# MILAB-IIT-CV/ATDN_vSLAM

Measured on AMD Instinct MI355X. Metric: frame-pairs/sec, KITTI 1241x376 odometry inference at 1/2/4/8 MI355X, higher is better.
Workload: dtype f32 via 3xf16 split MFMA (fp32 accumulate); 1 GPU; KITTI seq-03-shaped 376x1241 uint8 frames (resident in HBM) resized to 376x1232, GMA flow 12 GRU iters + CLVO head -> 6-DoF trajectory (BASELINE configs[1]); streams_per_gpu=2, gru_iters=12, parallelism=pairs sharded x1, one all-gather of 512-d features, replicated LSTM scan

## Files before the change

### atdn_vslam_amd/csrc/capi.hip

```cpp
#include "../../include/atdn_hip.h"

#include <cmath>
#include <cstring>

#include "clvo.h"
#include "gma.h"
#include "vae.h"
#include "clvo_train.h"
#include "train_kernels.h"
#include "frontend.h"
#include "conv_sf.h"
#include "depth_fusion_host.h"
#include "epilogues_sf.h"
#include "epipolar_host.h"
#include "flow_args.h"
#include "flow_consistency_host.h"
#include "flow_track_host.h"
#include "multiview_depth_host.h"
#include "pnp_host.h"
#include "two_view_host.h"
#include "warm_start_host.h"

namespace atdn {
extern template TileChoice conv_dispatch<MODE_TAP, EpiBias<ACT_NONE>>(const ConvShape&, EpiBias<ACT_NONE>, hipStream_t);
extern template TileChoice conv_dispatch<MODE_TAP, EpiBias<ACT_RELU>>(const ConvShape&, EpiBias<ACT_RELU>, hipStream_t);
extern template TileChoice conv_dispatch<MODE_ROW, EpiBias<ACT_NONE>>(const ConvShape&, EpiBias<ACT_NONE>, hipStream_t);
extern template TileChoice conv_dispatch<MODE_ROW, EpiBias<ACT_RELU>>(const ConvShape&, EpiBias<ACT_RELU>, hipStream_t);
extern template TileChoice conv_dispatch<MODE_TAP, EpiScale>(const ConvShape&, EpiScale, hipStream_t);

extern template TileChoice conv_sf_dispatch<EpiBias<ACT_NONE>>(const ConvShape&, float, EpiBias<ACT_NONE>, hipStream_t);
extern template TileChoice conv_sf_dispatch<SfBias<ACT_NONE>>(const ConvShape&, float, SfBias<ACT_NONE>, hipStream_t);

static thread_local std::string g_last_error;
void set_last_error(const std::string& msg) { g_last_error = msg; }
}

using namespace atdn;

struct atdn_gma { GmaNet net; atdn_gma(int H, int W, int B, int prec) : net(H, W, B, prec) {} };
struct atdn_clvo { ClvoNet net; atdn_clvo(int H, int W, int B) : net(H, W, B) {} };
struct atdn_vae { VaeEncoder net; atdn_vae(int H, int W, int B) : net(H, W, B) {} };
struct atdn_ingest { FrameIngest in; atdn_ingest(int a, int b, int c, int d, int n, int aa) : in(a, b, c, d, n, aa) {} };
struct atdn_clvo_trainer { ClvoTrainer net; atdn_clvo_trainer(int H, int W, int B, int T) : net(H, W, B, T) {} };

template <class T>
static void euler_yxz(const T* r, T* R) {
  const T c1 = std::cos(r[0]), c2 = std::cos(r[1]), c3 = std::cos(r[2]);
  const T s1 = std::sin(r[0]), s2 = std::sin(r[1]), s3 = std::sin(r[2]);
  R[0] = c1 * c3 + s1 * s2 * s3; R[1] = c3 * s1 * s2 - c1 * s3; R[2] = c2 * s1;
  R[3] = c2 * s3;                R[4] = c2 * c3;                R[5] = -s2;
  R[6] = c1 * s2 * s3 - c3 * s1; R[7] = c1 * c3 * s2 + s1 * s3; R[8] = c1 * c2;
}
template <class T>
static void make_transform(const T* rot, const T* tr, T* m) {
  T R[9];
  euler_yxz(rot, R);
  for (int i = 0; i < 3; ++i) { for (int j = 0; j < 3; ++j) m[i * 4 + j] = R[i * 3 + j]; m[i * 4 + 3] = tr[i]; }
  m[12] = 0; m[13] = 0; m[14] = 0; m[15] = 1;
}
template <class T>
static void matmul4(const T* a, const T* b, T* c) {
  for (int i = 0; i < 4; ++i)
    for (int j = 0; j < 4; ++j) {
      T s = 0;
      for (int k = 0; k < 4; ++k) s += a[i * 4 + k] * b[k * 4 + j];
      c[i * 4 + j] = s;
    }
}

extern "C" {

int atdn_version(void) { return 100; }
const char* atdn_last_error(void) { return g_last_error.c_str(); }

int atdn_gma_create(atdn_gma** out, int H, int W, int max_batch, int precision) {
  ATDN_API_BEGIN
  ATDN_CHECK(out, "null out pointer");
  *out = new atdn_gma(H, W, max_batch, precision);
  ATDN_API_END
}
int atdn_gma_set_low_latency(atdn_gma* h, int on) {
  ATDN_API_BEGIN
  ATDN_CHECK(h, "null handle");
  h->net.set_low_latency(on != 0);
  ATDN_API_END
}
int atdn_gma_load(atdn_gma* h, const char* key, const float* data, const int64_t* shape, int rank) {
  ATDN_API_BEGIN
  ATDN_CHECK(h && key && data && rank >= 0 && rank <= 4, "bad state-dict entry");
  h->net.state().put(key, data, shape, rank);
  ATDN_API_END
}
int atdn_gma_finalize(atdn_gma* h) {
  ATDN_API_BEGIN
  ATDN_CHECK(h, "null handle");
  h->net.finalize();
  ATDN_API_END
}
int atdn_gma_forward(atdn_gma* h, const float* im1, const float* im2, int B, int iters, const float* flow_init,
                     float* flow_low, float* flow_up, void* stream) {
  ATDN_API_BEGIN
  ATDN_CHECK(h, "null handle");
  h->net.forward(im1, im2, B, iters, flow_init, flow_low, flow_up, (hipStream_t)stream);
  ATDN_API_END
}
int atdn_gma_forward_predictions(atdn_gma* h, const float* im1, const float* im2, int B, int iters, const float* flow_init,
                                 float* flow_predictions, void* stream) {
  ATDN_API_BEGIN
  ATDN_CHECK(h, "null handle");
  h->net.forward_predictions(im1, im2, B, iters, flow_init, flow_predictions, (hipStream_t)stream);
  ATDN_API_END
}
int atdn_gma_forward_sequence(atdn_gma* h, const float* frames, int B, int iters, const float* flow_init,
                              float* flow_low, float* flow_up, void* stream) {
  ATDN_API_BEGIN
  ATDN_CHECK(h, "null handle");
  h->net.forward_sequence(frames, B, iters, flow_init, flow_low, flow_up, (hipStream_t)stream);
  ATDN_API_END
}
int atdn_gma_forward_sequence_continued(atdn_gma* h, const float* frames, int B, int iters, const float* flow_init,
                                        float* flow_low, float* flow_up, void* stream) {
  ATDN_API_BEGIN
  ATDN_CHECK(h, "null handle");
  h->net.forward_sequence(frames, B, iters, flow_init, flow_low, flow_up, (hipStream_t)stream, true);
  ATDN_API_END
}
long atdn_gma_debug_read(atdn_gma* h, const char* name, float* host, long capacity, void* stream) {
  try {
    if (!h || !name || !host) throw Error("null argument");
    const long n = h->net.debug_read(name, host, capacity, (hipStream_t)stream);
    if (n < 0) throw Error(std::string("unknown tensor name: ") + name);
    return n;
  } catch (const std::exception& e) {
    set_last_error(e.what());
    return -1;
  }
}
int atdn_gma_profile(atdn_gma* h, int B, int iters, int reps, float* ms_out, void* stream) {
  ATDN_API_BEGIN
  ATDN_CHECK(h && ms_out, "null argument");
  static_assert(GmaNet::ST_COUNT == ATDN_GMA_STAGES, "stage table out of sync with the header");
  h->net.profile(B, iters, reps, ms_out, (hipStream_t)stream, 0);
  ATDN_API_END
}
int atdn_gma_profile_mode(atdn_gma* h, int B, int iters, int reps, int mode, float* ms_out, void* stream) {
  ATDN_API_BEGIN
  ATDN_CHECK(h && ms_out, "null argument");
  ATDN_CHECK(mode >= 0 && mode <= 2, "mode must be 0 (pair), 1 (sequence) or 2 (continued sequence)");
  h->net.profile(B, iters, reps, ms_out, (hipStream_t)stream, mode);
  ATDN_API_END
}
int atdn_gma_set_range_probe(atdn_gma* h, int on) {
  ATDN_API_BEGIN
  ATDN_CHECK(h, "null handle");
  h->net.set_probe(on != 0);
  ATDN_API_END
}
long atdn_gma_range_rows(atdn_gma* h) {
  if (!h) { set_last_error("null handle"); return -1; }
  return (long)h->net.probe_rows().size();
}
int atdn_gma_range_row(atdn_gma* h, long index, char* name, int name_capacity, int* iteration, int* limited, float* max_abs,
                       int64_t* over, int64_t* nonfinite) {
  ATDN_API_BEGIN
  ATDN_CHECK(h && name && iteration && limited && max_abs && over && nonfinite, "null argument");
  const auto& rows = h->net.probe_rows();
  ATDN_CHECK(index >= 0 && index < (long)rows.size(), "row index out of range");
  const GmaNet::ProbeRow& r = rows[(size_t)index];
  ATDN_CHECK(name_capacity > (int)r.name.size(), "name buffer too small");
  memcpy(name, r.name.c_str(), r.name.size() + 1);
  *iteration = r.iter; *limited = r.limited ? 1 : 0; *max_abs = r.max_abs;
  *over = (int64_t)r.over; *nonfinite = (int64_t)r.nonfinite;
  ATDN_API_END
}
int atdn_range_probe_launch(const float* x, int64_t rows, int64_t cols, int64_t ld, void* slot, void* stream) {
  ATDN_API_BEGIN
  launch_range_probe(x, (long)rows, (long)cols, (long)ld, static_cast<RangeSlot*>(slot), (hipStream_t)stream);
  ATDN_API_END
}
int atdn_range_probe(const float* x, int64_t rows, int64_t cols, int64_t ld, float* max_abs, int64_t* over, int64_t* nonfinite,
                     void* stream) {
  ATDN_API_BEGIN
  ATDN_CHECK(x && max_abs && over && nonfinite, "null argument");
  hipStream_t st = (hipStream_t)stream;
  DeviceArray<RangeSlot> slot;
  RangeSlot host{};
  slot.alloc(1);
  ATDN_HIP(hipMemsetAsync(slot.p, 0, sizeof(RangeSlot), st));
  launch_range_probe(x, (long)rows, (long)cols, (long)ld, slot.p, st);
  ATDN_HIP(hipMemcpyAsync(&host, slot.p, sizeof(RangeSlot), hipMemcpyDeviceToHost, st));
  ATDN_HIP(hipStreamSynchronize(st));
  memcpy(max_abs, &host.max_bits, sizeof(float));
  *over = (int64_t)host.over;
  *nonfinite = (int64_t)host.nonfinite;
  ATDN_API_END
}
size_t atdn_gma_workspace_bytes(atdn_gma* h) { return h ? h->net.workspace_bytes() : 0; }
void atdn_gma_destroy(atdn_gma* h) { delete h; }
int64_t atdn_device_bytes_live(void) { return (int64_t)device_bytes_live.load(); }

int atdn_clvo_create(atdn_clvo** out, int H, int W, int max_batch) {
  ATDN_API_BEGIN
  ATDN_CHECK(out, "null out pointer");
  *out = new atdn_clvo(H, W, max_batch);
  ATDN_API_END
}
int atdn_clvo_load(atdn_clvo* h, const char* key, const float* data, const int64_t* shape, int rank) {
  ATDN_API_BEGIN
  ATDN_CHECK(h && key && data && rank >= 0 && rank <= 4, "bad state-dict entry");
  h->net.state().put(key, data, shape, rank);
  ATDN_API_END
}
int atdn_clvo_finalize(atdn_clvo* h) {
  ATDN_API_BEGIN
  ATDN_CHECK(h, "null handle");
  h->net.finalize();
  ATDN_API_END
}
int atdn_clvo_encode(atdn_clvo* h, const float* flow, int B, float* feat, void* stream) {
  ATDN_API_BEGIN
  ATDN_CHECK(h && flow && feat, "null argument");
  h->net.encode(flow, B, feat, (hipStream_t)stream);
  ATDN_API_END
}
int atdn_clvo_step(atdn_clvo* h, const float* feat, int T, int Bs, float* state, float* rot, float* tr, void* stream) {
  ATDN_API_BEGIN
  ATDN_CHECK(h && feat && state && rot && tr, "null argument");
  h->net.step(feat, T, Bs, state, rot, tr, (hipStream_t)stream);
  ATDN_API_END
}
int atdn_clvo_last_scan_path(atdn_clvo* h) { return h ? h->net.last_scan_path() : 0; }
void atdn_clvo_destroy(atdn_clvo* h) { delete h; }

int atdn_vae_create(atdn_vae** out, int H, int W, int max_batch) {
  ATDN_API_BEGIN
  ATDN_CHECK(out, "null out pointer");
  *out = new atdn_vae(H, W, max_batch);
  ATDN_API_END
}
int atdn_vae_load(atdn_vae* h, const char* key, const float* data, const int64_t* shape, int rank) {
  ATDN_API_BEGIN
  ATDN_CHECK(h && key && data && rank >= 0 && rank <= 4, "bad state-dict entry");
  h->net.state().put(key, data, shape, rank);
  ATDN_API_END
}
int atdn_vae_finalize(atdn_vae* h) {
  ATDN_API_BEGIN
  ATDN_CHECK(h, "null handle");
  h->net.finalize();
  ATDN_API_END
}
int atdn_vae_embedding_shape(const atdn_vae* h, int* out_h, int* out_w) {
  ATDN_API_BEGIN
  ATDN_CHECK(h && out_h && out_w, "null argument");
  *out_h = h->net.out_h();
  *out_w = h->net.out_w();
  ATDN_API_END
}
int atdn_vae_encode(atdn_vae* h, const float* images, int B, float* mu, void* stream) {
  ATDN_API_BEGIN
  ATDN_CHECK(h && images && mu, "null argument");
  h->net.encode(images, B, mu, (hipStream_t)stream);
  ATDN_API_END
}
int atdn_vae_debug_stage(atdn_vae* h, const float* images, int B, int stage, float* out, long capacity, void* stream) {
  ATDN_API_BEGIN
  ATDN_CHECK(h && images && out, "null argument");
  h->net.debug_stage(images, B, stage, out, capacity, (hipStream_t)stream);
  ATDN_API_END
}
int atdn_vae_scratch_floats(int H, int W, long* floats, int* stages) {
  ATDN_API_BEGIN
  ATDN_CHECK(floats && stages, "null argument");
  ATDN_CHECK(H >= 1 && W >= 1 && (long)H * W <= (1L << 24), "frame size out of range");
  const VaePlan p = vae_plan(H, W);
  floats[0] = p.in4; floats[1] = p.bufA; floats[2] = p.bufB; floats[3] = p.bufS;
  for (int k = 0; k < kVaeStages; ++k) { stages[3 * k] = p.h[k]; stages[3 * k + 1] = p.w[k]; stages[3 * k + 2] = p.ld[k]; }
  ATDN_API_END
}
void atdn_vae_destroy(atdn_vae* h) { delete h; }

int atdn_clvo_trainer_create(atdn_clvo_trainer** out, int H, int W, int batch, int sequence_length) {
  ATDN_API_BEGIN
  ATDN_CHECK(out, "null out pointer");
  *out = new atdn_clvo_trainer(H, W, batch, sequence_length);
  ATDN_API_END
}
int atdn_clvo_trainer_load(atdn_clvo_trainer* h, const char* key, const float* data, const int64_t* shape, int rank) {
  ATDN_API_BEGIN
  ATDN_CHECK(h && key && data && rank >= 0 && rank <= 4, "bad state-dict entry");
  h->net.state().put(key, data, shape, rank);
  ATDN_API_END
}
int atdn_clvo_trainer_finalize(atdn_clvo_trainer* h) {
  ATDN_API_BEGIN
  ATDN_CHECK(h, "null handle");
  h->net.finalize();
  ATDN_API_END
}
int atdn_clvo_trainer_forward_backward(atdn_clvo_trainer* h, const float* flows, const float* true_rot, const float* true_tr,
                                       float* pred_rot, float* pred_tr, float* loss_out, void* stream) {
  ATDN_API_BEGIN
  ATDN_CHECK(h && flows && true_rot && true_tr && loss_out, "null argument");
  *loss_out = h->net.forward_backward(flows, true_rot, true_tr, pred_rot, pred_tr, (hipStream_t)stream);
  ATDN_API_END
}
int atdn_clvo_trainer_gradients(atdn_clvo_trainer* h, float** device_ptr, long* count) {
  ATDN_API_BEGIN
  ATDN_CHECK(h && device_ptr && count, "null argument");
  *device_ptr = h->net.grad_buffer();
  *count = h->net.grad_count();
  ATDN_API_END
}
int atdn_clvo_trainer_adamw_step(atdn_clvo_trainer* h, float lr, float weight_decay, float eps, int step, void* stream) {
  ATDN_API_BEGIN
  ATDN_CHECK(h, "null handle");
  h->net.adamw_step(lr, weight_decay, eps, step, (hipStream_t)stream);
  ATDN_API_END
}
int atdn_clvo_trainer_set_loss(atdn_clvo_trainer* h, float alpha, int w, int mode) {
  ATDN_API_BEGIN
  ATDN_CHECK(h, "null handle");
  h->net.set_loss(alpha, w, mode);
  ATDN_API_END
}
int atdn_clvo_trainer_loss_terms(atdn_clvo_trainer* h, float* terms3_host) {
  ATDN_API_BEGIN
  ATDN_CHECK(h && terms3_host, "null argument");
  const float* t = h->net.loss_terms();
  ATDN_CHECK(t, "loss_terms: no iteration with alpha != 1 has run since set_loss");
  std::memcpy(terms3_host, t, 3 * sizeof(float));
  ATDN_API_END
}
int atdn_clvo_loss(const float* pred_rot, const float* pred_tr, const float* true_rot, const float* true_tr, int B, int T, float alpha,
                   int w, int mode, float* loss3_host, float* d_rot, float* d_tr, void* stream) {
  ATDN_API_BEGIN
  ATDN_CHECK(pred_rot && pred_tr && true_rot && true_tr && loss3_host && d_rot && d_tr, "null argument");
  ATDN_CHECK(mode == 0 || mode == 1, "atdn_clvo_loss: mode is 0 (reference) or 1 (gradient)");
  ATDN_CHECK(B >= 1 && T >= 1 && w >= 1 && w <= T, "atdn_clvo_loss: the composite window needs 1 <= w <= sequence length");
  hipStream_t st = (hipStream_t)stream;
  DeviceBuf loss3;
  loss3.alloc(4);
  launch_clvo_loss_composite(pred_rot, pred_tr, true_rot, true_tr, B, T, alpha, w, mode == 1, false, loss3.p, d_rot, d_tr, st);
  ATDN_HIP(hipMemcpyAsync(loss3_host, loss3.p, 3 * sizeof(float), hipMemcpyDeviceToHost, st));
  ATDN_HIP(hipStreamSynchronize(st));
  ATDN_API_END
}
long atdn_clvo_trainer_read(atdn_clvo_trainer* h, const char* key, int kind, float* host, long capacity, void* stream) {
  try {
    ATDN_CHECK(h && key && host, "null argument");
    return h->net.read(key, kind, host, capacity, (hipStream_t)stream);
  } catch (const std::exception& e) {
    set_last_error(e.what());
    return -1;
  }
}
void atdn_clvo_trainer_destroy(atdn_clvo_trainer* h) { delete h; }

int atdn_pose_transform_f32(const float* rot, const float* tr, float* mat16) {
  ATDN_API_BEGIN
  ATDN_CHECK(rot && tr && mat16, "null argument");
  make_transform(rot, tr, mat16);
  ATDN_API_END
}
int atdn_pose_rel2abs(const float* rot, const float* tr, int T, double* poses) {
  ATDN_API_BEGIN
  ATDN_CHECK(rot && tr && poses && T >= 0, "bad argument");
  for (int i = 0; i < 16; ++i) poses[i] = (i % 5 == 0) ? 1.0 : 0.0;
  for (int t = 0; t < T; ++t) {
    const double r[3] = {rot[t * 3], rot[t * 3 + 1], rot[t * 3 + 2]};
    const double x[3] = {tr[t * 3], tr[t * 3 + 1], tr[t * 3 + 2]};
    double m[16];
    make_transform(r, x, m);
    matmul4(poses + (long)t * 16, m, poses + (long)(t + 1) * 16);
  }
  ATDN_API_END
}
int atdn_pose_accumulate_f32(float* pose16, const float* rot, const float* tr) {
  ATDN_API_BEGIN
  ATDN_CHECK(pose16 && rot && tr, "null argument");
  float m[16], o[16];
  make_transform(rot, tr, m);
  matmul4(pose16, m, o);
  for (int i = 0; i < 16; ++i) pose16[i] = o[i];
  ATDN_API_END
}

int atdn_flow_forward_interpolate_host(const float* flow_low, int B, int h, int w, float* out) {
  ATDN_API_BEGIN
  ATDN_CHECK(flow_low && out, "null argument");
  ATDN_CHECK(B >= 1 && h >= 1 && w >= 1 && (long)h * w <= (1L << 24), "bad batch or grid size");
  const long bytes = (long)B * 2 * h * w * 4;
  ATDN_CHECK(disjoint(flow_low, bytes, out, bytes), "input and output overlap");
  forward_interpolate_host(flow_low, B, h, w, out);
  ATDN_API_END
}

int atdn_flow_consistency_host(const float* flow_fw, const float* flow_bw, int B, int H, int W, double alpha1, double alpha2,
                               unsigned char* mask, int* count) {
  ATDN_API_BEGIN
  flow_consistency_check_args(flow_fw, flow_bw, B, H, W, alpha1, alpha2, mask, count);
  flow_consistency_host(flow_fw, flow_bw, B, H, W, alpha1, alpha2, mask, count);
  ATDN_API_END
}

int atdn_flow_two_view_depth_host(const float* flow, const float* pose, const unsigned char* mask, int B, int H, int W, double fx,
                                  double fy, double cx, double cy, double max_epipolar, double min_sin2, double max_depth,
                                  float* depth, int* counts) {
  ATDN_API_BEGIN
  const TwoViewCamera cam{fx, fy, cx, cy, max_epipolar, min_sin2, max_depth};
  two_view_check_args(flow, pose, mask, B, H, W, cam, depth, counts);
  two_view_depth_host(flow, pose, mask, B, H, W, cam, depth, counts);
  ATDN_API_END
}

int atdn_flow_track_step_host(const float* flow, const unsigned char* mask, const float* acc_in, const unsigned char* alive_in,
                              int B, int H, int W, float* acc_out, unsigned char* alive_out, const float* pose, double fx,
                              double fy, double cx, double cy, double max_epipolar, double min_sin2, double max_depth, float* depth,
                              int* counts) {
  ATDN_API_BEGIN
  const TwoViewCamera cam{fx, fy, cx, cy, max_epipolar, min_sin2, max_depth};
  flow_track_check_args(flow, mask, acc_in, alive_in, B, H, W, acc_out, alive_out, pose, cam, depth, counts);
  flow_track_step_host(flow, mask, acc_in, alive_in, B, H, W, acc_out, alive_out, pose, cam, depth, counts);
  ATDN_API_END
}

int atdn_depth_fuse_host(const float* bank, const float* poses, const int* targets, const int* sources, int N, int B, int S, int H,
                         int W, double fx, double fy, double cx, double cy, double max_reproj, double max_rel_depth, int min_views,
                         double min_z, int average, float* fused, unsigned char* views, int* counts) {
  ATDN_API_BEGIN
  depth_fuse_check_args(bank, poses, targets, sources, N, B, S, H, W, fx, fy, cx, cy, max_reproj, max_rel_depth, min_views, min_z,
                        fused, views, counts);
  depth_fuse_host(bank, poses, targets, sources, N, B, S, H, W,
                  depth_fuse_params(fx, fy, cx, cy, max_reproj, max_rel_depth, min_views, min_z, average), fused, views, counts);
  ATDN_API_END
}

int atdn_multiview_depth_host(const float* acc_bank, const unsigned char* alive_bank, const float* poses, const int* slots,
                              const float* depth_init, int N, int B, int S, int H, int W, double fx, double fy, double cx, double cy,
                              double scale_px, double inlier_px, double min_z, int min_views, double max_rel_sigma, double max_depth,
                              int iters, float* depth, float* info, unsigned char* views, int* counts) {
  ATDN_API_BEGIN
  multiview_check_args(acc_bank, alive_bank, poses, slots, depth_init, N, B, S, H, W, fx, fy, cx, cy, scale_px, inlier_px, min_z,
                       min_views, max_rel_sigma, max_depth, iters, depth, info, views, counts);
  multiview_depth_host(acc_bank, alive_bank, poses, slots, depth_init, N, B, S, H, W,
                       multiview_params(fx, fy, cx, cy, scale_px, inlier_px, min_z, min_views, max_rel_sigma, max_depth, iters, H, W),
                       depth, info, views, counts);
  ATDN_API_END
}

int atdn_pnp_terms_host(const float* depth, const float* flow, const unsigned char* mask, const float* pose, int B, int H, int W,
                        double fx, double fy, double cx, double cy, double scale_px, double inlier_px, double min_z, double* sums,
                        int* counts) {
  ATDN_API_BEGIN
  const void* out[2] = {sums, counts};
  const long out_bytes[2] = {(long)B * PNP_TERMS * 8, (long)B * 12};
  pnp_check_args(depth, flow, mask, pose, B, H, W, fx, fy, cx, cy, scale_px, inlier_px, min_z, false, out, out_bytes, 2);
  pnp_terms_host(depth, flow, mask, pose, B, H, W, pnp_params(fx, fy, cx, cy, scale_px, inlier_px, min_z, H, W), sums, counts);
  ATDN_API_END
}

int atdn_pnp_solve_host(const float* depth, const float* flow, const unsigned char* mask, const float* pose_init, int B, int H,
                        int W, double fx, double fy, double cx, double cy, double scale_px, double inlier_px, double min_z, int iters,
                        float* pose_out, double* cost, int* counts) {
  ATDN_API_BEGIN
  const void* out[3] = {pose_out, cost, counts};
  const long out_bytes[3] = {(long)B * 48, (long)B * 8, (long)B * 16};
  pnp_check_args(depth, flow, mask, pose_init, B, H, W, fx, fy, cx, cy, scale_px, inlier_px, min_z, false, out, out_bytes, 3);
  ATDN_CHECK(iters >= 0 && iters <= 64, "iters must be in [0, 64]");
  pnp_solve_host(depth, flow, mask, pose_init, B, H, W, pnp_params(fx, fy, cx, cy, scale_px, inlier_px, min_z, H, W), iters,
                 pose_out, cost, counts);
  ATDN_API_END
}

int atdn_epipolar_terms_host(const float* flow, const unsigned char* mask, const float* pose, int B, int H, int W, double fx,
                             double fy, double cx, double cy, double scale_px, double inlier_px, double* sums, int* counts) {
  ATDN_API_BEGIN
  const void* out[2] = {sums, counts};
  const long out_bytes[2] = {(long)B * PLANE_TERMS * 8, (long)B * 12};
  epipolar_check_args(flow, mask, pose, B, H, W, fx, fy, cx, cy, scale_px, inlier_px, false, out, out_bytes, 2);
  epipolar_terms_host(flow, mask, pose, B, H, W, epipolar_params(fx, fy, cx, cy, scale_px, inlier_px), sums, counts);
  ATDN_API_END
}

int atdn_epipolar_solve_host(const float* flow, const unsigned char* mask, const float* pose_init, int B, int H, int W, double fx,
                             double fy, double cx, double cy, double scale_px, double inlier_px, int iters, float* pose_out,
                             double* cost, int* counts) {
  ATDN_API_BEGIN
  const void* out[3] = {pose_out, cost, counts};
  const long out_bytes[3] = {(long)B * 48, (long)B * 8, (long)B * 16};
  epipolar_check_args(flow, mask, pose_init, B, H, W, fx, fy, cx, cy, scale_px, inlier_px, false, out, out_bytes, 3);
  ATDN_CHECK(iters >= 0 && iters <= 64, "iters must be in [0, 64]");
  epipolar_solve_host(flow, mask, pose_init, B, H, W, epipolar_params(fx, fy, cx, cy, scale_px, inlier_px), iters, pose_out, cost,
                      counts);
  ATDN_API_END
}

int atdn_corr_lookup(const float* pyr0, const float* pyr1, const float* pyr2, const float* pyr3, int B, int H8,
                     int W8, const float* coords, float* out, int ldo, void* stream) {
  ATDN_API_BEGIN
  ATDN_CHECK(pyr0 && pyr1 && pyr2 && pyr3 && coords && out && B >= 1, "null argument");
  ATDN_CHECK((H8 >> 3) >= 2 && (W8 >> 3) >= 2, "map too small for four pyramid levels");
  PyramidLevels pl;
  const float* b[4] = {pyr0, pyr1, pyr2, pyr3};
  for (int l = 0; l < 4; ++l) { pl.base[l] = b[l]; pl.H[l] = H8 >> l; pl.W[l] = W8 >> l; }
  launch_lookup(pl, coords, (long)B * H8 * W8, out, ldo, (hipStream_t)stream);
  ATDN_API_END
}

int atdn_corr_pyramid(const float* fmap1, const float* fmap2, int B, int H8, int W8, int C, float* pyr0, float* pyr1,
                      float* pyr2, float* pyr3, void* stream) {
  ATDN_API_BEGIN
  ATDN_CHECK(fmap1 && fmap2 && pyr0 && pyr1 && pyr2 && pyr3 && B >= 1 && C % 32 == 0, "bad argument");
  const int N = H8 * W8;
  ConvShape c;
  c.src0 = fmap1; c.ld0 = C; c.sb0 = (long)N * C; c.C0 = C; c.H = 1; c.W = N;
  c.w = fmap2; c.wb = (long)N * C; c.ldw = C; c.N = N; c.nimg = B;
  conv_dispatch<MODE_TAP>(c, EpiScale{1.0f / sqrtf((float)C), pyr0, (long)N * N, N}, (hipStream_t)stream);
  float* p[4] = {pyr0, pyr1, pyr2, pyr3};
  for (int l = 1; l < 4; ++l) launch_avgpool(p[l - 1], H8 >> (l - 1), W8 >> (l - 1), p[l], (long)B * N, (hipStream_t)stream);
  ATDN_API_END
}

int atdn_corr_lookup_bricks(const float* fmap1, const float* fmap2, int B, int H8, int W8, int C, const float* coords,
                            float* pyr0, float* pyr1, float* pyr2, float* pyr3, float* samples,
                            const float* convc1_weight_host, const float* convc1_bias_host, float* cor1, void* stream) {
  ATDN_API_BEGIN
  ATDN_CHECK(fmap1 && fmap2 && B >= 1 && H8 >= 1 && W8 >= 1, "bad argument");
  ATDN_CHECK(C == 256, "the correlation kernel keeps a source strip's whole K = 256 in registers: C must be 256");
  ATDN_CHECK((H8 >> 3) >= 2 && (W8 >> 3) >= 2, "map too small for four pyramid levels");
  ATDN_CHECK(!(samples || cor1) || coords, "a lookup needs coordinates");
  ATDN_CHECK(!cor1 || (convc1_weight_host && convc1_bias_host), "cor1 needs convc1's weight [256][324] and bias [256]");
  hipStream_t st = (hipStream_t)stream;
  const int N = H8 * W8;
  const long n8 = (long)B * N;
  BrickPyramid bp;
  bp.N = N; bp.NPB = brick_pixel_blocks(N);
  WeightArena A;
  DeviceBuf f1, f2, plain[3], fbrick[4], pyr[4], scratch, outsf, csf;
  sf_counter_attach();
  f1.alloc(n8 * 256); f2.alloc(n8 * 256);
  launch_to_sf(fmap1, f1.p, n8, 256, st);
  launch_to_sf(fmap2, f2.p, n8, 256, st);
  float* rowmajor[4] = {pyr0, pyr1, pyr2, pyr3};
  int pH[4], pW[4];
  for (int l = 0; l < 4; ++l) {
    pH[l] = H8 >> l; pW[l] = W8 >> l;
    bp.H[l] = pH[l]; bp.W[l] = pW[l]; bp.BW[l] = cdiv(pW[l], 8); bp.BH[l] = cdiv(pH[l], 4); bp.NB[l] = bp.BW[l] * bp.BH[l] * 32;
    const float* src = f2.p;
    long src_sb = (long)N * 256;
    if (l > 0) {
      const float* prev = l == 1 ? f2.p : plain[l - 2].p;
      const long prev_sb = l == 1 ? (long)N * 256 : (long)pH[l - 1] * pW[l - 1] * 256;
      src_sb = (long)pH[l] * pW[l] * 256;
      plain[l - 1].alloc((long)B * src_sb);
      launch_pool_features_sf(prev, B, pH[l - 1], pW[l - 1], 256, prev_sb, plain[l - 1].p, src_sb, st);
      src = plain[l - 1].p;
    }
    fbrick[l].alloc((long)B * bp.NB[l] * 256);
    launch_brick_rows(src, src_sb, B, pH[l], pW[l], 256, fbrick[l].p, (long)bp.NB[l] * 256, st);
    pyr[l].alloc((long)B * bp.NPB * kBrickPixelBlock * bp.NB[l]);
    launch_corr_bricks(f1.p, (long)N * 256, fbrick[l].p, (long)bp.NB[l] * 256, B, N, bp.NB[l], 1.0f / sqrtf(256.0f), pyr[l].p, false, st);
    bp.base[l] = pyr[l].p;
    if (rowmajor[l]) launch_unbrick(pyr[l].p, bp.NB[l], N, pH[l], pW[l], n8, rowmajor[l], st);
  }
  if (samples) {
    outsf.alloc(n8 * 352);
    launch_lookup_bricks(bp, coords, n8, outsf.p, st);
    scratch.alloc(n8 * 352);
    launch_from_sf(outsf.p, scratch.p, n8, 352, st);
    ATDN_HIP(hipMemcpy2DAsync(samples, 324 * sizeof(float), scratch.p, 352 * sizeof(float), 324 * sizeof(float), (size_t)n8,
                              hipMemcpyDeviceToDevice, st));
  }
  if (cor1) {
    StateDict sd;
    const int64_t ws[4] = {256, 324, 1, 1}, bs[1] = {256};
    sd.put("c.weight", convc1_weight_host, ws, 4);
    sd.put("c.bias", convc1_bias_host, bs, 1);
    PackedConv L = pack_conv_sf(A, sd, {"c"});
    pack_fragment_major16(A, L);
    A.upload();
    resolve(A, L);
    csf.alloc(n8 * 256);
    launch_lookup_conv(bp, coords, n8, nullptr, L.wf16, L.wscale, L.b, csf.p, false, st);
    launch_from_sf(csf.p, cor1, n8, 256, st);
    ATDN_HIP(hipStreamSynchronize(st));
  }
  ATDN_HIP(hipStreamSynchronize(st));
  ATDN_API_END
}

int atdn_conv2d_nhwc(const float* src, int nimg, int H, int W, int Cin, const float* weight_host,
                     const float* bias_host, int Cout, int KH, int KW, int stride, int padH, int padW, int relu,
                     float* dst, void* stream) {
  ATDN_API_BEGIN
  ATDN_CHECK(src && weight_host && dst && nimg >= 1, "null argument");
  const bool row = (Cin == 4 || Cin == 16);
  ATDN_CHECK(row || Cin % 32 == 0, "Cin must be 4, 16 or a multiple of 32");
  StateDict sd;
  const int64_t ws[4] = {Cout, Cin, KH, KW};
  sd.put("c.weight", weight_host, ws, 4);
  std::vector<float> zb(Cout, 0.f);
  const int64_t bs[1] = {Cout};
  sd.put("c.bias", bias_host ? bias_host : zb.data(), bs, 1);
  WeightArena A;
  PackedConv L = pack_conv(A, sd, {"c"}, row ? MODE_ROW : MODE_TAP, Cin);
  A.upload();
  resolve(A, L);
  ConvShape s;
  s.src0 = src; s.ld0 = Cin; s.sb0 = (long)H * W * Cin; s.C0 = L.C; s.H = H; s.W = W;
  s.KH = KH; s.KW = KW; s.stride = stride; s.padH = padH; s.padW = padW;
  s.w = L.w; s.ldw = L.ldw; s.N = Cout; s.nimg = nimg;
  const int Ho = conv_out(H, KH, stride, padH), Wo = conv_out(W, KW, stride, padW);
  hipStream_t st = (hipStream_t)stream;
  if (row) {
    if (relu) conv_dispatch<MODE_ROW>(s, EpiBias<ACT_RELU>{L.b, dst, (long)Ho * Wo * Cout, Cout, 1.f}, st);
    else conv_dispatch<MODE_ROW>(s, EpiBias<ACT_NONE>{L.b, dst, (long)Ho * Wo * Cout, Cout, 1.f}, st);
  } else {
    if (relu) conv_dispatch<MODE_TAP>(s, EpiBias<ACT_RELU>{L.b, dst, (long)Ho * Wo * Cout, Cout, 1.f}, st);
    else conv_dispatch<MODE_TAP>(s, EpiBias<ACT_NONE>{L.b, dst, (long)Ho * Wo * Cout, Cout, 1.f}, st);
  }
  ATDN_HIP(hipStreamSynchronize(st));
  ATDN_API_END
}

int atdn_resize_frames(const float* src, int planes, int Hin, int Win, int Hout, int Wout, float* dst, void* stream) {
  return atdn_resize_frames_mode(src, planes, Hin, Win, Hout, Wout, ATDN_RESIZE_ANTIALIAS, dst, stream);
}
int atdn_resize_frames_mode(const float* src, int planes, int Hin, int Win, int Hout, int Wout, int antialias, float* dst,
                            void* stream) {
  ATDN_API_BEGIN
  ATDN_CHECK(src && dst && planes >= 1 && Hin >= 1 && Win >= 1 && Hout >= 1 && Wout >= 1, "bad argument");
  ATDN_CHECK(antialias == 0 || antialias == 1, "antialias must be ATDN_RESIZE_BILINEAR or ATDN_RESIZE_ANTIALIAS");
  launch_resize<float>(src, planes, Hin, Win, Hout, Wout, antialias, dst, (hipStream_t)stream);
  ATDN_API_END
}
int atdn_resize_frames_u8(const uint8_t* src, int planes, int Hin, int Win, int Hout, int Wout, int antialias, float* dst,
                          void* stream) {
  ATDN_API_BEGIN
  ATDN_CHECK(src && dst && planes >= 1 && Hin >= 1 && Win >= 1 && Hout >= 1 && Wout >= 1, "bad argument");
  ATDN_CHECK(antialias == 0 || antialias == 1, "antialias must be ATDN_RESIZE_BILINEAR or ATDN_RESIZE_ANTIALIAS");
  launch_resize<unsigned char>(src, planes, Hin, Win, Hout, Wout, antialias, dst, (hipStream_t)stream);
  ATDN_API_END
}
int atdn_pad_frames(const float* src, int planes, int H, int W, int left, int right, int top, int bottom, float* dst,
                    void* stream) {
  ATDN_API_BEGIN
  ATDN_CHECK(src && dst && planes >= 1 && H >= 1 && W >= 1 && left >= 0 && right >= 0 && top >= 0 && bottom >= 0, "bad argument");
  launch_pad_replicate(src, planes, H, W, left, right, top, bottom, dst, (hipStream_t)stream);
  ATDN_API_END
}
int atdn_ingest_create(atdn_ingest** out, int Hin, int Win, int Hout, int Wout, int max_frames, int antialias) {
  ATDN_API_BEGIN
  ATDN_CHECK(out, "null out pointer");
  ATDN_CHECK(antialias == 0 || antialias == 1, "antialias must be ATDN_RESIZE_BILINEAR or ATDN_RESIZE_ANTIALIAS");
  *out = new atdn_ingest(Hin, Win, Hout, Wout, max_frames, antialias);
  ATDN_API_END
}
int atdn_ingest_frames_u8(atdn_ingest* h, const uint8_t* host_frames, int n_frames, float* dst, void* stream) {
  ATDN_API_BEGIN
  ATDN_CHECK(h, "null handle");
  h->in.ingest(host_frames, n_frames, dst, (hipStream_t)stream);
  ATDN_API_END
}
void atdn_ingest_destroy(atdn_ingest* h) { delete h; }

int atdn_conv2d_nhwc_sf_epi(const float* src, int nimg, int H, int W, int Cin, const float* weight_host,
                            const float* bias_host, int Cout, int KH, int KW, int stride, int padH, int padW, int sf_store,
                            float* dst, void* stream) {
  ATDN_API_BEGIN
  ATDN_CHECK(src && weight_host && dst && nimg >= 1 && Cin % 32 == 0, "bad argument (Cin must be a multiple of 32)");
  ATDN_CHECK(sf_store >= 0 && sf_store <= 7 && (sf_store & 6) != 6, "sf_store: bit 0 names the epilogue, bit 1 or bit 2 the tile form");
  const int tile_form = (sf_store & 2) ? 1 : (sf_store & 4) ? 2 : 0;
  sf_store &= 1;
  ATDN_CHECK(!sf_store || Cout % 32 == 0, "the split-f16 store needs Cout % 32 == 0");
  StateDict sd;
  const int64_t ws[4] = {Cout, Cin, KH, KW};
  sd.put("c.weight", weight_host, ws, 4);
  std::vector<float> zb(Cout, 0.f);
  const int64_t bs[1] = {Cout};
  sd.put("c.bias", bias_host ? bias_host : zb.data(), bs, 1);
  WeightArena A;
  PackedConv L = pack_conv_sf(A, sd, {"c"});
  A.upload();
  resolve(A, L);
  hipStream_t st = (hipStream_t)stream;
  DeviceBuf tmp, osf;
  const long rows = (long)nimg * H * W;
  tmp.alloc(rows * Cin);
  launch_to_sf(src, tmp.p, rows, Cin, st);
  ConvShape s;
  s.src0 = tmp.p; s.ld0 = Cin; s.sb0 = (long)H * W * Cin; s.C0 = L.C; s.H = H; s.W = W;
  s.KH = KH; s.KW = KW; s.stride = stride; s.padH = padH; s.padW = padW;
  s.w = L.w; s.ldw = L.ldw; s.N = Cout; s.nimg = nimg;
  const int Ho = conv_out(H, KH, stride, padH), Wo = conv_out(W, KW, stride, padW);
  s.wfrag16 = L.wf16;
  s.tile_form = tile_form;
  if (sf_store) {
    const long orows = (long)nimg * Ho * Wo;
    osf.alloc(orows * Cout);
    conv_sf_dispatch(s, L.wscale, SfBias<ACT_NONE>{L.b, osf.p, (long)Ho * Wo * Cout, Cout}, st);
    launch_from_sf(osf.p, dst, orows, Cout, st);
    ATDN_HIP(hipStreamSynchronize(st));
  } else {
    conv_sf_dispatch(s, L.wscale, EpiBias<ACT_NONE>{L.b, dst, (long)Ho * Wo * Cout, Cout, 1.f}, st);
    ATDN_HIP(hipStreamSynchronize(st));
  }
  ATDN_API_END
}

int atdn_conv2d_nhwc_sf(const float* src, int nimg, int H, int W, int Cin, const float* weight_host,
                        const float* bias_host, int Cout, int KH, int KW, int stride, int padH, int padW, float* dst,
                        void* stream) {
  return atdn_conv2d_nhwc_sf_epi(src, nimg, H, W, Cin, weight_host, bias_host, Cout, KH, KW, stride, padH, padW, 0, dst, stream);
}

}
```

### atdn_vslam_amd/csrc/corr_bricks.hip

```cpp
#include "kernels.h"

#include "conv_mfma.h"
#include "sf.h"

namespace atdn {
namespace {

typedef float v4f __attribute__((ext_vector_type(4)));
typedef float f32x4v __attribute__((ext_vector_type(4)));
typedef __attribute__((address_space(1))) v4f gv4f;

struct CorrArgs {
  const float* f1; long sb1;
  const float* f2b; long sb2;
  float* out;
  int B, N, NB, NPB, strips, splits, tiles_per_split;
  float scale;
};

template <bool FAST>
__global__ __launch_bounds__(256, 2) void corr_bricks_kernel(const CorrArgs a) {
  constexpr int KROW = 160;
  constexpr int KT = 32;
  constexpr int NC = 8;
  constexpr int CH = KT * KROW;
  constexpr int IMG = NC * CH;
  __shared__ __attribute__((aligned(16))) char lds[2 * IMG];

  const int tid = threadIdx.x, lane = tid & 63, wave = tid >> 6;
  const int nblk = a.B * a.splits * a.strips;
  const int id = xcd_remap(blockIdx.x, nblk);
  const int strip4 = id % a.strips;
  const int rest = id / a.strips;
  const int split = rest % a.splits, b = rest / a.splits;
  const int n16 = lane & 15, g16 = lane >> 4;
  const char* f1 = reinterpret_cast<const char*>(a.f1 + (long)b * a.sb1);
  const char* f2 = reinterpret_cast<const char*>(a.f2b + (long)b * a.sb2);

  f16x8 qh[2][NC], ql[2][NC];
  int mrow[2];
#pragma unroll
  for (int rb = 0; rb < 2; ++rb) {
    mrow[rb] = (strip4 * 4 + wave) * 32 + 16 * rb + n16;
    const char* qrow = f1 + (long)min(mrow[rb], a.N - 1) * 1024 + 16 * g16;
#pragma unroll
    for (int c = 0; c < NC; ++c) {
      qh[rb][c] = *reinterpret_cast<const f16x8*>(qrow + c * 128);
      if (!FAST) ql[rb][c] = *reinterpret_cast<const f16x8*>(qrow + c * 128 + 64);
    }
  }

  const int lr = tid >> 3, ls = tid & 7;
  const int t0 = split * a.tiles_per_split;
  const int nt = min(a.tiles_per_split, a.NB / KT - t0);
  v4f kreg[NC];
  auto fetch = [&](int j) __attribute__((always_inline)) {
    const char* src = f2 + (long)((t0 + j) * KT + lr) * 1024 + 16 * ls;
#pragma unroll
    for (int c = 0; c < NC; ++c) kreg[c] = *reinterpret_cast<const v4f*>(src + c * 128);
  };
  auto stash = [&](int buf) __attribute__((always_inline)) {
#pragma unroll
    for (int c = 0; c < NC; ++c) *reinterpret_cast<v4f*>(lds + buf * IMG + c * CH + lr * KROW + 16 * ls) = kreg[c];
  };
  const bool odd = (lane & 1) != 0;
  long orow[2][2];
  const long NBK = a.NB / KT;
#pragma unroll
  for (int rb = 0; rb < 2; ++rb)
#pragma unroll
    for (int h = 0; h < 2; ++h) {
      const int prow = h == 0 ? (mrow[rb] & ~1) : (mrow[rb] | 1);
      orow[rb][h] = ((((long)b * a.NPB + (prow >> 6)) * NBK + t0) * 64 + (prow & 63)) * KT + (odd ? 16 : 0) + 4 * g16;
    }

  fetch(0);
  stash(0);
  __syncthreads();
  fetch(min(1, nt - 1));
  for (int j = 0; j < nt; ++j) {
    const char* img = lds + (j & 1) * IMG + n16 * KROW + 16 * g16;
    f32x4v acc[2][2];
#pragma unroll
    for (int kb = 0; kb < 2; ++kb)
#pragma unroll
      for (int rb = 0; rb < 2; ++rb)
#pragma unroll
        for (int e = 0; e < 4; ++e) acc[kb][rb][e] = 0.f;
    f16x8 kh[2][2], kl[2][2];
    auto read_rows = [&](int set, int c) __attribute__((always_inline)) {
#pragma unroll
      for (int kb = 0; kb < 2; ++kb) {
        const char* kp = img + c * CH + 16 * kb * KROW;
        kh[set][kb] = *reinterpret_cast<const f16x8*>(kp);
        if (!FAST) kl[set][kb] = *reinterpret_cast<const f16x8*>(kp + 64);
      }
    };
    read_rows(0, 0);
#pragma unroll
    for (int c = 0; c < NC; ++c) {
      if (c + 1 < NC) read_rows((c + 1) & 1, c + 1);
      __builtin_amdgcn_sched_barrier(0);
#pragma unroll
      for (int kb = 0; kb < 2; ++kb)
#pragma unroll
        for (int rb = 0; rb < 2; ++rb) {
          f32x4v v = acc[kb][rb];
          if (!FAST) {
            v = __builtin_amdgcn_mfma_f32_16x16x32_f16(kl[c & 1][kb], qh[rb][c], v, 0, 0, 0);
            v = __builtin_amdgcn_mfma_f32_16x16x32_f16(kh[c & 1][kb], ql[rb][c], v, 0, 0, 0);
          }
          v = __builtin_amdgcn_mfma_f32_16x16x32_f16(kh[c & 1][kb], qh[rb][c], v, 0, 0, 0);
          acc[kb][rb] = v;
        }
      __builtin_amdgcn_sched_barrier(0);
    }
    stash((j + 1) & 1);
    fetch(min(j + 2, nt - 1));
#pragma unroll
    for (int rb = 0; rb < 2; ++rb) {
      const f32x4v A = acc[0][rb] * a.scale, Bv = acc[1][rb] * a.scale;
      f32x4v recv;
#pragma unroll
      for (int e = 0; e < 4; ++e) {
        const float send = odd ? A[e] : Bv[e];
        recv[e] = __int_as_float(__builtin_amdgcn_update_dpp(0, __float_as_int(send), 0xB1, 0xF, 0xF, true));
      }
      f32x4v v1, v2;
#pragma unroll
      for (int e = 0; e < 4; ++e) { v1[e] = odd ? recv[e] : A[e]; v2[e] = odd ? Bv[e] : recv[e]; }
      __builtin_nontemporal_store(v1, reinterpret_cast<gv4f*>(reinterpret_cast<uintptr_t>(a.out + orow[rb][0])));
      __builtin_nontemporal_store(v2, reinterpret_cast<gv4f*>(reinterpret_cast<uintptr_t>(a.out + orow[rb][1])));
      orow[rb][0] += 64 * KT;
      orow[rb][1] += 64 * KT;
    }
    __syncthreads();
  }
}

}

void launch_corr_bricks(const float* f1, long sb1, const float* f2b, long sb2, int B, int N, int NB, float scale, float* out,
                        bool fast, hipStream_t st) {
  ATDN_CHECK(f1 && f2b && out && B >= 1 && N >= 1 && NB >= 32 && NB % 32 == 0, "corr_bricks: bad argument");
  CorrArgs a;
  a.NPB = brick_pixel_blocks(N);
  a.f1 = f1; a.sb1 = sb1; a.f2b = f2b; a.sb2 = sb2; a.out = out; a.B = B; a.N = N; a.NB = NB; a.scale = scale;
  a.strips = cdiv(N, 128);
  const int tiles = NB / 32;
  int best = 1;
  double best_eff = 0.0;
  for (int s = 1; s <= 8; ++s) {
    const int tps = cdiv(tiles, s);
    if (s > 1 && tps < 8) break;
    const int used = cdiv(tiles, tps);
    const double blocks = (double)B * a.strips * used;
    const double eff = blocks / (512.0 * std::ceil(blocks / 512.0));
    if (eff > best_eff + 0.02) { best_eff = eff; best = s; }
  }
  a.tiles_per_split = cdiv(tiles, best);
  a.splits = cdiv(tiles, a.tiles_per_split);
  const int nblk = B * a.splits * a.strips;
  if (fast) hipLaunchKernelGGL(corr_bricks_kernel<true>, dim3(nblk), dim3(256), 0, st, a);
  else hipLaunchKernelGGL(corr_bricks_kernel<false>, dim3(nblk), dim3(256), 0, st, a);
  ATDN_HIP(hipGetLastError());
}

}
```

### atdn_vslam_amd/csrc/gma.h

```cpp
#pragma once
#include <vector>
#include <map>
#include <memory>

#include "attention.h"
#include "conv_dispatch.h"
#include "device_buf.h"
#include "kernels.h"
#include "range_probe.h"
#include "weights.h"

namespace atdn {

struct EncoderWeights {
  PackedConv stem;
  struct Block { PackedConv c1, c2, ds; bool has_ds = false; } blk[6];
  PackedConv head;
};

class GmaNet {
 public:
  GmaNet(int H, int W, int max_batch, int precision);
  ~GmaNet();
  StateDict& state() { return sd_; }
  void finalize();
  void forward(const float* im1, const float* im2, int B, int iters, const float* flow_init, float* flow_low,
               float* flow_up, hipStream_t st);
  void forward_predictions(const float* im1, const float* im2, int B, int iters, const float* flow_init, float* preds,
                           hipStream_t st);
  void forward_sequence(const float* frames, int B, int iters, const float* flow_init, float* flow_low, float* flow_up,
                        hipStream_t st, bool continued = false);
  long debug_read(const char* name, float* host, long capacity, hipStream_t st);
  size_t workspace_bytes() const { return ws_bytes_; }
  enum Stage { ST_FNET = 0, ST_CORR, ST_POOL, ST_CNET, ST_ATTN, ST_LOOKUP, ST_MOTION, ST_AGG, ST_GRU_ZR, ST_GRU_Q, ST_FLOWHEAD,
               ST_MASK, ST_GRU_CTX, ST_ATTN_LOGITS, ST_AGG_VT, ST_CONVC1, ST_GRU_ZR_V, ST_GRU_Q_V, ST_COUNT };
  void profile(int B, int iters, int reps, float* ms, hipStream_t st, int mode = 0);

  int H, W, H8, W8, N, ldN, maxB, precision;
  int dev_ = 0;
  bool norm_on_load_ = false;
  bool classic_ = false;
  bool low_latency_ = false;
  void set_low_latency(bool on);
  DeviceBuf attn_part_;
  DeviceBuf enc2_[4];
  hipStream_t par_stream_ = nullptr;
  std::vector<hipEvent_t> par_events_;
  size_t par_next_ = 0;
  bool par_ = false;
  bool par_ok_ = true;
  void fork(hipStream_t from, hipStream_t to);
  DeviceBuf fbrick_[4], fplain_[3], coords_used_;
  int brickBW_[4], brickBH_[4], brickNB_[4];
  BrickPyramid brick_pyramid() const;
  DeviceBuf rowmax_, rinv_;

  struct ProbeRow { std::string name; int iter; bool limited; float max_abs; long long over, nonfinite; };
  static constexpr int kProbeMaxRows = 1536;
  void set_probe(bool on);
  const std::vector<ProbeRow>& probe_rows() const { return probe_rows_; }

 private:
  bool probe_ = false;
  int probe_it_ = -1;
  DeviceArray<RangeSlot> probe_slots_;
  std::vector<ProbeRow> probe_rows_;
  void probe_begin(hipStream_t st);
  void probe_end(hipStream_t st);
  void probe(const std::string& name, bool limited, const float* p, long rows, long cols, long ld, hipStream_t st);
  void run_body(int B, int iters, hipStream_t st);
  void run_encoder(const EncoderWeights& E, bool instance, int nimg, hipStream_t st, float** out_buf, int* outH,
                   int* outW);
  void iteration(int B, hipStream_t st);
  void run_body_sf(int B, int iters, hipStream_t st);
  void run_encoder_sf(const EncoderWeights& E, bool instance, int nimg, hipStream_t st, float** out_buf, int first_img = 0,
                      DeviceBuf* bufs = nullptr);
  void iteration_sf(int B, hipStream_t st);
  void capture(int B, int iters);
  void launch_body(int B, int iters, hipStream_t st);
  int seq_ = 0;
  int last_frame_ = -1;
  float* preds_out_ = nullptr;
  long preds_stride_ = 0;
  void mask_head_sf(int B, hipStream_t st);
  void mask_head(int B, hipStream_t st);
  int last_B_ = 0;

  StateDict sd_;
  WeightArena arena_;
  bool ready_ = false;
  bool use_graph_ = true;
  EncoderWeights fnet_, cnet_;
  PackedConv convc1_, convc2_, convf1_, convf2_, convm_, to_v_, to_qk_;
  long convf1_sf_off_ = -1;
  float convf1_wscale_ = 1.f;
  float fh2_mul_ = 1.f;
  long fh2_w32_off_ = -1;
  DeviceBuf fhG_;
  PackedConv gru_zr_[2], gru_q_[2], fh1_, fh2_, mask0_, mask2_;
  PackedConv gru_zr_ctx_[2], gru_q_ctx_[2];
  const float* gamma_ = nullptr;
  long gamma_off_ = -1;
  long to_v_w32_off_ = -1;

  DeviceBuf img4_, enc_[4], scratch_, pcnt_, fin_, fmap_, psum_, pm2_, mean_[3], rstd_[3];
  DeviceBuf pyr_[4], h_[2], x_, qk_, attn_, vT_, corrfeat_, cor1_, corflo_, flo1_, z_, rh_, fh_, mask_;
  DeviceBuf coords1_, flow4_, pre_zr_[2], pre_q_[2];
  int pyrH_[4], pyrW_[4];
  size_t ws_bytes_ = 0;

  struct Timer;
  Timer* timer_ = nullptr;
  void mark(int stage, hipStream_t st);

  hipStream_t cap_stream_ = nullptr;
  std::map<std::pair<int, int>, hipGraphExec_t> graphs_;
};

}
```

### atdn_vslam_amd/csrc/gma.hip

```cpp
#include "gma.h"
#include "small_convs.h"
#include "conv_sf.h"
#include "epilogues_sf.h"

namespace atdn { const float* zero_line(); }

namespace atdn {

extern template TileChoice conv_dispatch<MODE_TAP, EpiBias<ACT_NONE>>(const ConvShape&, EpiBias<ACT_NONE>, hipStream_t);
extern template TileChoice conv_dispatch<MODE_TAP, EpiBias<ACT_RELU>>(const ConvShape&, EpiBias<ACT_RELU>, hipStream_t);
extern template TileChoice conv_dispatch<MODE_ROW, EpiBias<ACT_RELU>>(const ConvShape&, EpiBias<ACT_RELU>, hipStream_t);
extern template TileChoice conv_dispatch<MODE_TAP, EpiBiasStats>(const ConvShape&, EpiBiasStats, hipStream_t);
extern template TileChoice conv_dispatch<MODE_ROW, EpiBiasStats>(const ConvShape&, EpiBiasStats, hipStream_t);
extern template TileChoice conv_dispatch<MODE_TAP, EpiBiasReluAddRelu>(const ConvShape&, EpiBiasReluAddRelu, hipStream_t);
extern template TileChoice conv_dispatch<MODE_TAP, EpiContextSplit>(const ConvShape&, EpiContextSplit, hipStream_t);
extern template TileChoice conv_dispatch<MODE_TAP, EpiScale>(const ConvShape&, EpiScale, hipStream_t);
extern template TileChoice conv_dispatch<MODE_TAP, EpiQK>(const ConvShape&, EpiQK, hipStream_t);
extern template TileChoice conv_dispatch<MODE_TAP, EpiStoreT>(const ConvShape&, EpiStoreT, hipStream_t);
extern template TileChoice conv_dispatch<MODE_TAP, EpiAggregate>(const ConvShape&, EpiAggregate, hipStream_t);
extern template TileChoice conv_dispatch<MODE_TAP, EpiGruZR>(const ConvShape&, EpiGruZR, hipStream_t);
extern template TileChoice conv_dispatch<MODE_TAP, EpiGruQ>(const ConvShape&, EpiGruQ, hipStream_t);
extern template TileChoice conv_dispatch<MODE_TAP, EpiFlowDelta>(const ConvShape&, EpiFlowDelta, hipStream_t);

extern template TileChoice conv_dispatch<MODE_ROW, SfBias<ACT_RELU>>(const ConvShape&, SfBias<ACT_RELU>, hipStream_t);
#define ATDN_EXTERN_SF(EPI) extern template TileChoice conv_sf_dispatch<EPI>(const ConvShape&, float, EPI, hipStream_t);
ATDN_EXTERN_SF(SfBias<ACT_NONE>) ATDN_EXTERN_SF(SfBias<ACT_RELU>) ATDN_EXTERN_SF(EpiBias<ACT_NONE>)
ATDN_EXTERN_SF(EpiBiasStats) ATDN_EXTERN_SF(SfBiasReluAddRelu) ATDN_EXTERN_SF(SfContextSplit)
ATDN_EXTERN_SF(SfQK) ATDN_EXTERN_SF(SfVT)
ATDN_EXTERN_SF(SfGruZR) ATDN_EXTERN_SF(SfGruQ)
extern template void conv_sf_dispatch_pair<SfBias<ACT_RELU>>(const ConvShape&, float, SfBias<ACT_RELU>, const ConvShape&, float,
                                                             SfBias<ACT_RELU>, hipStream_t);

namespace {

struct FastGuard {
  bool prev;
  explicit FastGuard(bool on) : prev(sf_fast_mode()) { sf_fast_mode() = on; }
  ~FastGuard() { sf_fast_mode() = prev; }
};

constexpr int XLD = 384;
constexpr int CORR_LD = 352;

ConvShape conv_shape(const PackedConv& L, const float* src, int ld, long sb, int nimg, int H, int W, int stride,
                     int padH, int padW) {
  ConvShape s;
  s.src0 = src; s.ld0 = ld; s.sb0 = sb; s.C0 = L.C;
  s.H = H; s.W = W; s.KH = L.KH; s.KW = L.KW; s.stride = stride; s.padH = padH; s.padW = padW;
  s.w = L.w; s.wfrag16 = L.wf16; s.ldw = L.ldw; s.N = L.N; s.nimg = nimg;
  return s;
}

EncoderWeights pack_encoder(WeightArena& A, const StateDict& sd, const std::string& p, bool batchnorm, bool sf) {
  EncoderWeights E;
  auto fold = [&](const std::string& norm) { return bn_affine(sd, norm); };
  auto pack_conv = [&](WeightArena& A_, const StateDict& sd_, const std::vector<std::string>& names, int mode, int cpix,
                       const ChannelAffine* f = nullptr) {
    return (sf && mode == MODE_TAP) ? pack_conv_sf(A_, sd_, names, f) : atdn::pack_conv(A_, sd_, names, mode, cpix, f);
  };
  if (batchnorm) { auto a = fold(p + "norm1"); E.stem = pack_conv(A, sd, {p + "conv1"}, MODE_ROW, 4, &a); }
  else E.stem = pack_conv(A, sd, {p + "conv1"}, MODE_ROW, 4);
  if (sf) pack_stem_sf(A, E.stem);
  int bi = 0;
  for (int li = 1; li <= 3; ++li)
    for (int k = 0; k < 2; ++k, ++bi) {
      const std::string q = p + "layer" + std::to_string(li) + "." + std::to_string(k) + ".";
      auto& B = E.blk[bi];
      B.has_ds = (li > 1 && k == 0);
      if (batchnorm) {
        auto a1 = fold(q + "norm1"), a2 = fold(q + "norm2");
        B.c1 = pack_conv(A, sd, {q + "conv1"}, MODE_TAP, 0, &a1);
        B.c2 = pack_conv(A, sd, {q + "conv2"}, MODE_TAP, 0, &a2);
        if (B.has_ds) { auto a3 = fold(q + "norm3"); B.ds = pack_conv(A, sd, {q + "downsample.0"}, MODE_TAP, 0, &a3); }
      } else {
        B.c1 = pack_conv(A, sd, {q + "conv1"}, MODE_TAP, 0);
        B.c2 = pack_conv(A, sd, {q + "conv2"}, MODE_TAP, 0);
        if (B.has_ds) B.ds = pack_conv(A, sd, {q + "downsample.0"}, MODE_TAP, 0);
      }
    }
  E.head = pack_conv(A, sd, {p + "conv2"}, MODE_TAP, 0);
  return E;
}

void resolve_encoder(const WeightArena& A, EncoderWeights& E) {
  resolve(A, E.stem);
  for (auto& b : E.blk) { resolve(A, b.c1); resolve(A, b.c2); if (b.has_ds) resolve(A, b.ds); }
  resolve(A, E.head);
}

}

struct GmaNet::Timer {
  std::vector<std::pair<int, hipEvent_t>> marks;
  hipEvent_t start = nullptr;
};

void GmaNet::mark(int stage, hipStream_t st) {
  if (!timer_) return;
  hipEvent_t e;
  ATDN_HIP(hipEventCreate(&e));
  ATDN_HIP(hipEventRecord(e, st));
  timer_->marks.emplace_back(stage, e);
}

void GmaNet::profile(int B, int iters, int reps, float* ms, hipStream_t st, int mode) {
  ATDN_CHECK(ready_ && B >= 1 && B <= maxB && reps >= 1, "bad profile request");
  ATDN_CHECK(mode == 0 || precision >= 1, "sequence modes are built for the split-f16 pipeline");
  ATDN_CHECK(!probe_, "switch the range probe off before profiling: its launches would be timed with the stages");
  for (int i = 0; i < ST_COUNT; ++i) ms[i] = 0.f;
  seq_ = mode;
  last_frame_ = 0;
  for (int r = 0; r < reps; ++r) {
    Timer t;
    timer_ = &t;
    if (precision >= 1) launch_init_coords_sf(nullptr, B, H8, W8, coords1_.p, flow4_.p, x_.p, XLD, 254, st);
    else launch_init_coords(nullptr, B, H8, W8, coords1_.p, flow4_.p, x_.p + 254, XLD, st);
    ATDN_HIP(hipEventCreate(&t.start));
    ATDN_HIP(hipEventRecord(t.start, st));
    try { if (precision >= 1) { FastGuard fg(precision == 2); run_body_sf(B, iters, st); } else run_body(B, iters, st); } catch (...) { timer_ = nullptr; throw; }
    timer_ = nullptr;
    ATDN_HIP(hipStreamSynchronize(st));
    hipEvent_t prev = t.start;
    for (auto& m : t.marks) {
      float d = 0.f;
      ATDN_HIP(hipEventElapsedTime(&d, prev, m.second));
      ms[m.first] += d;
      prev = m.second;
    }
    for (auto& m : t.marks) (void)hipEventDestroy(m.second);
    (void)hipEventDestroy(t.start);
  }
}

GmaNet::GmaNet(int H_, int W_, int max_batch, int precision_) : H(H_), W(W_), maxB(max_batch), precision(precision_) {
  ATDN_CHECK(precision >= 0 && precision <= 2, "precision must be 0 (fp32 MFMA), 1 (split-f16 MFMA) or 2 (plain f16 MFMA)");
  ATDN_CHECK(H % 8 == 0 && W % 8 == 0 && H > 0 && W > 0, "frame size must be a multiple of 8 (use the padder)");
  ATDN_CHECK(H >= 128 && W >= 128,
             "frame size must be at least 128x128: level 3 of the correlation pyramid needs at least 2x2 cells (the reference "
             "divides by H/64 - 1 and W/64 - 1 when it samples that level, and returns NaN below)");
  ATDN_CHECK(max_batch >= 1 && max_batch <= 64, "max_batch out of range");
  H8 = H / 8; W8 = W / 8; N = H8 * W8; ldN = round_up(N, 32);
  norm_on_load_ = precision == 1;
  classic_ = precision == 0;
  const char* ng = getenv("ATDN_NO_GRAPH");
  use_graph_ = !(ng && ng[0] == '1');
  (void)hipGetDevice(&dev_);
}

void GmaNet::fork(hipStream_t from, hipStream_t to) {
  ATDN_CHECK(par_next_ < par_events_.size(), "out of branch events");
  hipEvent_t e = par_events_[par_next_++];
  ATDN_HIP(hipEventRecord(e, from));
  ATDN_HIP(hipStreamWaitEvent(to, e, 0));
}

void GmaNet::set_low_latency(bool on) {
  ATDN_CHECK(!ready_, "set_low_latency: call it before finalize() (the workspace and the captured graphs depend on it)");
  low_latency_ = on;
}

GmaNet::~GmaNet() {
  DeviceGuard dg(dev_);
  (void)hipDeviceSynchronize();
  for (auto& kv : graphs_) (void)hipGraphExecDestroy(kv.second);
  if (cap_stream_) (void)hipStreamDestroy(cap_stream_);
  if (par_stream_) (void)hipStreamDestroy(par_stream_);
  for (auto& e : par_events_) (void)hipEventDestroy(e);
}

void GmaNet::set_probe(bool on) {
  ATDN_CHECK(!on || precision == 0,
             "the range probe needs an exact-fp32 handle (ATDN_PRECISION_F32): only that path writes every intermediate tensor "
             "as plain fp32 and never clamps; the split-f16 / f16 paths store range-limited values and fuse some tensors away");
  probe_ = on;
}

void GmaNet::probe_begin(hipStream_t st) {
  probe_slots_.reserve(kProbeMaxRows);
  ATDN_HIP(hipMemsetAsync(probe_slots_.p, 0, kProbeMaxRows * sizeof(RangeSlot), st));
  probe_rows_.clear();
  probe_it_ = -1;
}

void GmaNet::probe(const std::string& name, bool limited, const float* p, long rows, long cols, long ld, hipStream_t st) {
  ATDN_CHECK((int)probe_rows_.size() < kProbeMaxRows, "range probe: slot table full");
  launch_range_probe(p, rows, cols, ld, probe_slots_.p + probe_rows_.size(), st);
  probe_rows_.push_back({name, probe_it_, limited, 0.f, 0, 0});
}

void GmaNet::probe_end(hipStream_t st) {
  std::vector<RangeSlot> host(probe_rows_.size());
  if (!host.empty())
    ATDN_HIP(hipMemcpyAsync(host.data(), probe_slots_.p, host.size() * sizeof(RangeSlot), hipMemcpyDeviceToHost, st));
  ATDN_HIP(hipStreamSynchronize(st));
  for (size_t i = 0; i < host.size(); ++i) {
    ProbeRow& r = probe_rows_[i];
    static_assert(sizeof(float) == sizeof(unsigned int), "fp32");
    memcpy(&r.max_abs, &host[i].max_bits, sizeof(float));
    r.over = (long long)host[i].over;
    r.nonfinite = (long long)host[i].nonfinite;
  }
}

void GmaNet::finalize() {
  ATDN_CHECK(!ready_, "finalize called twice");
  const std::string u = "update_block.";
  const bool sf = precision >= 1;
  auto tap = [&](const std::vector<std::string>& names, bool has_bias = true) {
    return sf ? pack_conv_sf(arena_, sd_, names, nullptr, has_bias)
              : pack_conv(arena_, sd_, names, MODE_TAP, 0, nullptr, has_bias);
  };
  fnet_ = pack_encoder(arena_, sd_, "fnet.", false, sf);
  cnet_ = pack_encoder(arena_, sd_, "cnet.", true, sf);
  convc1_ = tap({u + "encoder.convc1"});
  if (sf) pack_fragment_major16(arena_, convc1_);
  convc2_ = tap({u + "encoder.convc2"});
  convf1_ = pack_conv(arena_, sd_, {u + "encoder.convf1"}, MODE_ROW, 4);
  {
    const HostTensor& w = sd_.get(u + "encoder.convf1.weight");
    ATDN_CHECK(w.shape[0] == 128 && w.shape[1] == 2 && w.shape[2] == 7 && w.shape[3] == 7, "convf1 is 7x7, 2 -> 128");
    float mx = 0.f;
    for (float v : w.data) mx = std::max(mx, std::fabs(v));
    int e = 0;
    if (mx > 0.f) (void)std::frexp(mx, &e);
    const int p = 1 - e;
    convf1_wscale_ = std::ldexp(1.0f, -p);
    convf1_sf_off_ = arena_.alloc(4L * 2 * 4 * 2 * 64 * 4);
    _Float16* f = reinterpret_cast<_Float16*>(arena_.at(convf1_sf_off_));
    for (int wv = 0; wv < 4; ++wv)
      for (int cb = 0; cb < 2; ++cb)
        for (int s = 0; s < 4; ++s)
          for (int lane = 0; lane < 64; ++lane)
            for (int i = 0; i < 8; ++i) {
              const int n = 32 * wv + 16 * cb + (lane & 15), g = lane >> 4;
              const int ky = 2 * s + (g >> 1), kx = 4 * (g & 1) + (i >> 1), c = i & 1;
              const float v = (ky < 7 && kx < 7) ? std::ldexp(w.data[(((long)n * 2 + c) * 7 + ky) * 7 + kx], p) : 0.f;
              const _Float16 hi = (_Float16)v, lo = (_Float16)(v - (float)hi);
              const long frag = (((long)wv * 2 + cb) * 4 + s) * 2;
              f[(frag * 64 + lane) * 8 + i] = hi;
              f[((frag + 1) * 64 + lane) * 8 + i] = lo;
            }
  }
  convf2_ = tap({u + "encoder.convf2"});
  convm_ = tap({u + "encoder.conv"});
  to_v_ = tap({u + "aggregator.to_v"}, false);
  to_qk_ = tap({"att.to_qk"}, false);
  for (int p = 0; p < 2; ++p) {
    const std::string t = std::to_string(p + 1);
    if (sf) {
      const std::vector<std::pair<int, int>> ctx = {{128, 256}};
      const HostTensor& wv = sd_.get(u + "aggregator.to_v.weight");
      const HostTensor& gam = sd_.get(u + "aggregator.gamma");
      ATDN_CHECK(gam.data.size() == 1, "aggregator.gamma is one value");
      gru_zr_[p] = pack_gru_sf_folded(arena_, sd_, {u + "gru.convz" + t, u + "gru.convr" + t}, wv, (double)gam.data[0]);
      gru_q_[p] = pack_gru_sf_folded(arena_, sd_, {u + "gru.convq" + t}, wv, (double)gam.data[0]);
      gru_zr_ctx_[p] = pack_conv_sf_channels(arena_, sd_, {u + "gru.convz" + t, u + "gru.convr" + t}, ctx, false);
      gru_q_ctx_[p] = pack_conv_sf_channels(arena_, sd_, {u + "gru.convq" + t}, ctx, false);
    } else {
      gru_zr_[p] = tap({u + "gru.convz" + t, u + "gru.convr" + t});
      gru_q_[p] = tap({u + "gru.convq" + t});
    }
  }
  fh1_ = tap({u + "flow_head.conv1"});
  fh2_ = tap({u + "flow_head.conv2"});
  if (sf) {
    const HostTensor& w = sd_.get(u + "flow_head.conv2.weight");
    ATDN_CHECK(w.shape.size() == 4 && w.shape[0] == 2 && w.shape[1] == 256 && w.shape[2] == 3 && w.shape[3] == 3, "flow head conv2 shape");
    fh2_w32_off_ = arena_.alloc(18 * 256);
    for (int o = 0; o < 2; ++o)
      for (int c = 0; c < 256; ++c)
        for (int t = 0; t < 9; ++t) arena_.at(fh2_w32_off_)[(t * 2 + o) * 256 + c] = w.data[((long)o * 256 + c) * 9 + t];
    float mx = 0.f;
    for (float v : w.data) mx = std::max(mx, std::fabs(v));
    int e = 0;
    if (mx > 0.f) (void)std::frexp(mx, &e);
    fh2_mul_ = std::ldexp(1.0f, 1 - e);
  }
  mask0_ = tap({u + "mask.0"});
  mask2_ = tap({u + "mask.2"});
  gamma_off_ = pack_vector(arena_, sd_.get(u + "aggregator.gamma").data);
  if (sf) to_v_w32_off_ = pack_vector(arena_, sd_.get(u + "aggregator.to_v.weight").data);
  arena_.upload();
  resolve_encoder(arena_, fnet_);
  resolve_encoder(arena_, cnet_);
  for (PackedConv* L : {&convc1_, &convc2_, &convf1_, &convf2_, &convm_, &to_v_, &to_qk_, &gru_zr_[0], &gru_zr_[1],
                        &gru_q_[0], &gru_q_[1], &fh1_, &fh2_, &mask0_, &mask2_})
    resolve(arena_, *L);
  if (sf) for (PackedConv* L : {&gru_zr_ctx_[0], &gru_zr_ctx_[1], &gru_q_ctx_[0], &gru_q_ctx_[1]}) resolve(arena_, *L);
  gamma_ = arena_.dev(gamma_off_);

  const int B = maxB;
  const int H2 = conv_out(H, 7, 2, 3), W2 = conv_out(W, 7, 2, 3);
  const long n8 = (long)B * N;
  img4_.alloc(2L * B * H * W * 4);
  for (int i = 0; i < (sf ? 4 : 3); ++i) enc_[i].alloc(2L * B * H2 * W2 * 64);
  fmap_.alloc(2L * B * N * 256);
  const long groups = (long)cdiv(H2 * W2, 64) * 4 + 8;
  psum_.alloc(2L * B * groups * 128); pm2_.alloc(2L * B * groups * 128); pcnt_.alloc(2L * B * groups); fin_.alloc(2L * B * 32 * 128 * 4 * 2);
  for (int i = 0; i < 3; ++i) { mean_[i].alloc(2L * B * 128); rstd_[i].alloc(2L * B * 128); }
  pyrH_[0] = H8; pyrW_[0] = W8;
  for (int l = 1; l < 4; ++l) { pyrH_[l] = pyrH_[l - 1] / 2; pyrW_[l] = pyrW_[l - 1] / 2; }
  ATDN_CHECK(pyrH_[3] >= 2 && pyrW_[3] >= 2, "frame too small for a 4-level pyramid");
  for (int l = 0; l < 4; ++l) {
    brickBW_[l] = cdiv(pyrW_[l], 8); brickBH_[l] = cdiv(pyrH_[l], 4); brickNB_[l] = brickBW_[l] * brickBH_[l] * 32;
    pyr_[l].alloc(classic_ ? n8 * pyrH_[l] * pyrW_[l] : (long)B * brick_pixel_blocks(N) * kBrickPixelBlock * brickNB_[l]);
  }
  if (sf) {
    for (int l = 0; l < 4; ++l) fbrick_[l].alloc((long)B * brickNB_[l] * 256);
    for (int l = 1; l < 4; ++l) fplain_[l - 1].alloc((long)B * pyrH_[l] * pyrW_[l] * 256);
    coords_used_.alloc(n8 * 2);
  }
  h_[0].alloc(n8 * 128); h_[1].alloc(n8 * 128); x_.alloc(n8 * XLD);
  const AttnGeom ag = attn_geom(B, N, ldN);
  qk_.alloc(n8 * 256); attn_.alloc(std::max(n8 * ldN, attn_floats(ag)));
  if (classic_) vT_.alloc((long)B * 128 * ldN);
  if (sf) { rowmax_.alloc((long)B * ag.Npad); rinv_.alloc((long)B * ag.Npad); }
  if (sf && low_latency_ && attn_v_splits(attn_geom(1, N, ldN)) > 1) attn_part_.alloc(8L * B * ag.Npad * 128);
  if (sf && low_latency_) {
    for (int i = 0; i < 4; ++i) enc2_[i].alloc((long)B * H2 * W2 * 64);
    ATDN_HIP(hipStreamCreateWithFlags(&par_stream_, hipStreamNonBlocking));
    par_events_.resize(2 * (1 + 64));
    for (auto& e : par_events_) ATDN_HIP(hipEventCreateWithFlags(&e, hipEventDisableTiming));
  }
  corrfeat_.alloc(n8 * CORR_LD); cor1_.alloc(n8 * 256); corflo_.alloc(n8 * 256); flo1_.alloc(n8 * 128);
  z_.alloc(n8 * 128); rh_.alloc(n8 * 128); fh_.alloc(n8 * 256); mask_.alloc(n8 * 576);
  if (sf) fhG_.alloc(2 * n8 * 18);
  coords1_.alloc(n8 * 2); flow4_.alloc(n8 * 4);
  if (sf) for (int p = 0; p < 2; ++p) { pre_zr_[p].alloc(n8 * 256); pre_q_[p].alloc(n8 * 128); }
  ATDN_HIP(hipMemset(corrfeat_.p, 0, corrfeat_.n * sizeof(float)));
  if (vT_.p) ATDN_HIP(hipMemset(vT_.p, 0, vT_.n * sizeof(float)));
  ATDN_HIP(hipMemset(attn_.p, 0, attn_.n * sizeof(float)));
  ATDN_HIP(hipMemset(flow4_.p, 0, flow4_.n * sizeof(float)));
  ATDN_HIP(hipDeviceSynchronize());
  ws_bytes_ = 0;
  DeviceBuf* all[] = {&img4_, &enc_[0], &enc_[1], &enc_[2], &enc_[3], &fmap_, &psum_, &pm2_, &pyr_[0], &pyr_[1], &pyr_[2],
                      &pyr_[3], &h_[0], &h_[1], &x_, &qk_, &attn_, &vT_, &corrfeat_, &cor1_, &corflo_, &flo1_, &z_,
                      &rh_, &fh_, &mask_, &coords1_, &flow4_};
  for (auto* b : all) ws_bytes_ += (size_t)b->n * sizeof(float);
  (void)zero_line();
  sf_counter_attach();
  ATDN_HIP(hipStreamCreateWithFlags(&cap_stream_, hipStreamNonBlocking));
  ready_ = true;
}

void GmaNet::run_encoder(const EncoderWeights& E, bool instance, int nimg, hipStream_t st, float** out_buf, int* outH,
                         int* outW) {
  int h = conv_out(H, 7, 2, 3), w = conv_out(W, 7, 2, 3);
  float* P = enc_[0].p; float* Q = enc_[1].p; float* R = enc_[2].p;
  auto stats_conv = [&](auto mode_tag, const PackedConv& L, const float* src, int ld, int ih, int iw, int stride,
                        int pad, float* dst, int slot) {
    constexpr int MODE = decltype(mode_tag)::value;
    ConvShape s = conv_shape(L, src, ld, (long)ih * iw * ld, nimg, ih, iw, stride, pad, pad);
    const int oh = conv_out(ih, L.KH, stride, pad), ow = conv_out(iw, L.KW, stride, pad);
    EpiBiasStats ep{L.b, dst, (long)oh * ow * L.N, L.N, psum_.p, pm2_.p, 0};
    TileChoice t = conv_dispatch<MODE>(s, ep, st);
    const int groups = cdiv(oh * ow, t.BM) * (t.BM / 32);
    ATDN_CHECK((long)nimg * groups * L.N <= psum_.n, "statistics scratch too small");
    launch_in_finalize_cnt(psum_.p, pm2_.p, nullptr, nimg, groups, oh * ow, L.N, 1e-5f, mean_[slot].p, rstd_[slot].p,
                           reinterpret_cast<double*>(fin_.p), st);
  };
  using TapT = std::integral_constant<int, MODE_TAP>;
  using RowT = std::integral_constant<int, MODE_ROW>;
  auto pr = [&](int bi, const char* leaf, bool limited, const float* p, long pixels, int ch) {
    if (!probe_) return;
    std::string name = instance ? "fnet." : "cnet.";
    if (bi >= 0) name += "layer" + std::to_string(bi / 2 + 1) + "." + std::to_string(bi % 2);
    probe(name + leaf, limited, p, (long)nimg * pixels, ch, ch, st);
  };

  if (instance) {
    stats_conv(RowT{}, E.stem, img4_.p, 4, H, W, 2, 3, P, 0);
    pr(-1, "conv1.raw", false, P, (long)h * w, 64);
    launch_in_apply(P, mean_[0].p, rstd_[0].p, nullptr, nullptr, nullptr, nimg, (long)h * w, 64, st);
  } else {
    ConvShape s = conv_shape(E.stem, img4_.p, 4, (long)H * W * 4, nimg, H, W, 2, 3, 3);
    conv_dispatch<MODE_ROW>(s, EpiBias<ACT_RELU>{E.stem.b, P, (long)h * w * 64, 64, 1.f}, st);
  }
  pr(-1, "conv1.out", true, P, (long)h * w, 64);
  int c = 64;
  for (int bi = 0; bi < 6; ++bi) {
    const auto& Bk = E.blk[bi];
    const int stride = Bk.has_ds ? 2 : 1;
    const int co = Bk.c1.N;
    const int oh = conv_out(h, 3, stride, 1), ow = conv_out(w, 3, stride, 1);
    const long ohw = (long)oh * ow;
    if (instance) {
      stats_conv(TapT{}, Bk.c1, P, c, h, w, stride, 1, Q, 0);
      pr(bi, ".conv1.raw", false, Q, ohw, co);
      launch_in_apply(Q, mean_[0].p, rstd_[0].p, nullptr, nullptr, nullptr, nimg, ohw, co, st);
      pr(bi, ".conv1.out", true, Q, ohw, co);
      stats_conv(TapT{}, Bk.c2, Q, co, oh, ow, 1, 1, R, 0);
      pr(bi, ".conv2.raw", false, R, ohw, co);
      if (Bk.has_ds) {
        stats_conv(TapT{}, Bk.ds, P, c, h, w, 2, 0, Q, 1);
        pr(bi, ".downsample.raw", false, Q, ohw, co);
        launch_in_apply(R, mean_[0].p, rstd_[0].p, Q, mean_[1].p, rstd_[1].p, nimg, ohw, co, st);
      } else {
        launch_in_apply(R, mean_[0].p, rstd_[0].p, P, nullptr, nullptr, nimg, ohw, co, st);
      }
      std::swap(P, R);
    } else {
      ConvShape s1 = conv_shape(Bk.c1, P, c, (long)h * w * c, nimg, h, w, stride, 1, 1);
      conv_dispatch<MODE_TAP>(s1, EpiBias<ACT_RELU>{Bk.c1.b, Q, ohw * co, co, 1.f}, st);
      pr(bi, ".conv1.out", true, Q, ohw, co);
      ConvShape s2 = conv_shape(Bk.c2, Q, co, ohw * co, nimg, oh, ow, 1, 1, 1);
      if (Bk.has_ds) {
        ConvShape sd = conv_shape(Bk.ds, P, c, (long)h * w * c, nimg, h, w, 2, 0, 0);
        conv_dispatch<MODE_TAP>(sd, EpiBias<ACT_NONE>{Bk.ds.b, R, ohw * co, co, 1.f}, st);
        pr(bi, ".downsample.out", true, R, ohw, co);
        conv_dispatch<MODE_TAP>(s2, EpiBiasReluAddRelu{Bk.c2.b, R, ohw * co, co, P, ohw * co, co}, st);
      } else {
        conv_dispatch<MODE_TAP>(s2, EpiBiasReluAddRelu{Bk.c2.b, P, ohw * co, co, R, ohw * co, co}, st);
        std::swap(P, R);
      }
    }
    pr(bi, "", true, P, ohw, co);
    h = oh; w = ow; c = co;
  }
  *out_buf = P; *outH = h; *outW = w;
}

void GmaNet::iteration(int B, hipStream_t st) {
  const long n8 = (long)B * N;
  PyramidLevels pl;
  for (int l = 0; l < 4; ++l) { pl.base[l] = pyr_[l].p; pl.H[l] = pyrH_[l]; pl.W[l] = pyrW_[l]; }
  launch_lookup(pl, coords1_.p, n8, corrfeat_.p, CORR_LD, st);
  mark(ST_LOOKUP, st);
  auto pr = [&](const char* name, bool limited, const float* p, long rows, long cols, long ld) {
    if (probe_) probe(name, limited, p, rows, cols, ld, st);
  };
  pr("corr_lookup", true, corrfeat_.p, n8, 324, CORR_LD);

  ConvShape s = conv_shape(convc1_, corrfeat_.p, CORR_LD, (long)N * CORR_LD, B, H8, W8, 1, 0, 0);
  conv_dispatch<MODE_TAP>(s, EpiBias<ACT_RELU>{convc1_.b, cor1_.p, (long)N * 256, 256, 1.f}, st);
  mark(ST_CONVC1, st);
  pr("encoder.convc1", true, cor1_.p, n8, 256, 256);
  s = conv_shape(convc2_, cor1_.p, 256, (long)N * 256, B, H8, W8, 1, 1, 1);
  conv_dispatch<MODE_TAP>(s, EpiBias<ACT_RELU>{convc2_.b, corflo_.p, (long)N * 256, 256, 1.f}, st);
  pr("encoder.convc2", true, corflo_.p, n8, convc2_.N, 256);
  s = conv_shape(convf1_, flow4_.p, 4, (long)N * 4, B, H8, W8, 1, 3, 3);
  conv_dispatch<MODE_ROW>(s, EpiBias<ACT_RELU>{convf1_.b, flo1_.p, (long)N * 128, 128, 1.f}, st);
  pr("encoder.convf1", true, flo1_.p, n8, 128, 128);
  s = conv_shape(convf2_, flo1_.p, 128, (long)N * 128, B, H8, W8, 1, 1, 1);
  conv_dispatch<MODE_TAP>(s, EpiBias<ACT_RELU>{convf2_.b, corflo_.p + 192, (long)N * 256, 256, 1.f}, st);
  pr("encoder.convf2", true, corflo_.p + 192, n8, convf2_.N, 256);
  s = conv_shape(convm_, corflo_.p, 256, (long)N * 256, B, H8, W8, 1, 1, 1);
  float* mf = x_.p + 128;
  conv_dispatch<MODE_TAP>(s, EpiBias<ACT_RELU>{convm_.b, mf, (long)N * XLD, XLD, 1.f}, st);
  mark(ST_MOTION, st);
  pr("encoder.conv", true, mf, n8, convm_.N, XLD);

  s = conv_shape(to_v_, mf, XLD, (long)N * XLD, B, H8, W8, 1, 0, 0);
  conv_dispatch<MODE_TAP>(s, EpiStoreT{vT_.p, (long)128 * ldN, ldN}, st);
  mark(ST_AGG_VT, st);
  pr("aggregator.to_v", true, vT_.p, (long)B * 128, N, ldN);
  ConvShape a;
  a.src0 = attn_.p; a.ld0 = ldN; a.sb0 = (long)N * ldN; a.C0 = ldN; a.H = 1; a.W = N;
  a.w = vT_.p; a.wb = (long)128 * ldN; a.ldw = ldN; a.N = 128; a.nimg = B;
  conv_dispatch<MODE_TAP>(a, EpiAggregate{gamma_, mf, (long)N * XLD, XLD, x_.p + 256, (long)N * XLD, XLD}, st);
  mark(ST_AGG, st);
  pr("aggregator.out", true, x_.p + 256, n8, 128, XLD);

  for (int p = 0; p < 2; ++p) {
    const float* hin = h_[p].p;
    float* hout = h_[p ^ 1].p;
    const int ph = p ? 2 : 0, pw = p ? 0 : 2;
    ConvShape g = conv_shape(gru_zr_[p], hin, 128, (long)N * 128, B, H8, W8, 1, ph, pw);
    g.C0 = 128; g.src1 = x_.p; g.ld1 = XLD; g.sb1 = (long)N * XLD; g.C1 = XLD;
    conv_dispatch<MODE_TAP>(g, EpiGruZR{gru_zr_[p].b, hin, z_.p, rh_.p, (long)N * 128}, st);
    mark(p ? ST_GRU_ZR_V : ST_GRU_ZR, st);
    pr(p ? "gru.z2" : "gru.z1", false, z_.p, n8, 128, 128);
    pr(p ? "gru.rh2" : "gru.rh1", true, rh_.p, n8, 128, 128);
    g.src0 = rh_.p; g.w = gru_q_[p].w; g.ldw = gru_q_[p].ldw; g.N = gru_q_[p].N;
    conv_dispatch<MODE_TAP>(g, EpiGruQ{gru_q_[p].b, hin, z_.p, hout, (long)N * 128}, st);
    mark(p ? ST_GRU_Q_V : ST_GRU_Q, st);
    pr(p ? "gru.h2" : "gru.h1", true, hout, n8, 128, 128);
  }

  s = conv_shape(fh1_, h_[0].p, 128, (long)N * 128, B, H8, W8, 1, 1, 1);
  conv_dispatch<MODE_TAP>(s, EpiBias<ACT_RELU>{fh1_.b, fh_.p, (long)N * 256, 256, 1.f}, st);
  pr("flow_head.conv1", true, fh_.p, n8, 256, 256);
  s = conv_shape(fh2_, fh_.p, 256, (long)N * 256, B, H8, W8, 1, 1, 1);
  conv_dispatch<MODE_TAP>(s, EpiFlowDelta{fh2_.b, coords1_.p, flow4_.p, x_.p + 254, XLD, (long)N * XLD, W8, (long)N}, st);
  mark(ST_FLOWHEAD, st);
  pr("flow", true, flow4_.p, n8, 2, 4);
  pr("coords1", false, coords1_.p, n8, 2, 2);
}

void GmaNet::run_body(int B, int iters, hipStream_t st) {
  float* f; int fh, fw;
  run_encoder(fnet_, true, 2 * B, st, &f, &fh, &fw);
  ATDN_CHECK(fh == H8 && fw == W8, "encoder geometry mismatch");
  ConvShape s = conv_shape(fnet_.head, f, 128, (long)N * 128, 2 * B, H8, W8, 1, 0, 0);
  conv_dispatch<MODE_TAP>(s, EpiBias<ACT_NONE>{fnet_.head.b, fmap_.p, (long)N * 256, 256, 1.f}, st);
  mark(ST_FNET, st);
  auto pr = [&](const char* name, bool limited, const float* p, long rows, long cols, long ld) {
    if (probe_) probe(name, limited, p, rows, cols, ld, st);
  };
  pr("fnet.conv2", true, fmap_.p, 2L * B * N, 256, 256);

  ConvShape c;
  c.src0 = fmap_.p; c.ld0 = 256; c.sb0 = (long)N * 256; c.C0 = 256; c.H = 1; c.W = N;
  c.w = fmap_.p + (long)B * N * 256; c.wb = (long)N * 256; c.ldw = 256; c.N = N; c.nimg = B;
  conv_dispatch<MODE_TAP>(c, EpiScale{1.0f / sqrtf(256.0f), pyr_[0].p, (long)N * N, N}, st);
  mark(ST_CORR, st);
  pr("corr.0", false, pyr_[0].p, (long)B * N, N, N);
  for (int l = 1; l < 4; ++l) {
    launch_avgpool(pyr_[l - 1].p, pyrH_[l - 1], pyrW_[l - 1], pyr_[l].p, (long)B * N, st);
    if (probe_) probe("corr." + std::to_string(l), false, pyr_[l].p, (long)B * N, (long)pyrH_[l] * pyrW_[l], (long)pyrH_[l] * pyrW_[l], st);
  }
  mark(ST_POOL, st);

  run_encoder(cnet_, false, B, st, &f, &fh, &fw);
  s = conv_shape(cnet_.head, f, 128, (long)N * 128, B, H8, W8, 1, 0, 0);
  conv_dispatch<MODE_TAP>(s, EpiContextSplit{cnet_.head.b, h_[0].p, (long)N * 128, x_.p, (long)N * XLD, XLD}, st);
  mark(ST_CNET, st);
  pr("net0", true, h_[0].p, (long)B * N, 128, 128);
  pr("inp", true, x_.p, (long)B * N, 128, XLD);

  s = conv_shape(to_qk_, x_.p, XLD, (long)N * XLD, B, H8, W8, 1, 0, 0);
  conv_dispatch<MODE_TAP>(s, EpiQK{1.0f / sqrtf(128.0f), 128, qk_.p, (long)N * 256, 256}, st);
  pr("att.qk", true, qk_.p, (long)B * N, 256, 256);
  ConvShape q;
  q.src0 = qk_.p; q.ld0 = 256; q.sb0 = (long)N * 256; q.C0 = 128; q.H = 1; q.W = N;
  q.w = qk_.p + 128; q.wb = (long)N * 256; q.ldw = 256; q.N = N; q.nimg = B;
  conv_dispatch<MODE_TAP>(q, EpiScale{1.0f, attn_.p, (long)N * ldN, ldN}, st);
  mark(ST_ATTN_LOGITS, st);
  pr("att.logits", false, attn_.p, (long)B * N, N, ldN);
  launch_softmax_rows(attn_.p, (long)B * N, N, ldN, st);
  mark(ST_ATTN, st);
  pr("att.attn", false, attn_.p, (long)B * N, N, ldN);

  for (int it = 0; it < iters; ++it) {
    probe_it_ = it;
    iteration(B, st);
    if (preds_out_) {
      mask_head(B, st);
      launch_upsample(mask_.p, flow4_.p, B, H8, W8, nullptr, preds_out_ + it * preds_stride_, st);
      pr("flow_up", false, preds_out_ + it * preds_stride_, 1, preds_stride_, preds_stride_);
    }
  }
  probe_it_ = -1;
  if (!preds_out_) mask_head(B, st);
  mark(ST_MASK, st);
}

void GmaNet::mask_head(int B, hipStream_t st) {
  ConvShape s = conv_shape(mask0_, h_[0].p, 128, (long)N * 128, B, H8, W8, 1, 1, 1);
  conv_dispatch<MODE_TAP>(s, EpiBias<ACT_RELU>{mask0_.b, fh_.p, (long)N * 256, 256, 1.f}, st);
  if (probe_) probe("mask.0", true, fh_.p, (long)B * N, 256, 256, st);
  s = conv_shape(mask2_, fh_.p, 256, (long)N * 256, B, H8, W8, 1, 0, 0);
  conv_dispatch<MODE_TAP>(s, EpiBias<ACT_NONE>{mask2_.b, mask_.p, (long)N * 576, 576, 0.25f}, st);
  if (probe_) probe("mask", false, mask_.p, (long)B * N, 576, 576, st);
}

void GmaNet::run_encoder_sf(const EncoderWeights& E, bool instance, int nimg, hipStream_t st, float** out_buf, int first_img,
                            DeviceBuf* bufs) {
  const float* images = img4_.p + (long)first_img * H * W * 4;
  int h = conv_out(H, 7, 2, 3), w = conv_out(W, 7, 2, 3);
  DeviceBuf* eb = bufs ? bufs : enc_;
  float* X = eb[0].p; float* R = eb[1].p; float* Y = eb[2].p; float* O = eb[3].p;
  auto stats_sf = [&](const PackedConv& L, const float* src, int ld, int ih, int iw, int stride, int pad, float* dst,
                      int slot, int in_slot = -1) {
    ConvShape s = conv_shape(L, src, ld, (long)ih * iw * ld, nimg, ih, iw, stride, pad, pad);
    if (in_slot >= 0) { s.in_mean = mean_[in_slot].p; s.in_rstd = rstd_[in_slot].p; }
    const int oh = conv_out(ih, L.KH, stride, pad), ow = conv_out(iw, L.KW, stride, pad);
    EpiBiasStats ep{L.b, dst, (long)oh * ow * L.N, L.N, psum_.p, pm2_.p, 0, pcnt_.p};
    TileChoice t = conv_sf_dispatch(s, L.wscale, ep, st);
    const int groups = t.groups_per_img;
    ATDN_CHECK((long)nimg * groups * L.N <= psum_.n && (long)nimg * groups <= pcnt_.n, "statistics scratch too small");
    if (t.counted)
      launch_in_finalize_cnt(psum_.p, pm2_.p, pcnt_.p, nimg, groups, oh * ow, L.N, 1e-5f, mean_[slot].p,
                             rstd_[slot].p, reinterpret_cast<double*>(fin_.p), st);
    else
      launch_in_finalize_cnt(psum_.p, pm2_.p, nullptr, nimg, groups, oh * ow, L.N, 1e-5f, mean_[slot].p, rstd_[slot].p,
                             reinterpret_cast<double*>(fin_.p), st);
  };
  const bool stem_raw = instance && norm_on_load_;
  if (stem_raw) {
    const int groups = stem_sf_groups(h, w);
    ATDN_CHECK((long)nimg * groups * 64 <= psum_.n && (long)nimg * groups <= pcnt_.n, "statistics scratch too small");
    launch_stem_sf(3, images, nimg, H, W, E.stem.wf, E.stem.wscale, E.stem.b, X, psum_.p, pm2_.p, pcnt_.p, nullptr, nullptr, st);
    launch_in_finalize_cnt(psum_.p, pm2_.p, pcnt_.p, nimg, groups, h * w, 64, 1e-5f, mean_[2].p, rstd_[2].p,
                           reinterpret_cast<double*>(fin_.p), st);
  } else if (instance) {
    const int groups = stem_sf_groups(h, w);
    ATDN_CHECK((long)nimg * groups * 64 <= psum_.n && (long)nimg * groups <= pcnt_.n, "statistics scratch too small");
    launch_stem_sf(1, images, nimg, H, W, E.stem.wf, E.stem.wscale, E.stem.b, nullptr, psum_.p, pm2_.p, pcnt_.p, nullptr,
                   nullptr, st);
    launch_in_finalize_cnt(psum_.p, pm2_.p, pcnt_.p, nimg, groups, h * w, 64, 1e-5f, mean_[0].p, rstd_[0].p,
                           reinterpret_cast<double*>(fin_.p), st);
    launch_stem_sf(2, images, nimg, H, W, E.stem.wf, E.stem.wscale, E.stem.b, X, nullptr, nullptr, nullptr, mean_[0].p,
                   rstd_[0].p, st);
  } else {
    launch_stem_sf(0, images, nimg, H, W, E.stem.wf, E.stem.wscale, E.stem.b, X, nullptr, nullptr, nullptr, nullptr,
                   nullptr, st);
  }
  int c = 64;
  for (int bi = 0; bi < 6; ++bi) {
    const auto& Bk = E.blk[bi];
    const int stride = Bk.has_ds ? 2 : 1;
    const int co = Bk.c1.N;
    const int oh = conv_out(h, 3, stride, 1), ow = conv_out(w, 3, stride, 1);
    const long ohw = (long)oh * ow;
    if (instance && norm_on_load_) {
      const bool raw_in = stem_raw && bi == 0;
      ATDN_CHECK(!raw_in || !Bk.has_ds, "the block behind the stem has no downsample branch");
      stats_sf(Bk.c1, X, c, h, w, stride, 1, R, 0, raw_in ? 2 : -1);
      stats_sf(Bk.c2, R, co, oh, ow, 1, 1, Y, 1, 0);
      if (Bk.has_ds) {
        stats_sf(Bk.ds, X, c, h, w, 2, 0, R, 0);
        launch_in_apply_sf(Y, O, mean_[1].p, rstd_[1].p, nullptr, R, mean_[0].p, rstd_[0].p, nimg, ohw, co, st);
      } else if (raw_in) {
        launch_in_apply_sf(Y, O, mean_[1].p, rstd_[1].p, nullptr, X, mean_[2].p, rstd_[2].p, nimg, ohw, co, st, true);
      } else {
        launch_in_apply_sf(Y, O, mean_[1].p, rstd_[1].p, X, nullptr, nullptr, nullptr, nimg, ohw, co, st);
      }
    } else if (instance) {
      stats_sf(Bk.c1, X, c, h, w, stride, 1, R, 0);
      launch_in_apply_sf(R, Y, mean_[0].p, rstd_[0].p, nullptr, nullptr, nullptr, nullptr, nimg, ohw, co, st);
      stats_sf(Bk.c2, Y, co, oh, ow, 1, 1, R, 0);
      if (Bk.has_ds) {
        stats_sf(Bk.ds, X, c, h, w, 2, 0, Y, 1);
        launch_in_apply_sf(R, O, mean_[0].p, rstd_[0].p, nullptr, Y, mean_[1].p, rstd_[1].p, nimg, ohw, co, st);
      } else {
        launch_in_apply_sf(R, O, mean_[0].p, rstd_[0].p, X, nullptr, nullptr, nullptr, nimg, ohw, co, st);
      }
    } else {
      const float* res = X;
      if (Bk.has_ds) {
        ConvShape sd = conv_shape(Bk.ds, X, c, (long)h * w * c, nimg, h, w, 2, 0, 0);
        conv_sf_dispatch(sd, Bk.ds.wscale, SfBias<ACT_NONE>{Bk.ds.b, R, ohw * co, co}, st);
        res = R;
      }
      ConvShape s1 = conv_shape(Bk.c1, X, c, (long)h * w * c, nimg, h, w, stride, 1, 1);
      conv_sf_dispatch(s1, Bk.c1.wscale, SfBias<ACT_RELU>{Bk.c1.b, Y, ohw * co, co}, st);
      ConvShape s2 = conv_shape(Bk.c2, Y, co, ohw * co, nimg, oh, ow, 1, 1, 1);
      conv_sf_dispatch(s2, Bk.c2.wscale, SfBiasReluAddRelu{Bk.c2.b, res, ohw * co, co, O, ohw * co, co}, st);
    }
    std::swap(X, O);
    h = oh; w = ow; c = co;
  }
  ATDN_CHECK(h == H8 && w == W8, "encoder geometry mismatch");
  *out_buf = X;
}

void GmaNet::iteration_sf(int B, hipStream_t st) {
  const long n8 = (long)B * N;
  ConvShape s;
  if (par_) fork(st, par_stream_);
  launch_lookup_conv(brick_pyramid(), coords1_.p, n8, coords_used_.p, convc1_.wf16, convc1_.wscale, convc1_.b, cor1_.p,
                     sf_fast_mode(), st);
  mark(ST_LOOKUP, st);
  s = conv_shape(convc2_, cor1_.p, 256, (long)N * 256, B, H8, W8, 1, 1, 1);
  const ConvShape sf2 = conv_shape(convf2_, flo1_.p, 128, (long)N * 128, B, H8, W8, 1, 1, 1);
  if (par_) {
    launch_flow_conv7_sf(flow4_.p, B, H8, W8, arena_.dev(convf1_sf_off_), convf1_wscale_, convf1_.b, flo1_.p, sf_fast_mode(), par_stream_);
    conv_sf_dispatch(sf2, convf2_.wscale, SfBias<ACT_RELU>{convf2_.b, corflo_.p + 192, (long)N * 256, 256}, par_stream_);
    conv_sf_dispatch(s, convc2_.wscale, SfBias<ACT_RELU>{convc2_.b, corflo_.p, (long)N * 256, 256}, st);
    fork(par_stream_, st);
  } else {
    launch_flow_conv7_sf(flow4_.p, B, H8, W8, arena_.dev(convf1_sf_off_), convf1_wscale_, convf1_.b, flo1_.p, sf_fast_mode(), st);
    conv_sf_dispatch_pair(s, convc2_.wscale, SfBias<ACT_RELU>{convc2_.b, corflo_.p, (long)N * 256, 256},
                          sf2, convf2_.wscale, SfBias<ACT_RELU>{convf2_.b, corflo_.p + 192, (long)N * 256, 256}, st);
  }
  s = conv_shape(convm_, corflo_.p, 256, (long)N * 256, B, H8, W8, 1, 1, 1);
  float* mf = x_.p + 128;
  conv_sf_dispatch(s, convm_.wscale, SfBias<ACT_RELU>{convm_.b, mf, (long)N * XLD, XLD}, st);
  mark(ST_MOTION, st);

  launch_attn_v(attn_.p, rinv_.p, attn_geom(B, N, ldN), nullptr, nullptr, mf, x_.p + 256, (long)N * XLD, XLD,
                sf_fast_mode(), st, attn_part_.p);
  mark(ST_AGG, st);

  for (int p = 0; p < 2; ++p) {
    const float* hin = h_[p].p;
    float* hout = h_[p ^ 1].p;
    const int ph = p ? 2 : 0, pw = p ? 0 : 2;
    ConvShape g = conv_shape(gru_zr_[p], hin, 128, (long)N * 128, B, H8, W8, 1, ph, pw);
    g.C0 = 128; g.src1 = x_.p + 128; g.ld1 = XLD; g.sb1 = (long)N * XLD; g.C1 = 256;
    conv_sf_dispatch(g, gru_zr_[p].wscale,
                     SfGruZR{gru_zr_[p].b, hin, z_.p, rh_.p, (long)N * 128, pre_zr_[p].p, (long)N * 256}, st);
    mark(p ? ST_GRU_ZR_V : ST_GRU_ZR, st);
    g.src0 = rh_.p; g.w = gru_q_[p].w; g.wfrag16 = gru_q_[p].wf16; g.ldw = gru_q_[p].ldw; g.N = gru_q_[p].N;
    conv_sf_dispatch(g, gru_q_[p].wscale, SfGruQ{gru_q_[p].b, hin, z_.p, hout, (long)N * 128, pre_q_[p].p}, st);
    mark(p ? ST_GRU_Q_V : ST_GRU_Q, st);
  }

  s = conv_shape(fh1_, h_[0].p, 128, (long)N * 128, B, H8, W8, 1, 1, 1);
  const SfFlowDelta fd{fh2_.b, coords1_.p, flow4_.p, x_.p, XLD, (long)N * XLD, 254, W8, (long)N};
  const long fh_gs = (long)maxB * N * 18;
  launch_flow_head_fused(s, fh1_.wscale, SfFlowHeadPartial{fh1_.b, arena_.dev(fh2_w32_off_), fhG_.p, (long)N, fh2_mul_, 1.0f / fh2_mul_, fh_gs}, st);
  launch_flow_gather(fhG_.p, fh_gs, B, H8, W8, fd, st);
  mark(ST_FLOWHEAD, st);
}

void GmaNet::run_body_sf(int B, int iters, hipStream_t st) {
  float* f;
  const int nfeat = seq_ == 0 ? 2 * B : seq_ == 1 ? B + 1 : B;
  hipStream_t sB = par_ ? par_stream_ : st;
  if (par_) fork(st, sB);
  run_encoder_sf(fnet_, true, nfeat, st, &f, seq_ == 2 ? 1 : 0);
  ConvShape s = conv_shape(fnet_.head, f, 128, (long)N * 128, nfeat, H8, W8, 1, 0, 0);
  float* fdst = fmap_.p + (seq_ == 2 ? (long)N * 256 : 0);
  conv_sf_dispatch(s, fnet_.head.wscale, SfBias<ACT_NONE>{fnet_.head.b, fdst, (long)N * 256, 256}, st);
  mark(ST_FNET, st);

  const float* target = fmap_.p + (long)(seq_ ? 1 : B) * N * 256;
  for (int l = 0; l < 4; ++l) {
    const float* plain = target;
    long plain_sb = (long)N * 256;
    if (l > 0) {
      const float* prev = l == 1 ? target : fplain_[l - 2].p;
      const long prev_sb = l == 1 ? (long)N * 256 : (long)pyrH_[l - 1] * pyrW_[l - 1] * 256;
      plain_sb = (long)pyrH_[l] * pyrW_[l] * 256;
      launch_pool_features_sf(prev, B, pyrH_[l - 1], pyrW_[l - 1], 256, prev_sb, fplain_[l - 1].p, plain_sb, st);
      plain = fplain_[l - 1].p;
    }
    launch_brick_rows(plain, plain_sb, B, pyrH_[l], pyrW_[l], 256, fbrick_[l].p, (long)brickNB_[l] * 256, st);
    launch_corr_bricks(fmap_.p, (long)N * 256, fbrick_[l].p, (long)brickNB_[l] * 256, B, N, brickNB_[l], 1.0f / sqrtf(256.0f), pyr_[l].p,
                       sf_fast_mode(), st);
    if (l == 0) mark(ST_CORR, st);
  }
  mark(ST_POOL, st);

  run_encoder_sf(cnet_, false, B, sB, &f, 0, par_ ? enc2_ : nullptr);
  s = conv_shape(cnet_.head, f, 128, (long)N * 128, B, H8, W8, 1, 0, 0);
  conv_sf_dispatch(s, cnet_.head.wscale,
                   SfContextSplit{cnet_.head.b, h_[0].p, (long)N * 128, x_.p, (long)N * XLD, XLD}, sB);
  mark(ST_CNET, st);

  s = conv_shape(to_qk_, x_.p, XLD, (long)N * XLD, B, H8, W8, 1, 0, 0);
  conv_sf_dispatch(s, to_qk_.wscale, SfQK{1.0f / sqrtf(128.0f), 128, qk_.p, (long)N * 256, 256}, sB);
  {
    const AttnGeom ag = attn_geom(B, N, ldN);
    launch_qk_rowmax(qk_.p, ag, rowmax_.p, sB);
    mark(ST_ATTN_LOGITS, st);
    launch_qk_softmax(qk_.p, ag, rowmax_.p, attn_.p, rinv_.p, sf_fast_mode(), sB);
  }
  mark(ST_ATTN, st);

  for (int p = 0; p < 2; ++p) {
    const int ph = p ? 2 : 0, pw = p ? 0 : 2;
    ConvShape g = conv_shape(gru_zr_ctx_[p], x_.p, XLD, (long)N * XLD, B, H8, W8, 1, ph, pw);
    conv_sf_dispatch(g, gru_zr_ctx_[p].wscale, EpiBias<ACT_NONE>{nullptr, pre_zr_[p].p, (long)N * 256, 256, 1.f}, sB);
    g = conv_shape(gru_q_ctx_[p], x_.p, XLD, (long)N * XLD, B, H8, W8, 1, ph, pw);
    conv_sf_dispatch(g, gru_q_ctx_[p].wscale, EpiBias<ACT_NONE>{nullptr, pre_q_[p].p, (long)N * 128, 128, 1.f}, sB);
  }
  mark(ST_GRU_CTX, st);
  if (par_) fork(sB, st);

  for (int it = 0; it < iters; ++it) {
    iteration_sf(B, st);
    if (preds_out_) {
      mask_head_sf(B, st);
      launch_upsample(mask_.p, flow4_.p, B, H8, W8, nullptr, preds_out_ + it * preds_stride_, st);
    }
  }
  if (!preds_out_) mask_head_sf(B, st);
  mark(ST_MASK, st);
}

void GmaNet::mask_head_sf(int B, hipStream_t st) {
  ConvShape s = conv_shape(mask0_, h_[0].p, 128, (long)N * 128, B, H8, W8, 1, 1, 1);
  conv_sf_dispatch(s, mask0_.wscale, SfBias<ACT_RELU>{mask0_.b, fh_.p, (long)N * 256, 256}, st);
  s = conv_shape(mask2_, fh_.p, 256, (long)N * 256, B, H8, W8, 1, 0, 0);
  conv_sf_dispatch(s, mask2_.wscale, EpiBias<ACT_NONE>{mask2_.b, mask_.p, (long)N * 576, 576, 0.25f}, st);
}

void GmaNet::capture(int B, int iters) {
  const bool want_par = low_latency_ && precision >= 1 && B <= 2 && par_stream_ != nullptr && !preds_out_ && par_ok_;
  for (int attempt = want_par ? 0 : 1; attempt < 2; ++attempt) {
    hipGraph_t graph = nullptr;
    hipGraphExec_t exec = nullptr;
    ATDN_HIP(hipStreamBeginCapture(cap_stream_, hipStreamCaptureModeThreadLocal));
    par_ = attempt == 0;
    par_next_ = 0;
    try {
      if (precision >= 1) { FastGuard fg(precision == 2); run_body_sf(B, iters, cap_stream_); } else run_body(B, iters, cap_stream_);
      par_ = false;
      ATDN_HIP(hipStreamEndCapture(cap_stream_, &graph));
      ATDN_HIP(hipGraphInstantiate(&exec, graph, nullptr, nullptr, 0));
    } catch (...) {
      const bool was_par = par_ || attempt == 0;
      par_ = false;
      hipGraph_t g2 = nullptr;
      (void)hipStreamEndCapture(cap_stream_, &g2);
      if (g2) (void)hipGraphDestroy(g2);
      if (graph) (void)hipGraphDestroy(graph);
      (void)hipGetLastError();
      if (attempt == 0 && was_par) {
        fprintf(stderr, "atdn: the flow graph could not be captured with parallel branches; capturing it as one chain\n");
        par_ok_ = false;
        continue;
      }
      throw;
    }
    (void)hipGraphDestroy(graph);
    graphs_[{B, iters * 4 + seq_}] = exec;
    return;
  }
}

void GmaNet::forward_sequence(const float* frames, int B, int iters, const float* flow_init, float* flow_low,
                               float* flow_up, hipStream_t st, bool continued) {
  ATDN_CHECK(ready_, "weights not finalized");
  ATDN_CHECK(precision >= 1, "sequence mode is built for the split-f16 pipeline");
  ATDN_CHECK(B >= 1 && B <= maxB, "batch exceeds max_batch of this handle");
  ATDN_CHECK(iters >= 1 && iters <= 64, "iters out of range");
  ATDN_CHECK(frames && flow_low && flow_up, "null tensor");
  const long frame = 3L * H * W;
  if (continued) {
    ATDN_CHECK(last_frame_ >= 1, "continued sequence call without a previous sequence call on this handle");
    ATDN_HIP(hipMemcpyAsync(fmap_.p, fmap_.p + (long)last_frame_ * N * 256, (size_t)N * 256 * sizeof(float),
                            hipMemcpyDeviceToDevice, st));
    seq_ = 2;
  } else {
    seq_ = 1;
  }
  last_frame_ = 0;
  launch_prep_images(frames, frames + (long)B * frame, B, H, W, img4_.p, st, 1);
  launch_init_coords_sf(flow_init, B, H8, W8, coords1_.p, flow4_.p, x_.p, XLD, 254, st);
  launch_body(B, iters, st);
  launch_upsample(mask_.p, flow4_.p, B, H8, W8, flow_low, flow_up, st);
  last_frame_ = B;
}

void GmaNet::launch_body(int B, int iters, hipStream_t st) {
  last_B_ = B;
  if (use_graph_ && !probe_) {
    auto key = std::make_pair(B, iters * 4 + seq_);
    if (!graphs_.count(key)) capture(B, iters);
    ATDN_HIP(hipGraphLaunch(graphs_[key], st));
  } else {
    if (precision >= 1) { FastGuard fg(precision == 2); run_body_sf(B, iters, st); } else run_body(B, iters, st);
  }
}

void GmaNet::forward(const float* im1, const float* im2, int B, int iters, const float* flow_init, float* flow_low,
                     float* flow_up, hipStream_t st) {
  ATDN_CHECK(ready_, "weights not finalized");
  ATDN_CHECK(B >= 1 && B <= maxB, "batch exceeds max_batch of this handle");
  ATDN_CHECK(iters >= 1 && iters <= 64, "iters out of range");
  ATDN_CHECK(im1 && im2 && flow_low && flow_up, "null tensor");
  seq_ = 0;
  last_frame_ = 0;
  if (probe_) probe_begin(st);
  launch_prep_images(im1, im2, B, H, W, img4_.p, st, B);
  if (precision >= 1) launch_init_coords_sf(flow_init, B, H8, W8, coords1_.p, flow4_.p, x_.p, XLD, 254, st);
  else launch_init_coords(flow_init, B, H8, W8, coords1_.p, flow4_.p, x_.p + 254, XLD, st);
  if (probe_) {
    probe("image", true, img4_.p, 2L * B * H * W, 3, 4, st);
    probe("flow_init", true, flow4_.p, (long)B * N, 2, 4, st);
  }
  launch_body(B, iters, st);
  launch_upsample(mask_.p, flow4_.p, B, H8, W8, flow_low, flow_up, st);
  if (probe_) {
    probe("flow_low", false, flow_low, 1, 2L * B * N, 2L * B * N, st);
    probe("flow_up", false, flow_up, 1, 2L * B * H * W, 2L * B * H * W, st);
    probe_end(st);
  }
}

void GmaNet::forward_predictions(const float* im1, const float* im2, int B, int iters, const float* flow_init, float* preds,
                                 hipStream_t st) {
  ATDN_CHECK(ready_, "weights not finalized");
  ATDN_CHECK(B >= 1 && B <= maxB, "batch exceeds max_batch of this handle");
  ATDN_CHECK(iters >= 1 && iters <= 64, "iters out of range");
  ATDN_CHECK(im1 && im2 && preds, "null tensor");
  seq_ = 0;
  last_frame_ = 0;
  last_B_ = B;
  if (probe_) probe_begin(st);
  launch_prep_images(im1, im2, B, H, W, img4_.p, st, B);
  if (precision >= 1) launch_init_coords_sf(flow_init, B, H8, W8, coords1_.p, flow4_.p, x_.p, XLD, 254, st);
  else launch_init_coords(flow_init, B, H8, W8, coords1_.p, flow4_.p, x_.p + 254, XLD, st);
  if (probe_) {
    probe("image", true, img4_.p, 2L * B * H * W, 3, 4, st);
    probe("flow_init", true, flow4_.p, (long)B * N, 2, 4, st);
  }
  struct Guard {
    GmaNet* n; ~Guard() { n->preds_out_ = nullptr; n->preds_stride_ = 0; }
  } guard{this};
  preds_out_ = preds;
  preds_stride_ = (long)B * 2 * H * W;
  if (precision >= 1) { FastGuard fg(precision == 2); run_body_sf(B, iters, st); } else run_body(B, iters, st);
  if (probe_) probe_end(st);
}

BrickPyramid GmaNet::brick_pyramid() const {
  BrickPyramid bp;
  for (int l = 0; l < 4; ++l) {
    bp.base[l] = pyr_[l].p; bp.H[l] = pyrH_[l]; bp.W[l] = pyrW_[l];
    bp.BW[l] = brickBW_[l]; bp.BH[l] = brickBH_[l]; bp.NB[l] = brickNB_[l];
  }
  bp.N = N; bp.NPB = brick_pixel_blocks(N);
  return bp;
}

long GmaNet::debug_read(const char* name, float* host, long capacity, hipStream_t st) {
  const std::string k(name);
  if (!classic_ && k.size() == 4 && k.compare(0, 3, "pyr") == 0 && k[3] >= '0' && k[3] <= '3') {
    const int l = k[3] - '0';
    const long rows = (long)maxB * N, total = rows * pyrH_[l] * pyrW_[l];
    scratch_.reserve(total);
    launch_unbrick(pyr_[l].p, brickNB_[l], N, pyrH_[l], pyrW_[l], rows, scratch_.p, st);
    ATDN_HIP(hipStreamSynchronize(st));
    const long n = std::min(capacity, total);
    ATDN_HIP(hipMemcpy(host, scratch_.p, (size_t)n * sizeof(float), hipMemcpyDeviceToHost));
    return n;
  }
  if (!classic_ && k == "corrfeat") {
    launch_lookup_bricks(brick_pyramid(), coords_used_.p, (long)(last_B_ > 0 ? last_B_ : maxB) * N, corrfeat_.p, st);
  }
  if (k == "sf_clamped") {
    ATDN_CHECK(capacity >= 1, "sf_clamped needs room for one float");
    host[0] = (float)sf_counter_read_reset(st);
    return 1;
  }
  const DeviceBuf* b = nullptr;
  if (k == "fmap") b = &fmap_; else if (k == "pyr0") b = &pyr_[0]; else if (k == "pyr1") b = &pyr_[1];
  else if (k == "pyr2") b = &pyr_[2]; else if (k == "pyr3") b = &pyr_[3]; else if (k == "net") b = &h_[0];
  else if (k == "x") b = &x_; else if (k == "attn") b = &attn_; else if (k == "corrfeat") b = &corrfeat_;
  else if (k == "mask") b = &mask_; else if (k == "coords1") b = &coords1_; else if (k == "flow4") b = &flow4_;
  else if (k == "qk") b = &qk_; else if (k == "img4") b = &img4_;
  else if (k == "cor1") b = &cor1_;
  if (k == "agg") {
    if (classic_) return -1;
    scratch_.reserve(x_.n);
    launch_from_sf(x_.p, scratch_.p, x_.n / 32, 32, st);
    ATDN_HIP(hipStreamSynchronize(st));
    const long rows = std::min(capacity / 128, (long)maxB * N);
    if (rows > 0)
      ATDN_HIP(hipMemcpy2D(host, 128 * sizeof(float), scratch_.p + 256, XLD * sizeof(float), 128 * sizeof(float), (size_t)rows,
                           hipMemcpyDeviceToHost));
    return rows * 128;
  }
  if (!b) return -1;
  long n = std::min(capacity, b->n);
  if (k == "attn" && !classic_) {
    const long rows = (long)maxB * N * ldN;
    scratch_.reserve(rows);
    ATDN_HIP(hipMemsetAsync(scratch_.p, 0, (size_t)rows * sizeof(float), st));
    launch_attn_decode(attn_.p, rinv_.p, attn_geom(maxB, N, ldN), scratch_.p, st);
    ATDN_HIP(hipStreamSynchronize(st));
    n = std::min(capacity, rows);
    ATDN_HIP(hipMemcpy(host, scratch_.p, (size_t)n * sizeof(float), hipMemcpyDeviceToHost));
    return n;
  }
  const bool is_sf = precision >= 1 && (k == "fmap" || k == "net" || k == "x" || k == "attn" || k == "corrfeat" || k == "qk" || k == "cor1");
  const float* src = b->p;
  if (is_sf) {
    scratch_.reserve(b->n);
    launch_from_sf(b->p, scratch_.p, b->n / 32, 32, st);
    src = scratch_.p;
    if (k == "x")
      launch_mfg_reconstruct(scratch_.p, (long)maxB * N, XLD, 128, 256, arena_.dev(to_v_w32_off_), gamma_, coords_used_.p, N, W8, 254, st);
  }
  ATDN_HIP(hipStreamSynchronize(st));
  ATDN_HIP(hipMemcpy(host, src, (size_t)n * sizeof(float), hipMemcpyDeviceToHost));
  return n;
}

}
```

### atdn_vslam_amd/csrc/kernels.h

```cpp
#pragma once
#include "common.h"

namespace atdn {

bool& sf_fast_mode();

struct PyramidLevels {
  const float* base[4];
  int H[4], W[4];
};

void launch_prep_images(const float* im1, const float* im2, int B, int H, int W, float* img4, hipStream_t st, int n2);

int stem_sf_groups(int Ho, int Wo);
void launch_stem_sf(int mode, const float* img4, int nimg, int H, int W, const float* wfrag, float wscale,
                    const float* bias, float* out_sf, float* part_sum, float* part_m2, float* part_cnt,
                    const float* mean, const float* rstd, hipStream_t st);

void launch_in_finalize_cnt(const float* part_sum, const float* part_m2, const float* part_cnt, int nimg,
                            int groups_per_img, int HW, int C, float eps, float* mean, float* rstd, double* scratch,
                            hipStream_t st);
void launch_in_apply(float* x, const float* mean, const float* rstd, const float* res, const float* rmean,
                     const float* rrstd, int nimg, long HW, int C, hipStream_t st);

void launch_avgpool(const float* src, int H, int W, float* dst, long rows, hipStream_t st);

void launch_lookup(const PyramidLevels& pyr, const float* coords1, long npix_total, float* out, int ldo,
                   hipStream_t st);

void launch_softmax_rows(float* x, long rows, int n, int ld, hipStream_t st);

void launch_init_coords(const float* flow_init, int B, int H8, int W8, float* coords1, float* flow4, float* xflow,
                        int ldx, hipStream_t st);

void launch_upsample(const float* mask, const float* flow4, int B, int H8, int W8, float* flow_low, float* flow_up,
                     hipStream_t st);

void launch_prep_flow(const float* flow, int B, int H, int W, const float* dw_w, const float* dw_b, float* out4,
                      hipStream_t st);
void launch_prep_rgb(const float* images, int B, int H, int W, float* out4, hipStream_t st);
void launch_linear(const float* W0, const float* x0, int K0, int ldx0, const float* W1, const float* x1, int K1,
                   int ldx1, const float* b0, const float* b1, int act, float* y, int ldy, int N, int B,
                   hipStream_t st);
struct LstmPipeArgs {
  int Hd, B, do1, do_lin, do2;
  const float *pre1, *Whh1, *bhh1, *h1_in; float *c1, *h1_out;
  const float *Wlin, *blin, *lin_in; float* lin_out;
  const float *Wih2, *bih2, *Whh2, *bhh2, *x2_in, *h2_in; float *c2, *h2_out;
};
void launch_lstm_pipe(const LstmPipeArgs& a, hipStream_t st);
long lstm_scan_exchange_bytes();
bool lstm_scan_fits_device();
void launch_lstm_scan(const float* pre1, const float* Whh1, const float* bhh1, const float* Wlin, const float* blin,
                      const float* Wih2, const float* bih2, const float* Whh2, const float* bhh2, float* state, float* h2seq,
                      void* exchange, int T, hipStream_t st);
struct MlpHead { const float *w0, *b0, *w1, *b1, *w2; };
void launch_mlp_heads(const float* h2, int B, MlpHead rot, MlpHead tr, float* rot_out, float* tr_out, hipStream_t st);

void launch_to_sf(const float* src, float* dst, long rows, int C, hipStream_t st);
void launch_from_sf(const float* src, float* dst, long rows, int C, hipStream_t st);
void launch_mfg_reconstruct(float* x, long rows, int ld, int cmf, int cagg, const float* wv, const float* gamma,
                            const float* coords_used, int N, int W8, int cflow, hipStream_t st);
void launch_in_apply_sf(const float* x, float* y, const float* mean, const float* rstd, const float* res,
                        const float* res_raw, const float* rmean, const float* rrstd, int nimg, long HW, int C,
                        hipStream_t st, bool res_relu = false);
void launch_pool_features_sf(const float* src, int nimg, int H, int W, int C, long sb, float* dst, long db, hipStream_t st);
void launch_init_coords_sf(const float* flow_init, int B, int H8, int W8, float* coords1, float* flow4, float* x,
                           int ldx, int cflow, hipStream_t st);

void launch_fill(float* p, long n, float v, hipStream_t st);

constexpr int kBrickPixelBlock = 64;
struct BrickPyramid {
  const float* base[4];
  int H[4], W[4], BW[4], BH[4], NB[4];
  int N;
  int NPB;
};
inline int brick_pixel_blocks(int N) { return 2 * ((N + 127) / 128); }
void launch_brick_rows(const float* src, long sb, int nimg, int H, int W, int C, float* dst, long db, hipStream_t st);
void launch_corr_bricks(const float* f1, long sb1, const float* f2b, long sb2, int B, int N, int NB, float scale, float* out,
                        bool fast, hipStream_t st);
void launch_unbrick(const float* src, long NB, int N, int H, int W, long npix, float* dst, hipStream_t st);
void launch_lookup_conv(const BrickPyramid& pyr, const float* coords1, long npix, float* coords_used, const float* wfrag,
                        float wscale, const float* bias, float* out, bool fast, hipStream_t st);
void launch_lookup_bricks(const BrickPyramid& pyr, const float* coords1, long npix, float* out, hipStream_t st);

}
```

### atdn_vslam_amd/csrc/kernels.hip

```cpp
#include "kernels.h"
#include "sf.h"

namespace atdn {

bool& sf_fast_mode() {
  static thread_local bool fast = false;
  return fast;
}

__device__ __forceinline__ float wave_sum(float v) {
#pragma unroll
  for (int o = 32; o > 0; o >>= 1) v += __shfl_xor(v, o);
  return v;
}
__device__ __forceinline__ float wave_max(float v) {
#pragma unroll
  for (int o = 32; o > 0; o >>= 1) v = fmaxf(v, __shfl_xor(v, o));
  return v;
}
template <bool MAX>
__device__ __forceinline__ float block_reduce(float v, float* sm) {
  v = MAX ? wave_max(v) : wave_sum(v);
  __syncthreads();
  if ((threadIdx.x & 63) == 0) sm[threadIdx.x >> 6] = v;
  __syncthreads();
  const float a = sm[0], b = sm[1], c = sm[2], d = sm[3];
  return MAX ? fmaxf(fmaxf(a, b), fmaxf(c, d)) : ((a + b) + (c + d));
}

__global__ void prep_images_kernel(const float* __restrict__ im1, const float* __restrict__ im2, int B, int n2, long HW,
                                   float4* __restrict__ out) {
  const long i = (long)blockIdx.x * blockDim.x + threadIdx.x;
  if (i >= (long)(B + n2) * HW) return;
  const long img = i / HW, p = i - img * HW;
  const float* src = (img < B ? im1 + img * 3 * HW : im2 + (img - B) * 3 * HW) + p;
  float4 v;
  v.x = 2.f * (src[0] / 255.0f) - 1.0f;
  v.y = 2.f * (src[HW] / 255.0f) - 1.0f;
  v.z = 2.f * (src[2 * HW] / 255.0f) - 1.0f;
  v.w = 0.f;
  out[i] = v;
}
void launch_prep_images(const float* im1, const float* im2, int B, int H, int W, float* img4, hipStream_t st, int n2) {
  const long n = (long)(B + n2) * H * W;
  hipLaunchKernelGGL(prep_images_kernel, dim3((unsigned)cdivl(n, 256)), dim3(256), 0, st, im1, im2, B, n2, (long)H * W,
                     reinterpret_cast<float4*>(img4));
  ATDN_HIP(hipGetLastError());
}

constexpr int FIN_SPLIT = 32;
__global__ __launch_bounds__(1024) void in_finalize_cnt_kernel(const float* __restrict__ ps,
                                                               const float* __restrict__ pm2,
                                                               const float* __restrict__ pc, int groups, int C,
                                                               int HW, double* __restrict__ part) {
  __shared__ double s_n[16][64], s_s1[16][64], s_sq[16][64], s_m2[16][64];
  const int img = blockIdx.y, z = blockIdx.z, lane = threadIdx.x & 63, wv = threadIdx.x >> 6;
  const int c = blockIdx.x * 64 + lane;
  const int per = (groups + FIN_SPLIT - 1) / FIN_SPLIT;
  const int g0 = z * per, g1 = min(groups, g0 + per);
  double n = 0.0, s1 = 0.0, sq = 0.0, m2 = 0.0;
  if (c < C) {
    const float* s = ps + (long)img * groups * C + c;
    const float* m = pm2 + (long)img * groups * C + c;
    const float* cn = pc ? pc + (long)img * groups : nullptr;
#pragma unroll 8
    for (int g = g0 + wv; g < g1; g += 16) {
      const float cnt = cn ? cn[g] : (float)max(0, min(32, HW - g * 32));
      if (cnt > 0.f) {
        const double sg = (double)s[(long)g * C];
        n += (double)cnt;
        s1 += sg;
        sq += sg * sg * (cnt == 32.f ? 0.03125 : 1.0 / (double)cnt);
        m2 += (double)m[(long)g * C];
      }
    }
  }
  s_n[wv][lane] = n; s_s1[wv][lane] = s1; s_sq[wv][lane] = sq; s_m2[wv][lane] = m2;
  __syncthreads();
  if (wv == 0 && c < C) {
    n = 0.0; s1 = 0.0; sq = 0.0; m2 = 0.0;
    for (int k = 0; k < 16; ++k) { n += s_n[k][lane]; s1 += s_s1[k][lane]; sq += s_sq[k][lane]; m2 += s_m2[k][lane]; }
    double* o = part + (((long)img * FIN_SPLIT + z) * C + c) * 4;
    o[0] = n; o[1] = s1; o[2] = sq; o[3] = m2;
  }
}
__global__ void in_finalize_merge_kernel(const double* __restrict__ part, int nimg, int HW, int C, float eps,
                                         float* __restrict__ mean, float* __restrict__ rstd) {
  const int i = blockIdx.x * blockDim.x + threadIdx.x;
  if (i >= nimg * C) return;
  const int img = i / C, c = i - img * C;
  double n = 0.0, s1 = 0.0, sq = 0.0, m2 = 0.0;
  for (int z = 0; z < FIN_SPLIT; ++z) {
    const double* p = part + (((long)img * FIN_SPLIT + z) * C + c) * 4;
    n += p[0]; s1 += p[1]; sq += p[2]; m2 += p[3];
  }
  const double mu = n > 0.0 ? s1 / n : 0.0;
  const double between = n > 0.0 ? fmax(sq - s1 * s1 / n, 0.0) : 0.0;
  const float mu_f = (float)mu, rs_f = (float)(1.0 / sqrt((m2 + between) / (double)HW + (double)eps));
  mean[i] = mu_f;
  rstd[i] = rs_f;
  sf_report(!(fabsf(mu_f) <= 3.0e38f) | !(rs_f <= 3.0e38f));
}
void launch_in_finalize_cnt(const float* part_sum, const float* part_m2, const float* part_cnt, int nimg,
                            int groups_per_img, int HW, int C, float eps, float* mean, float* rstd, double* scratch,
                            hipStream_t st) {
  hipLaunchKernelGGL(in_finalize_cnt_kernel, dim3(cdiv(C, 64), nimg, FIN_SPLIT), dim3(1024), 0, st, part_sum, part_m2,
                     part_cnt, groups_per_img, C, HW, scratch);
  ATDN_HIP(hipGetLastError());
  hipLaunchKernelGGL(in_finalize_merge_kernel, dim3(cdiv(nimg * C, 128)), dim3(128), 0, st, scratch, nimg, HW, C, eps,
                     mean, rstd);
  ATDN_HIP(hipGetLastError());
}

__global__ void in_apply_kernel(float4* __restrict__ x, const float* __restrict__ mean, const float* __restrict__ rstd,
                                const float4* __restrict__ res, const float* __restrict__ rmean,
                                const float* __restrict__ rrstd, long per_img4, int C, long total4) {
  for (long i = (long)blockIdx.x * blockDim.x + threadIdx.x; i < total4; i += (long)gridDim.x * blockDim.x) {
    const long img = i / per_img4;
    const int c = (int)((i * 4) % C);
    const float* mu = mean + img * C + c;
    const float* rs = rstd + img * C + c;
    float4 v = x[i];
    v.x = fmaxf((v.x - mu[0]) * rs[0], 0.f);
    v.y = fmaxf((v.y - mu[1]) * rs[1], 0.f);
    v.z = fmaxf((v.z - mu[2]) * rs[2], 0.f);
    v.w = fmaxf((v.w - mu[3]) * rs[3], 0.f);
    if (res) {
      float4 r = res[i];
      if (rmean) {
        const float* m2 = rmean + img * C + c;
        const float* r2 = rrstd + img * C + c;
        r.x = (r.x - m2[0]) * r2[0]; r.y = (r.y - m2[1]) * r2[1];
        r.z = (r.z - m2[2]) * r2[2]; r.w = (r.w - m2[3]) * r2[3];
      }
      v.x = fmaxf(r.x + v.x, 0.f); v.y = fmaxf(r.y + v.y, 0.f);
      v.z = fmaxf(r.z + v.z, 0.f); v.w = fmaxf(r.w + v.w, 0.f);
    }
    x[i] = v;
  }
}
void launch_in_apply(float* x, const float* mean, const float* rstd, const float* res, const float* rmean,
                     const float* rrstd, int nimg, long HW, int C, hipStream_t st) {
  ATDN_CHECK(C % 4 == 0, "in_apply needs C % 4 == 0");
  const long per_img4 = HW * C / 4, total4 = per_img4 * nimg;
  const int grid = (int)std::min<long>(cdivl(total4, 256), 256 * 16);
  hipLaunchKernelGGL(in_apply_kernel, dim3(grid), dim3(256), 0, st, reinterpret_cast<float4*>(x), mean, rstd,
                     reinterpret_cast<const float4*>(res), rmean, rrstd, per_img4, C, total4);
  ATDN_HIP(hipGetLastError());
}

__global__ void avgpool_kernel(const float* __restrict__ src, int H, int W, int Ho, int Wo, float* __restrict__ dst,
                               long total) {
  for (long i = (long)blockIdx.x * blockDim.x + threadIdx.x; i < total; i += (long)gridDim.x * blockDim.x) {
    const long row = i / (Ho * Wo);
    const int rem = (int)(i - row * (Ho * Wo));
    const int y = rem / Wo, x = rem - y * Wo;
    const float* p = src + row * ((long)H * W) + (long)(2 * y) * W + 2 * x;
    dst[i] = (((p[0] + p[1]) + p[W]) + p[W + 1]) * 0.25f;
  }
}
void launch_avgpool(const float* src, int H, int W, float* dst, long rows, hipStream_t st) {
  const int Ho = H / 2, Wo = W / 2;
  const long total = rows * Ho * Wo;
  const int grid = (int)std::min<long>(cdivl(total, 256), 256 * 32);
  hipLaunchKernelGGL(avgpool_kernel, dim3(grid), dim3(256), 0, st, src, H, W, Ho, Wo, dst, total);
  ATDN_HIP(hipGetLastError());
}

constexpr int LK_WIN = 12;
__global__ __launch_bounds__(256) void lookup_kernel(const PyramidLevels pyr, const float* __restrict__ coords1,
                                                     long npix, float* __restrict__ out, int ldo) {
  __shared__ float win[4][LK_WIN * LK_WIN + 16];
  const int lvl = threadIdx.x >> 6, lane = threadIdx.x & 63;
  const int Hl = pyr.H[lvl], Wl = pyr.W[lvl];
  const float inv = 1.0f / (float)(1 << lvl);
  const float wm1 = (float)(Wl - 1), hm1 = (float)(Hl - 1);
  const float sfx = wm1 / 2.f, sfy = hm1 / 2.f;
  float* w = win[lvl];
  for (long p = blockIdx.x; p < npix; p += gridDim.x) {
    const float xc = coords1[p * 2 + 0] * inv, yc = coords1[p * 2 + 1] * inv;
    const bool sane = (fabsf(xc) < 1.0e6f) && (fabsf(yc) < 1.0e6f);
    const int wx0 = sane ? (int)floorf(xc) - 5 : -(1 << 24), wy0 = sane ? (int)floorf(yc) - 5 : -(1 << 24);
    const float* src = pyr.base[lvl] + p * ((long)Hl * Wl);
#pragma unroll
    for (int t = 0; t < 3; ++t) {
      const int c = lane + 64 * t;
      if (c < LK_WIN * LK_WIN) {
        const int wy = c / LK_WIN, wx = c - wy * LK_WIN;
        const int y = wy0 + wy, x = wx0 + wx;
        const bool ok = ((unsigned)y < (unsigned)Hl) & ((unsigned)x < (unsigned)Wl);
        w[c] = ok ? src[(long)y * Wl + x] : 0.f;
      }
    }
    __builtin_amdgcn_s_waitcnt(0);
    __builtin_amdgcn_wave_barrier();
    float* o = out + p * ldo + lvl * 81;
#pragma unroll
    for (int t = 0; t < 2; ++t) {
      const int k = lane + 64 * t;
      if (k < 81) {
        const int i = k / 9, j = k - i * 9;
        float v = 0.f;
        if (sane) {
          const float px = xc + (float)(i - 4), py = yc + (float)(j - 4);
          const float xg = 2.f * px / wm1 - 1.f, yg = 2.f * py / hm1 - 1.f;
          const float ix = (xg + 1.f) * sfx, iy = (yg + 1.f) * sfy;
          const float xw = floorf(ix), yn = floorf(iy);
          const float ww = ix - xw, ee = 1.f - ww, nn = iy - yn, ss = 1.f - nn;
          const int lx = min(max((int)xw - wx0, 0), LK_WIN - 2), ly = min(max((int)yn - wy0, 0), LK_WIN - 2);
          const float* q = w + ly * LK_WIN + lx;
          v = ((q[0] * (ee * ss) + q[1] * (ww * ss)) + q[LK_WIN] * (ee * nn)) + q[LK_WIN + 1] * (ww * nn);
        }
        o[k] = v;
      }
    }
    __builtin_amdgcn_wave_barrier();
  }
}
void launch_lookup(const PyramidLevels& pyr, const float* coords1, long npix_total, float* out, int ldo,
                   hipStream_t st) {
  ATDN_CHECK(ldo >= 324, "lookup output row too short");
  const int grid = (int)std::min<long>(npix_total, 256 * 16);
  hipLaunchKernelGGL(lookup_kernel, dim3(grid), dim3(256), 0, st, pyr, coords1, npix_total, out, ldo);
  ATDN_HIP(hipGetLastError());
}

__global__ __launch_bounds__(256) void softmax_rows_kernel(float* __restrict__ x, int n, int ld) {
  __shared__ float sm[4];
  float* row = x + (long)blockIdx.x * ld;
  float mx = -INFINITY;
  for (int i = threadIdx.x; i < n; i += 256) mx = fmaxf(mx, row[i]);
  mx = block_reduce<true>(mx, sm);
  float s = 0.f;
  for (int i = threadIdx.x; i < n; i += 256) {
    const float e = expf(row[i] - mx);
    row[i] = e;
    s += e;
  }
  s = block_reduce<false>(s, sm);
  for (int i = threadIdx.x; i < n; i += 256) row[i] = row[i] / s;
  for (int i = n + threadIdx.x; i < ld; i += 256) row[i] = 0.f;
}
void launch_softmax_rows(float* x, long rows, int n, int ld, hipStream_t st) {
  hipLaunchKernelGGL(softmax_rows_kernel, dim3((unsigned)rows), dim3(256), 0, st, x, n, ld);
  ATDN_HIP(hipGetLastError());
}

__global__ void init_coords_kernel(const float* __restrict__ flow_init, int B, int H8, int W8,
                                   float* __restrict__ coords1, float* __restrict__ flow4, float* __restrict__ xflow,
                                   int ldx) {
  const long N = (long)H8 * W8;
  const long i = (long)blockIdx.x * blockDim.x + threadIdx.x;
  if (i >= B * N) return;
  const long img = i / N;
  const int m = (int)(i - img * N);
  const float x0 = (float)(m % W8), y0 = (float)(m / W8);
  float fx = 0.f, fy = 0.f;
  if (flow_init) { fx = flow_init[(img * 2 + 0) * N + m]; fy = flow_init[(img * 2 + 1) * N + m]; }
  const float cx = x0 + fx, cy = y0 + fy;
  coords1[i * 2 + 0] = cx;
  coords1[i * 2 + 1] = cy;
  const float flx = cx - x0, fly = cy - y0;
  reinterpret_cast<float4*>(flow4)[i] = make_float4(flx, fly, 0.f, 0.f);
  xflow[i * ldx + 0] = flx;
  xflow[i * ldx + 1] = fly;
}
void launch_init_coords(const float* flow_init, int B, int H8, int W8, float* coords1, float* flow4, float* xflow,
                        int ldx, hipStream_t st) {
  const long n = (long)B * H8 * W8;
  hipLaunchKernelGGL(init_coords_kernel, dim3((unsigned)cdivl(n, 256)), dim3(256), 0, st, flow_init, B, H8, W8,
                     coords1, flow4, xflow, ldx);
  ATDN_HIP(hipGetLastError());
}

__global__ __launch_bounds__(256) void upsample_kernel(const float* __restrict__ mask, const float* __restrict__ flow4,
                                                       int B, int H8, int W8, float* __restrict__ flow_low,
                                                       float* __restrict__ flow_up) {
  const long N = (long)H8 * W8;
  const long p = (long)blockIdx.x * 4 + (threadIdx.x >> 6);
  if (p >= B * N) return;
  const int lane = threadIdx.x & 63;
  const long img = p / N;
  const int m = (int)(p - img * N);
  const int h = m / W8, w = m - h * W8;
  const float* mk = mask + p * 576 + lane;
  float e[9];
  float mx = -INFINITY;
#pragma unroll
  for (int k = 0; k < 9; ++k) { e[k] = mk[k * 64]; mx = fmaxf(mx, e[k]); }
  float s = 0.f;
#pragma unroll
  for (int k = 0; k < 9; ++k) { e[k] = __builtin_amdgcn_exp2f((e[k] - mx) * 1.4426950408889634f); s += e[k]; }
  const float rs = 1.0f / s;
  float ux = 0.f, uy = 0.f;
#pragma unroll
  for (int k = 0; k < 9; ++k) {
    const int yy = h + k / 3 - 1, xx = w + k % 3 - 1;
    float fx = 0.f, fy = 0.f;
    if ((unsigned)yy < (unsigned)H8 && (unsigned)xx < (unsigned)W8) {
      const float4 f = reinterpret_cast<const float4*>(flow4)[img * N + (long)yy * W8 + xx];
      fx = 8.f * f.x; fy = 8.f * f.y;
    }
    const float wk = e[k] * rs;
    ux += wk * fx;
    uy += wk * fy;
  }
  const int i = lane >> 3, j = lane & 7;
  const long Hf = 8L * H8, Wf = 8L * W8;
  const long o = (img * 2) * Hf * Wf + (long)(8 * h + i) * Wf + 8 * w + j;
  flow_up[o] = ux;
  flow_up[o + Hf * Wf] = uy;
  if (lane == 0 && flow_low) {
    const float4 f = reinterpret_cast<const float4*>(flow4)[p];
    flow_low[(img * 2 + 0) * N + m] = f.x;
    flow_low[(img * 2 + 1) * N + m] = f.y;
  }
}
void launch_upsample(const float* mask, const float* flow4, int B, int H8, int W8, float* flow_low, float* flow_up,
                     hipStream_t st) {
  const long n = (long)B * H8 * W8;
  hipLaunchKernelGGL(upsample_kernel, dim3((unsigned)cdivl(n, 4)), dim3(256), 0, st, mask, flow4, B, H8, W8, flow_low,
                     flow_up);
  ATDN_HIP(hipGetLastError());
}

__global__ void prep_flow_kernel(const float* __restrict__ flow, int B, long HW, float sx, float sy, const float* dw_w,
                                 const float* dw_b, float4* __restrict__ out) {
  const long i = (long)blockIdx.x * blockDim.x + threadIdx.x;
  if (i >= B * HW) return;
  const long img = i / HW, p = i - img * HW;
  const float* s = flow + img * 2 * HW + p;
  float4 v;
  v.x = (s[0] / sx) * dw_w[0] + dw_b[0];
  v.y = (s[HW] / sy) * dw_w[1] + dw_b[1];
  v.z = 0.f; v.w = 0.f;
  out[i] = v;
}
void launch_prep_flow(const float* flow, int B, int H, int W, const float* dw_w, const float* dw_b, float* out4,
                      hipStream_t st) {
  const long n = (long)B * H * W;
  hipLaunchKernelGGL(prep_flow_kernel, dim3((unsigned)cdivl(n, 256)), dim3(256), 0, st, flow, B, (long)H * W,
                     58.1837f, 17.7647f, dw_w, dw_b, reinterpret_cast<float4*>(out4));
  ATDN_HIP(hipGetLastError());
}

__global__ void prep_rgb_kernel(const float* __restrict__ img, int B, long HW, float4* __restrict__ out) {
  const long i = (long)blockIdx.x * blockDim.x + threadIdx.x;
  if (i >= B * HW) return;
  const long b = i / HW, p = i - b * HW;
  const float* s = img + b * 3 * HW + p;
  float4 v;
  v.x = ((s[0] / 255.0f) - 0.485f) / 0.229f;
  v.y = ((s[HW] / 255.0f) - 0.456f) / 0.224f;
  v.z = ((s[2 * HW] / 255.0f) - 0.406f) / 0.225f;
  v.w = 0.f;
  out[i] = v;
}
void launch_prep_rgb(const float* images, int B, int H, int W, float* out4, hipStream_t st) {
  const long n = (long)B * H * W;
  hipLaunchKernelGGL(prep_rgb_kernel, dim3((unsigned)cdivl(n, 256)), dim3(256), 0, st, images, B, (long)H * W,
                     reinterpret_cast<float4*>(out4));
  ATDN_HIP(hipGetLastError());
}

__global__ __launch_bounds__(256) void linear_kernel(const float* __restrict__ W0, const float* __restrict__ x0, int K0,
                                                     int ldx0, const float* __restrict__ W1,
                                                     const float* __restrict__ x1, int K1, int ldx1,
                                                     const float* __restrict__ b0, const float* __restrict__ b1,
                                                     int act, float* __restrict__ y, int ldy, int N, int B) {
  const int n = blockIdx.x * 4 + (threadIdx.x >> 6);
  if (n >= N) return;
  const int lane = threadIdx.x & 63;
  for (int b = 0; b < B; ++b) {
    float acc = 0.f;
    const float4* w = reinterpret_cast<const float4*>(W0 + (long)n * K0);
    const float4* x = reinterpret_cast<const float4*>(x0 + (long)b * ldx0);
    for (int k = lane; k < K0 / 4; k += 64) {
      const float4 a = w[k], v = x[k];
      acc += a.x * v.x + a.y * v.y + a.z * v.z + a.w * v.w;
    }
    if (W1) {
      const float4* w1 = reinterpret_cast<const float4*>(W1 + (long)n * K1);
      const float4* x1v = reinterpret_cast<const float4*>(x1 + (long)b * ldx1);
      for (int k = lane; k < K1 / 4; k += 64) {
        const float4 a = w1[k], v = x1v[k];
        acc += a.x * v.x + a.y * v.y + a.z * v.z + a.w * v.w;
      }
    }
    acc = wave_sum(acc);
    if (lane == 0) {
      float v = acc + (b0 ? b0[n] : 0.f) + (b1 ? b1[n] : 0.f);
      if (act == 1) v = mishf_(v);
      y[(long)b * ldy + n] = v;
    }
  }
}
void launch_linear(const float* W0, const float* x0, int K0, int ldx0, const float* W1, const float* x1, int K1,
                   int ldx1, const float* b0, const float* b1, int act, float* y, int ldy, int N, int B,
                   hipStream_t st) {
  ATDN_CHECK(K0 % 4 == 0 && K1 % 4 == 0 && ldx0 % 4 == 0 && ldx1 % 4 == 0, "linear: K and ld must be multiples of 4");
  hipLaunchKernelGGL(linear_kernel, dim3(cdiv(N, 4)), dim3(256), 0, st, W0, x0, K0, ldx0, W1, x1, K1, ldx1, b0, b1, act,
                     y, ldy, N, B);
  ATDN_HIP(hipGetLastError());
}

__global__ __launch_bounds__(256) void lstm_pipe_kernel(const LstmPipeArgs a) {
  __shared__ float gate[4];
  const int Hd = a.Hd, lane = threadIdx.x & 63, wv = threadIdx.x >> 6;
  auto dot = [&](const float* __restrict__ wrow, const float* __restrict__ x) {
    float acc = 0.f;
    for (int k = lane; k < Hd / 4; k += 64) {
      const float4 w = reinterpret_cast<const float4*>(wrow)[k];
      const float4 v = reinterpret_cast<const float4*>(x)[k];
      acc += w.x * v.x + w.y * v.y + w.z * v.z + w.w * v.w;
    }
    return wave_sum(acc);
  };
  int blk = blockIdx.x;
  if (blk < Hd) {
    if (!a.do1) return;
    const int j = blk;
    for (int b = 0; b < a.B; ++b) {
      const float acc = dot(a.Whh1 + ((long)wv * Hd + j) * Hd, a.h1_in + (long)b * Hd);
      if (lane == 0) gate[wv] = a.pre1[(long)b * 4 * Hd + wv * Hd + j] + (acc + a.bhh1[wv * Hd + j]);
      __syncthreads();
      if (threadIdx.x == 0) {
        const float cn = sigmoidf_(gate[1]) * a.c1[(long)b * Hd + j] + sigmoidf_(gate[0]) * tanhf(gate[2]);
        a.c1[(long)b * Hd + j] = cn;
        a.h1_out[(long)b * Hd + j] = sigmoidf_(gate[3]) * tanhf(cn);
      }
      __syncthreads();
    }
    return;
  }
  blk -= Hd;
  if (blk < Hd / 4) {
    if (!a.do_lin) return;
    const int j = blk * 4 + wv;
    for (int b = 0; b < a.B; ++b) {
      const float acc = dot(a.Wlin + (long)j * Hd, a.lin_in + (long)b * Hd);
      if (lane == 0) a.lin_out[(long)b * Hd + j] = mishf_(acc + a.blin[j]);
    }
    return;
  }
  blk -= Hd / 4;
  if (!a.do2) return;
  const int j = blk;
  for (int b = 0; b < a.B; ++b) {
    const float ax = dot(a.Wih2 + ((long)wv * Hd + j) * Hd, a.x2_in + (long)b * Hd);
    const float ah = dot(a.Whh2 + ((long)wv * Hd + j) * Hd, a.h2_in + (long)b * Hd);
    if (lane == 0) gate[wv] = (ax + a.bih2[wv * Hd + j]) + (ah + a.bhh2[wv * Hd + j]);
    __syncthreads();
    if (threadIdx.x == 0) {
      const float cn = sigmoidf_(gate[1]) * a.c2[(long)b * Hd + j] + sigmoidf_(gate[0]) * tanhf(gate[2]);
      a.c2[(long)b * Hd + j] = cn;
      a.h2_out[(long)b * Hd + j] = sigmoidf_(gate[3]) * tanhf(cn);
    }
    __syncthreads();
  }
}
void launch_lstm_pipe(const LstmPipeArgs& a, hipStream_t st) {
  ATDN_CHECK(a.Hd % 16 == 0 && a.B >= 1, "lstm_pipe: bad arguments");
  hipLaunchKernelGGL(lstm_pipe_kernel, dim3(2 * a.Hd + a.Hd / 4), dim3(256), 0, st, a);
  ATDN_HIP(hipGetLastError());
}

__global__ __launch_bounds__(256) void mlp_heads_kernel(const float* __restrict__ h2, MlpHead rot, MlpHead tr,
                                                        float* __restrict__ rot_out, float* __restrict__ tr_out) {
  __shared__ float x[512];
  __shared__ float a1[2][128];
  __shared__ float a2[2][64];
  const int b = blockIdx.x, t = threadIdx.x;
  x[t] = h2[(long)b * 512 + t];
  x[t + 256] = h2[(long)b * 512 + 256 + t];
  __syncthreads();
  const int hd = t >> 7, u = t & 127;
  const MlpHead& H = hd ? tr : rot;
  {
    const float* w = H.w0 + (long)u * 512;
    float acc = 0.f;
    for (int k = 0; k < 512; ++k) acc += w[k] * x[k];
    a1[hd][u] = mishf_(acc + H.b0[u]);
  }
  __syncthreads();
  if (u < 64) {
    const float* w = H.w1 + (long)u * 128;
    float acc = 0.f;
    for (int k = 0; k < 128; ++k) acc += w[k] * a1[hd][k];
    a2[hd][u] = mishf_(acc + H.b1[u]);
  }
  __syncthreads();
  if (u < 3) {
    const float* w = H.w2 + (long)u * 64;
    float acc = 0.f;
    for (int k = 0; k < 64; ++k) acc += w[k] * a2[hd][k];
    (hd ? tr_out : rot_out)[(long)b * 3 + u] = acc;
  }
}
void launch_mlp_heads(const float* h2, int B, MlpHead rot, MlpHead tr, float* rot_out, float* tr_out, hipStream_t st) {
  hipLaunchKernelGGL(mlp_heads_kernel, dim3(B), dim3(256), 0, st, h2, rot, tr, rot_out, tr_out);
  ATDN_HIP(hipGetLastError());
}

const float* zero_line() {
  static float* z = nullptr;
  if (!z) {
    ATDN_HIP(hipMalloc(&z, 256));
    ATDN_HIP(hipMemset(z, 0, 256));
    ATDN_HIP(hipDeviceSynchronize());
  }
  return z;
}

__global__ void fill_kernel(float* p, long n, float v) {
  for (long i = (long)blockIdx.x * blockDim.x + threadIdx.x; i < n; i += (long)gridDim.x * blockDim.x) p[i] = v;
}
void launch_fill(float* p, long n, float v, hipStream_t st) {
  if (n <= 0) return;
  hipLaunchKernelGGL(fill_kernel, dim3((unsigned)std::min<long>(cdivl(n, 256), 4096)), dim3(256), 0, st, p, n, v);
  ATDN_HIP(hipGetLastError());
}

}

#include "sf.h"
#include <mutex>
#include <vector>
namespace atdn {

namespace {
std::vector<void (*)(unsigned int*)>& sf_counter_setters() { static std::vector<void (*)(unsigned int*)> v; return v; }
std::mutex g_sf_counter_mutex;
struct SfCounterDev { int dev; unsigned int* ptr; };
std::vector<SfCounterDev> g_sf_counters;
unsigned int* sf_counter_for_current_device(bool create) {
  int dev = 0;
  ATDN_HIP(hipGetDevice(&dev));
  for (auto& c : g_sf_counters) if (c.dev == dev) return c.ptr;
  if (!create) return nullptr;
  unsigned int* p = nullptr;
  ATDN_HIP(hipMalloc(&p, 2 * sizeof(unsigned int)));
  ATDN_HIP(hipMemset(p, 0, 2 * sizeof(unsigned int)));
  for (auto set : sf_counter_setters()) {
    set(p);
    ATDN_HIP(hipGetLastError());
  }
  ATDN_HIP(hipDeviceSynchronize());
  g_sf_counters.push_back({dev, p});
  return p;
}
}
void sf_counter_register(void (*setter)(unsigned int*)) { sf_counter_setters().push_back(setter); }
void sf_counter_attach() {
  std::lock_guard<std::mutex> lock(g_sf_counter_mutex);
  (void)sf_counter_for_current_device(true);
}
__global__ void sf_counter_exchange_kernel(unsigned int* counter, unsigned int* out) { *out = atomicExch(counter, 0u); }
unsigned int sf_counter_read_reset(hipStream_t st) {
  std::lock_guard<std::mutex> lock(g_sf_counter_mutex);
  unsigned int* p = sf_counter_for_current_device(true);
  unsigned int* slot = p + 1;
  unsigned int v = 0;
  hipLaunchKernelGGL(sf_counter_exchange_kernel, dim3(1), dim3(1), 0, st, p, slot);
  ATDN_HIP(hipGetLastError());
  ATDN_HIP(hipMemcpyAsync(&v, slot, sizeof(v), hipMemcpyDeviceToHost, st));
  ATDN_HIP(hipStreamSynchronize(st));
  return v;
}

__device__ __forceinline__ void sf_store4(float* dst, long i4, float4 v) {
  const long grp = i4 >> 3;
  const int sl = (int)(i4 & 7);
  _Float16* g = reinterpret_cast<_Float16*>(dst + grp * 32) + sl * 4;
  const SfPair a = sf_split(v.x), b = sf_split(v.y), c = sf_split(v.z), d = sf_split(v.w);
  typedef _Float16 h4 __attribute__((ext_vector_type(4)));
  h4 hi = {a.hi, b.hi, c.hi, d.hi};
  h4 lo = {a.lo, b.lo, c.lo, d.lo};
  *reinterpret_cast<h4*>(g) = hi;
  *reinterpret_cast<h4*>(g + 32) = lo;
}
__device__ __forceinline__ float4 sf_load4(const float* src, long i4) {
  const long grp = i4 >> 3;
  const int sl = (int)(i4 & 7);
  const _Float16* g = reinterpret_cast<const _Float16*>(src + grp * 32) + sl * 4;
  typedef _Float16 h4 __attribute__((ext_vector_type(4)));
  const h4 hi = *reinterpret_cast<const h4*>(g);
  const h4 lo = *reinterpret_cast<const h4*>(g + 32);
  return make_float4((float)hi[0] + (float)lo[0], (float)hi[1] + (float)lo[1], (float)hi[2] + (float)lo[2],
                     (float)hi[3] + (float)lo[3]);
}

__global__ void to_sf_kernel(const float4* __restrict__ src, float* __restrict__ dst, long total4) {
  for (long i = (long)blockIdx.x * blockDim.x + threadIdx.x; i < total4; i += (long)gridDim.x * blockDim.x)
    sf_store4(dst, i, src[i]);
}
void launch_to_sf(const float* src, float* dst, long rows, int C, hipStream_t st) {
  ATDN_CHECK(C % 32 == 0, "sf tensors need C % 32 == 0");
  const long total4 = rows * C / 4;
  hipLaunchKernelGGL(to_sf_kernel, dim3((unsigned)std::min<long>(cdivl(total4, 256), 4096)), dim3(256), 0, st,
                     reinterpret_cast<const float4*>(src), dst, total4);
  ATDN_HIP(hipGetLastError());
}
__global__ void from_sf_kernel(const float* __restrict__ src, float4* __restrict__ dst, long total4) {
  for (long i = (long)blockIdx.x * blockDim.x + threadIdx.x; i < total4; i += (long)gridDim.x * blockDim.x)
    dst[i] = sf_load4(src, i);
}
void launch_from_sf(const float* src, float* dst, long rows, int C, hipStream_t st) {
  ATDN_CHECK(C % 32 == 0, "sf tensors need C % 32 == 0");
  const long total4 = rows * C / 4;
  hipLaunchKernelGGL(from_sf_kernel, dim3((unsigned)std::min<long>(cdivl(total4, 256), 4096)), dim3(256), 0, st, src,
                     reinterpret_cast<float4*>(dst), total4);
  ATDN_HIP(hipGetLastError());
}

__global__ __launch_bounds__(128) void mfg_reconstruct_kernel(float* __restrict__ x, int ld, int cmf, int cagg,
                                                              const float* __restrict__ wv, const float* __restrict__ gamma,
                                                              const float* __restrict__ coords_used, int N, int W8, int cflow) {
  __shared__ float a[128];
  const long pix = blockIdx.x;
  float* row = x + pix * ld;
  const int c = threadIdx.x;
  a[c] = row[cagg + c];
  __syncthreads();
  float s = 0.f;
  for (int k = 0; k < 128; ++k) s = fmaf(wv[c * 128 + k], a[k], s);
  float m = row[cmf + c];
  const int n = cmf + c - cflow;
  if (coords_used && (n == 0 || n == 1)) {
    const int p = (int)(pix % N);
    const float f = coords_used[pix * 2 + n] - (n == 0 ? (float)(p % W8) : (float)(p / W8));
    const _Float16 hi = (_Float16)f;
    m = (float)hi + (float)(_Float16)(f - (float)hi);
  }
  row[cagg + c] = m + gamma[0] * s;
}

void launch_mfg_reconstruct(float* x, long rows, int ld, int cmf, int cagg, const float* wv, const float* gamma,
                            const float* coords_used, int N, int W8, int cflow, hipStream_t st) {
  if (rows <= 0) return;
  hipLaunchKernelGGL(mfg_reconstruct_kernel, dim3((unsigned)rows), dim3(128), 0, st, x, ld, cmf, cagg, wv, gamma, coords_used, N, W8, cflow);
  ATDN_HIP(hipGetLastError());
}

__global__ void in_apply_sf_kernel(const float4* __restrict__ x, float* __restrict__ y, const float* __restrict__ mean,
                                   const float* __restrict__ rstd, const float* __restrict__ res,
                                   const float4* __restrict__ res_raw, const float* __restrict__ rmean,
                                   const float* __restrict__ rrstd, int res_relu, long per_img4, int C, long total4) {
  for (long i = (long)blockIdx.x * blockDim.x + threadIdx.x; i < total4; i += (long)gridDim.x * blockDim.x) {
    const long img = i / per_img4;
    const int c = (int)((i * 4) % C);
    const float* mu = mean + img * C + c;
    const float* rs = rstd + img * C + c;
    float4 v = x[i];
    v.x = fmaxf((v.x - mu[0]) * rs[0], 0.f);
    v.y = fmaxf((v.y - mu[1]) * rs[1], 0.f);
    v.z = fmaxf((v.z - mu[2]) * rs[2], 0.f);
    v.w = fmaxf((v.w - mu[3]) * rs[3], 0.f);
    if (res || res_raw) {
      float4 r;
      if (res) {
        r = sf_load4(res, i);
      } else {
        r = res_raw[i];
        const float* m2 = rmean + img * C + c;
        const float* r2 = rrstd + img * C + c;
        r.x = (r.x - m2[0]) * r2[0]; r.y = (r.y - m2[1]) * r2[1];
        r.z = (r.z - m2[2]) * r2[2]; r.w = (r.w - m2[3]) * r2[3];
        if (res_relu) {
          r.x = fmaxf(r.x, 0.f); r.y = fmaxf(r.y, 0.f); r.z = fmaxf(r.z, 0.f); r.w = fmaxf(r.w, 0.f);
        }
      }
      v.x = fmaxf(r.x + v.x, 0.f); v.y = fmaxf(r.y + v.y, 0.f);
      v.z = fmaxf(r.z + v.z, 0.f); v.w = fmaxf(r.w + v.w, 0.f);
    }
    sf_store4(y, i, v);
  }
}
void launch_in_apply_sf(const float* x, float* y, const float* mean, const float* rstd, const float* res,
                        const float* res_raw, const float* rmean, const float* rrstd, int nimg, long HW, int C,
                        hipStream_t st, bool res_relu) {
  ATDN_CHECK(C % 32 == 0, "sf tensors need C % 32 == 0");
  const long per_img4 = HW * C / 4, total4 = per_img4 * nimg;
  const int grid = (int)std::min<long>(cdivl(total4, 256), 256 * 16);
  hipLaunchKernelGGL(in_apply_sf_kernel, dim3(grid), dim3(256), 0, st, reinterpret_cast<const float4*>(x), y, mean,
                     rstd, res, reinterpret_cast<const float4*>(res_raw), rmean, rrstd, res_relu ? 1 : 0, per_img4, C, total4);
  ATDN_HIP(hipGetLastError());
}

__global__ void pool_features_sf_kernel(const float* __restrict__ src, int H, int W, int C, long sb, float* __restrict__ dst,
                                        long db, long total) {
  const long i = (long)blockIdx.x * blockDim.x + threadIdx.x;
  if (i >= total) return;
  const int Ho = H / 2, Wo = W / 2, c4 = C / 4;
  const int cq = (int)(i % c4);
  const long pq = i / c4;
  const int po = (int)(pq % ((long)Ho * Wo));
  const long img = pq / ((long)Ho * Wo);
  const int y = po / Wo, x = po - y * Wo;
  const float* s = src + img * sb;
  const long p00 = ((long)(2 * y) * W + 2 * x) * C;
  const float4 a = sf_load4(s, p00, 4 * cq), b = sf_load4(s, p00 + C, 4 * cq);
  const float4 c = sf_load4(s, p00 + (long)W * C, 4 * cq), d = sf_load4(s, p00 + (long)W * C + C, 4 * cq);
  const float4 o = make_float4((((a.x + b.x) + c.x) + d.x) * 0.25f, (((a.y + b.y) + c.y) + d.y) * 0.25f,
                               (((a.z + b.z) + c.z) + d.z) * 0.25f, (((a.w + b.w) + c.w) + d.w) * 0.25f);
  sf_store4(dst + img * db, (long)po * C, 4 * cq, o);
}
void launch_pool_features_sf(const float* src, int nimg, int H, int W, int C, long sb, float* dst, long db, hipStream_t st) {
  ATDN_CHECK(C % 32 == 0, "sf tensors need C % 32 == 0");
  const long total = (long)nimg * (H / 2) * (W / 2) * (C / 4);
  hipLaunchKernelGGL(pool_features_sf_kernel, dim3((unsigned)cdivl(total, 256)), dim3(256), 0, st, src, H, W, C, sb, dst, db, total);
  ATDN_HIP(hipGetLastError());
}

__global__ void init_coords_sf_kernel(const float* __restrict__ flow_init, int B, int H8, int W8,
                                      float* __restrict__ coords1, float* __restrict__ flow4, float* __restrict__ x,
                                      int ldx, int cflow) {
  const long N = (long)H8 * W8;
  const long i = (long)blockIdx.x * blockDim.x + threadIdx.x;
  if (i >= B * N) return;
  const long img = i / N;
  const int m = (int)(i - img * N);
  const float x0 = (float)(m % W8), y0 = (float)(m / W8);
  float fx = 0.f, fy = 0.f;
  if (flow_init) { fx = flow_init[(img * 2 + 0) * N + m]; fy = flow_init[(img * 2 + 1) * N + m]; }
  const float cx = x0 + fx, cy = y0 + fy;
  coords1[i * 2 + 0] = cx;
  coords1[i * 2 + 1] = cy;
  const float flx = cx - x0, fly = cy - y0;
  reinterpret_cast<float4*>(flow4)[i] = make_float4(flx, fly, 0.f, 0.f);
  sf_store(x, i * ldx, cflow, flx);
  sf_store(x, i * ldx, cflow + 1, fly);
}
void launch_init_coords_sf(const float* flow_init, int B, int H8, int W8, float* coords1, float* flow4, float* x,
                           int ldx, int cflow, hipStream_t st) {
  const long n = (long)B * H8 * W8;
  hipLaunchKernelGGL(init_coords_sf_kernel, dim3((unsigned)cdivl(n, 256)), dim3(256), 0, st, flow_init, B, H8, W8,
                     coords1, flow4, x, ldx, cflow);
  ATDN_HIP(hipGetLastError());
}

}
```

### atdn_vslam_amd/csrc/lookup_fused.hip

```cpp
#include "conv_mfma.h"
#include "kernels.h"
#include "sf.h"

namespace atdn {
namespace {

typedef float v4f __attribute__((ext_vector_type(4)));

constexpr int LP = kBrickPixelBlock;
constexpr int TP = 32;
constexpr int NCH = 352;
constexpr int APITCH = 1504;
constexpr int ADUMP = 1408;
constexpr int GW = 24, GH = 24;
constexpr int DEPTH = 4;
constexpr int NWAVE = TP / 4;
constexpr int UPW = TP * 4 / NWAVE;


typedef unsigned int u32x4 __attribute__((ext_vector_type(4)));

template <bool FUSED, bool FAST>
__global__ __launch_bounds__(NWAVE * 64, TP == 32 ? 4 : 1) void lookup_conv_kernel(const BrickPyramid pyr, const float* __restrict__ coords1,
                                                            const long npix, float* __restrict__ coords_used,
                                                            const float* __restrict__ wfrag, const float wscale,
                                                            const float* __restrict__ bias, float* __restrict__ out) {
  __shared__ __attribute__((aligned(16))) char atile[TP * APITCH];
  __shared__ __attribute__((aligned(16))) float grid[NWAVE][GH * GW];

  const int tid = threadIdx.x, lane = tid & 63;
  const int wave = __builtin_amdgcn_readfirstlane(tid >> 6);
  static_assert(LP % TP == 0 && TP % 16 == 0 && TP <= 64, "a block of this kernel is a whole fraction of a pixel block");
  const int bpp = (pyr.N + TP - 1) / TP;
  const int pair = (int)blockIdx.x / bpp, kblk = (int)blockIdx.x - pair * bpp;
  const int pblk = (kblk * TP) / LP, poff = (kblk * TP) % LP;
  const long p0 = (long)pair * pyr.N + (long)kblk * TP;
  const int np = min(TP, pyr.N - kblk * TP);
  (void)npix;

  for (int i = tid; i < TP * 28; i += NWAVE * 64) {
    const int row = i / 28, c = 324 + (i - row * 28);
    _Float16* q = reinterpret_cast<_Float16*>(atile + row * APITCH + (c >> 5) * 128) + (c & 31);
    q[0] = (_Float16)0.f;
    q[32] = (_Float16)0.f;
  }

  static_assert(DEPTH % 4 == 0, "unit pi has level pi & 3 = (pi % DEPTH) & 3");
  const int pbase = wave * (UPW / 4);
  const long pc = p0 + min(lane, np - 1);
  const float2 cmine = *reinterpret_cast<const float2*>(coords1 + pc * 2);
  if (wave == 0 && lane < np && coords_used) *reinterpret_cast<float2*>(coords_used + (p0 + lane) * 2) = cmine;

  int P_m12, P_sb, P_gb;
  float P_w00, P_w01, P_w10, P_w11;
  {
#pragma clang fp contract(off)
    const int myu = lane & 15, lev = myu & 3;
    const int mypp = min(pbase + (myu >> 2), np - 1);
    const float cx = __shfl(cmine.x, mypp), cy = __shfl(cmine.y, mypp);
    const int Wl = lev == 0 ? pyr.W[0] : lev == 1 ? pyr.W[1] : lev == 2 ? pyr.W[2] : pyr.W[3];
    const int Hl = lev == 0 ? pyr.H[0] : lev == 1 ? pyr.H[1] : lev == 2 ? pyr.H[2] : pyr.H[3];
    const float inv = lev == 0 ? 1.0f : lev == 1 ? 0.5f : lev == 2 ? 0.25f : 0.125f;
    float xc = cx * inv, yc = cy * inv;
    const bool sane = (fabsf(xc) < 1.0e6f) && (fabsf(yc) < 1.0e6f);
    xc = sane ? xc : 0.f; yc = sane ? yc : 0.f;
    auto chain = [](float c0, float sz) __attribute__((always_inline)) {
      const float rs = 1.0f / sz, hs = sz / 2.f;
      const float t = 2.f * c0;
      float q = t * rs;
      q = __builtin_fmaf(__builtin_fmaf(-q, sz, t), rs, q);
      return ((q - 1.f) + 1.f) * hs;
    };
    const float ux = chain(xc, (float)(Wl - 1)), uy = chain(yc, (float)(Hl - 1));
    const float flx = floorf(ux), fly = floorf(uy);
    const float ww = ux - flx, nn = uy - fly, ee = 1.f - ww, ss = 1.f - nn;
    P_w00 = ee * ss; P_w01 = ww * ss; P_w10 = ee * nn; P_w11 = ww * nn;
    const int wx0 = sane ? (int)flx - 4 : -(1 << 24), wy0 = sane ? (int)fly - 4 : -(1 << 24);
    const int bx0 = wx0 >> 3, by0 = wy0 >> 2;
    P_gb = sane ? ((wy0 - 4 * by0) * GW + (wx0 - 8 * bx0)) * 4 : 0;
    const int BWl = lev == 0 ? pyr.BW[0] : lev == 1 ? pyr.BW[1] : lev == 2 ? pyr.BW[2] : pyr.BW[3];
    const int BHl = lev == 0 ? pyr.BH[0] : lev == 1 ? pyr.BH[1] : lev == 2 ? pyr.BH[2] : pyr.BH[3];
    const int nbx = (((wx0 & 7) + 9) >> 3) + 1, nby = (((wy0 & 3) + 9) >> 2) + 1;
    const int clo = max(0, -bx0), chi = max(min(nbx, BWl - bx0), clo);
    const int rlo = max(0, -by0), rhi = max(min(nby, BHl - by0), rlo);
    const unsigned cm = (1u << (chi & 31)) - (1u << (clo & 31));
    const unsigned rm = 0x249u & ((1u << ((3 * rhi) & 31)) - (1u << ((3 * rlo) & 31)));
    P_m12 = (int)((clo < 3 && rlo < 4) ? rm * cm : 0u);
    P_sb = (int)((unsigned)(by0 * BWl + bx0) * (unsigned)(LP * 128));
  }

  v4f bv[DEPTH][2];
  int bxi[2], byi[2];
#pragma unroll
  for (int k = 0; k < 2; ++k) { const int bi = 8 * k + (lane >> 3); byi[k] = bi / 3; bxi[k] = bi - 3 * byi[k]; }
  int loff[4][2];
#pragma unroll
  for (int l = 0; l < 4; ++l)
#pragma unroll
    for (int k = 0; k < 2; ++k) loff[l][k] = (byi[k] * pyr.BW[l] + bxi[k]) * (LP * 128) + (lane & 7) * 16;
  const int big = 0x7FFFFFF0;
  auto rep8 = [](unsigned m8) __attribute__((always_inline)) {
    unsigned long long r;
    asm("s_bitreplicate_b64_b32 %0, %1" : "=s"(r) : "s"(m8));
    asm("s_bitreplicate_b64_b32 %0, %1" : "=s"(r) : "s"((unsigned)r));
    asm("s_bitreplicate_b64_b32 %0, %1" : "=s"(r) : "s"((unsigned)r));
    return r;
  };
  auto issue = [&](int pi, int sl) __attribute__((always_inline)) {
    const int l = sl & 3;
    const int pp = min(pbase + (pi >> 2), np - 1);
    const unsigned m12 = (unsigned)__builtin_amdgcn_readlane(P_m12, pi);
    const int sbase = (int)((unsigned)__builtin_amdgcn_readlane(P_sb, pi) + (unsigned)((poff + pp) * 128));
    const unsigned long long lm0 = rep8(m12 & 0xFFu), lm1 = rep8(m12 >> 8);
    const long NBl = pyr.NB[l];
    const __amdgpu_buffer_rsrc_t rs = __builtin_amdgcn_make_buffer_rsrc(
        const_cast<float*>(pyr.base[l] + ((long)pair * pyr.NPB + pblk) * NBl * LP), 0, (int)(NBl * LP * 4), 0x00020000);
#pragma unroll
    for (int k = 0; k < 2; ++k) {
      int off;
      asm("v_cndmask_b32_e64 %0, %1, %2, %3" : "=v"(off) : "v"(big), "v"((int)((unsigned)loff[l][k] + (unsigned)sbase)), "s"(k == 0 ? lm0 : lm1));
      bv[sl][k] = __builtin_bit_cast(v4f, __builtin_amdgcn_raw_buffer_load_b128(rs, off, 0, 0));
    }
  };
#pragma unroll
  for (int d = 0; d < DEPTH - 1; ++d) issue(d, d);
  float* gw = grid[wave];
  int gofs[2], dofs[4][2], sofs[2];
#pragma unroll
  for (int k = 0; k < 2; ++k) {
    const int part = lane & 7;
    gofs[k] = (byi[k] * 4 + (part >> 1)) * GW + bxi[k] * 8 + (part & 1) * 4;
    const int i9 = k == 0 ? (lane & 7) : (lane < 9 ? 8 : (lane < 17 ? lane - 9 : 8));
    const int j9 = k == 0 ? (lane >> 3) : (lane < 9 ? lane : 8);
    sofs[k] = (j9 * GW + i9) * 4;
#pragma unroll
    for (int l = 0; l < 4; ++l) {
      const int c = l * 81 + i9 * 9 + j9;
      dofs[l][k] = (k == 0 || lane < 17) ? (c >> 5) * 128 + (c & 31) * 2 : ADUMP + (lane & 15) * 2;
    }
  }
  auto fence = [&]() __attribute__((always_inline)) {
    __builtin_amdgcn_fence(__ATOMIC_RELEASE, "wavefront");
    __builtin_amdgcn_wave_barrier();
    __builtin_amdgcn_fence(__ATOMIC_ACQUIRE, "wavefront");
  };
  static_assert(UPW % DEPTH == 0, "units per wave must be a multiple of the prefetch depth");
  float vmax = 0.f;
  for (int pi0 = 0; pi0 < UPW; pi0 += DEPTH) {
#pragma unroll
    for (int d = 0; d < DEPTH; ++d) {
      const int pi = pi0 + d;
      issue(pi + DEPTH - 1, (d + DEPTH - 1) % DEPTH);
#pragma unroll
      for (int k = 0; k < 2; ++k) *reinterpret_cast<v4f*>(gw + gofs[k]) = bv[d][k];
      fence();
      const float w00 = __int_as_float(__builtin_amdgcn_readlane(__float_as_int(P_w00), pi));
      const float w01 = __int_as_float(__builtin_amdgcn_readlane(__float_as_int(P_w01), pi));
      const float w10 = __int_as_float(__builtin_amdgcn_readlane(__float_as_int(P_w10), pi));
      const float w11 = __int_as_float(__builtin_amdgcn_readlane(__float_as_int(P_w11), pi));
      const char* q0 = reinterpret_cast<const char*>(gw) + __builtin_amdgcn_readlane(P_gb, pi);
      float q00[2], q01[2], q10[2], q11[2];
#pragma unroll
      for (int t = 0; t < 2; ++t) {
        const float* q = reinterpret_cast<const float*>(q0 + sofs[t]);
        q00[t] = q[0]; q01[t] = q[1]; q10[t] = q[GW]; q11[t] = q[GW + 1];
      }
      char* arow = atile + (pbase + (pi >> 2)) * APITCH;
      float va[2];
#pragma unroll
      for (int t = 0; t < 2; ++t) {
#pragma clang fp contract(off)
        const float v = __builtin_fmaf(q11[t], w11, __builtin_fmaf(q10[t], w10, __builtin_fmaf(q01[t], w01, q00[t] * w00)));
        va[t] = v;
        const float vc = __builtin_amdgcn_fmed3f(v, -65504.f, 65504.f);
        unsigned hi, lo;
        asm("v_cvt_f16_f32_e32 %0, %1" : "=v"(hi) : "v"(vc));
        asm("v_fma_mixlo_f16 %0, %1, -1.0, %2 op_sel_hi:[1,0,0]" : "=v"(lo) : "v"(hi), "v"(vc));
        unsigned short* dst = reinterpret_cast<unsigned short*>(arow + dofs[d & 3][t]);
        dst[0] = (unsigned short)hi;
        dst[32] = (unsigned short)lo;
      }
      vmax = fmaxf(fmaxf(fabsf(va[0]), fabsf(va[1])), vmax);
    }
  }
  const bool clamped = !(vmax <= 65504.f);
  sf_report(clamped);

  constexpr int NQ = NCH / 32;
  constexpr int WD = 4;
  constexpr int CB = 256 / 16 / NWAVE, PB = TP / 16;
  static_assert(CB * NWAVE * 16 == 256, "the block's waves cover convc1's 256 output channels");
  typedef float f32x4v __attribute__((ext_vector_type(4)));
  const int n16 = lane & 15, g16 = lane >> 4;
  const char* wbase = reinterpret_cast<const char*>(wfrag) + (long)(wave * CB) * NQ * 2048 + lane * 16;
  f16x8 wh[WD][CB], wl[WD][CB];
  auto load_w = [&](int slot, int q) __attribute__((always_inline)) {
#pragma unroll
    for (int cb = 0; cb < CB; ++cb) {
      const char* p = wbase + ((long)cb * NQ + q) * 2048;
      wh[slot][cb] = *reinterpret_cast<const f16x8*>(p);
      if (!FAST) wl[slot][cb] = *reinterpret_cast<const f16x8*>(p + 1024);
    }
  };
  if (FUSED) {
#pragma unroll
    for (int q = 0; q < WD; ++q) load_w(q, q);
  }
  __syncthreads();

  if (!FUSED) {
    for (int i = tid; i < np * 88; i += NWAVE * 64) {
      const int row = i / 88, part = i - row * 88;
      *reinterpret_cast<v4f*>(reinterpret_cast<char*>(out) + (p0 + row) * (NCH * 4L) + part * 16) =
          *reinterpret_cast<const v4f*>(atile + row * APITCH + part * 16);
    }
    return;
  }

  f32x4v acc[CB][PB];
#pragma unroll
  for (int cb = 0; cb < CB; ++cb)
#pragma unroll
    for (int pb = 0; pb < PB; ++pb)
#pragma unroll
      for (int e = 0; e < 4; ++e) acc[cb][pb][e] = 0.f;
  const char* arow = atile + n16 * APITCH + 16 * g16;
#pragma unroll
  for (int q = 0; q < NQ; ++q) {
#pragma unroll
    for (int pb = 0; pb < PB; ++pb) {
      const f16x8 ah = *reinterpret_cast<const f16x8*>(arow + 16 * pb * APITCH + q * 128);
      f16x8 al = ah;
      if (!FAST) al = *reinterpret_cast<const f16x8*>(arow + 16 * pb * APITCH + q * 128 + 64);
#pragma unroll
      for (int cb = 0; cb < CB; ++cb) {
        f32x4v c = acc[cb][pb];
        if (!FAST) {
          c = __builtin_amdgcn_mfma_f32_16x16x32_f16(wh[q % WD][cb], al, c, 0, 0, 0);
          c = __builtin_amdgcn_mfma_f32_16x16x32_f16(wl[q % WD][cb], ah, c, 0, 0, 0);
        }
        c = __builtin_amdgcn_mfma_f32_16x16x32_f16(wh[q % WD][cb], ah, c, 0, 0, 0);
        acc[cb][pb] = c;
      }
    }
    if (q + WD < NQ) load_w(q % WD, q + WD);
  }
#pragma unroll
  for (int cb = 0; cb < CB; ++cb) {
    const int c = 16 * (wave * CB + cb) + 4 * g16;
    const float4 b = *reinterpret_cast<const float4*>(bias + c);
#pragma unroll
    for (int pb = 0; pb < PB; ++pb) {
      const int px = 16 * pb + n16;
      if (px < np) {
        const float4 o = make_float4(fmaxf(acc[cb][pb][0] * wscale + b.x, 0.f), fmaxf(acc[cb][pb][1] * wscale + b.y, 0.f),
                                     fmaxf(acc[cb][pb][2] * wscale + b.z, 0.f), fmaxf(acc[cb][pb][3] * wscale + b.w, 0.f));
        sf_store4(out + (p0 + px) * 256, 0, c, o);
      }
    }
  }
}

__global__ void brick_rows_kernel(const float* __restrict__ src, long sb, int H, int W, int BW, int C,
                                  float* __restrict__ dst, long db, long total4) {
  const long i = (long)blockIdx.x * blockDim.x + threadIdx.x;
  if (i >= total4) return;
  const int c4 = C / 4;
  const int part = (int)(i % c4);
  const long row = i / c4;
  const long per_img = db / C;
  const long img = row / per_img;
  const int n = (int)(row - img * per_img);
  const int brick = n >> 5, within = n & 31;
  const int y = (brick / BW) * 4 + (within >> 3), x = (brick % BW) * 8 + (within & 7);
  v4f v = {0.f, 0.f, 0.f, 0.f};
  if (y < H && x < W) v = *reinterpret_cast<const v4f*>(src + img * sb + ((long)y * W + x) * C + part * 4);
  *reinterpret_cast<v4f*>(dst + img * db + (long)n * C + part * 4) = v;
}

__global__ void unbrick_kernel(const float* __restrict__ src, long NB, int N, int NPB, int H, int W, int BW, float* __restrict__ dst,
                               long total) {
  const long i = (long)blockIdx.x * blockDim.x + threadIdx.x;
  if (i >= total) return;
  const int hw = H * W;
  const long p = i / hw;
  const int c = (int)(i - p * hw);
  const int y = c / W, x = c - y * W;
  const long pair = p / N, pin = p - pair * N;
  const long brick = (long)(y >> 2) * BW + (x >> 3);
  dst[i] = src[(((pair * NPB + (pin >> 6)) * (NB / 32) + brick) * 64 + (pin & 63)) * 32 + (y & 3) * 8 + (x & 7)];
}

}

void launch_brick_rows(const float* src, long sb, int nimg, int H, int W, int C, float* dst, long db, hipStream_t st) {
  ATDN_CHECK(C % 4 == 0 && db % C == 0, "brick_rows: bad geometry");
  const int BW = (W + 7) / 8;
  const long total4 = (long)nimg * (db / C) * (C / 4);
  hipLaunchKernelGGL(brick_rows_kernel, dim3((unsigned)cdivl(total4, 256)), dim3(256), 0, st, src, sb, H, W, BW, C, dst, db, total4);
  ATDN_HIP(hipGetLastError());
}

void launch_unbrick(const float* src, long NB, int N, int H, int W, long npix, float* dst, hipStream_t st) {
  const long total = npix * H * W;
  hipLaunchKernelGGL(unbrick_kernel, dim3((unsigned)cdivl(total, 256)), dim3(256), 0, st, src, NB, N, brick_pixel_blocks(N), H, W,
                     (W + 7) / 8, dst, total);
  ATDN_HIP(hipGetLastError());
}

void launch_lookup_conv(const BrickPyramid& pyr, const float* coords1, long npix, float* coords_used, const float* wfrag,
                        float wscale, const float* bias, float* out, bool fast, hipStream_t st) {
  ATDN_CHECK(wfrag && bias && out, "lookup_conv: missing operand");
  ATDN_CHECK(pyr.N >= 1 && npix % pyr.N == 0, "lookup_conv: npix must be whole pairs of pyr.N pixels");
  const dim3 grid((unsigned)((npix / pyr.N) * cdiv(pyr.N, TP)));
  if (fast) hipLaunchKernelGGL((lookup_conv_kernel<true, true>), grid, dim3(NWAVE * 64), 0, st, pyr, coords1, npix, coords_used, wfrag, wscale, bias, out);
  else hipLaunchKernelGGL((lookup_conv_kernel<true, false>), grid, dim3(NWAVE * 64), 0, st, pyr, coords1, npix, coords_used, wfrag, wscale, bias, out);
  ATDN_HIP(hipGetLastError());
}

void launch_lookup_bricks(const BrickPyramid& pyr, const float* coords1, long npix, float* out, hipStream_t st) {
  ATDN_CHECK(pyr.N >= 1 && npix % pyr.N == 0, "lookup_bricks: npix must be whole pairs of pyr.N pixels");
  hipLaunchKernelGGL((lookup_conv_kernel<false, false>), dim3((unsigned)((npix / pyr.N) * cdiv(pyr.N, TP))), dim3(NWAVE * 64), 0, st, pyr, coords1,
                     npix, nullptr, nullptr, 1.f, nullptr, out);
  ATDN_HIP(hipGetLastError());
}

}
```

### atdn_vslam_amd/csrc/weights.h

```cpp
#pragma once
#include <algorithm>
#include <cmath>
#include <cstring>
#include <map>
#include <string>
#include <vector>

#include "conv_mfma.h"
#include "device_buf.h"

namespace atdn {

struct HostTensor {
  std::vector<int64_t> shape;
  std::vector<float> data;
  long numel() const { long n = 1; for (auto d : shape) n *= d; return n; }
};

class StateDict {
 public:
  void put(const std::string& key, const float* data, const int64_t* shape, int rank) {
    std::string k = key;
    if (k.rfind("module.", 0) == 0) k = k.substr(7);
    HostTensor t;
    t.shape.assign(shape, shape + rank);
    const long n = t.numel();
    t.data.assign(data, data + n);
    map_[k] = std::move(t);
  }
  const HostTensor& get(const std::string& key) const {
    auto it = map_.find(key);
    if (it == map_.end()) throw Error("missing state-dict entry: " + key);
    return it->second;
  }
  bool has(const std::string& key) const { return map_.count(key) != 0; }
  std::vector<std::string> keys() const {
    std::vector<std::string> k;
    for (auto& e : map_) k.push_back(e.first);
    return k;
  }
  size_t size() const { return map_.size(); }

 private:
  std::map<std::string, HostTensor> map_;
};

struct PackedConv {
  long w_off = -1, b_off = -1;
  int N = 0, ldw = 0, KH = 1, KW = 1, C = 0;
  int mode = MODE_TAP;
  float wscale = 1.f;
  const float* w = nullptr;
  const float* b = nullptr;
  long wf_off = -1;
  const float* wf = nullptr;
  long wf16_off = -1;
  const float* wf16 = nullptr;
};

class WeightArena {
 public:
  long alloc(long n) {
    const long off = (long)host_.size();
    host_.resize(off + ((n + 3) / 4) * 4, 0.f);
    return off;
  }
  float* at(long off) { return host_.data() + off; }
  void upload() {
    dev_.alloc((long)host_.size());
    ATDN_HIP(hipMemcpy(dev_.p, host_.data(), host_.size() * sizeof(float), hipMemcpyHostToDevice));
  }
  const float* dev(long off) const { return dev_.p + off; }
  size_t bytes() const { return host_.size() * sizeof(float); }

 private:
  std::vector<float> host_;
  DeviceBuf dev_;
};

struct ChannelAffine { std::vector<double> scale, shift; };

inline ChannelAffine bn_affine(const StateDict& sd, const std::string& p, double eps = 1e-5) {
  const auto& w = sd.get(p + ".weight"); const auto& b = sd.get(p + ".bias");
  const auto& rm = sd.get(p + ".running_mean"); const auto& rv = sd.get(p + ".running_var");
  ChannelAffine a;
  const size_t n = w.data.size();
  a.scale.resize(n); a.shift.resize(n);
  for (size_t i = 0; i < n; ++i) {
    a.scale[i] = (double)w.data[i] / std::sqrt((double)rv.data[i] + eps);
    a.shift[i] = (double)b.data[i] - (double)rm.data[i] * a.scale[i];
  }
  return a;
}

inline PackedConv pack_conv(WeightArena& A, const StateDict& sd, const std::vector<std::string>& names, int mode,
                            int Cpix, const ChannelAffine* fold = nullptr, bool has_bias = true) {
  PackedConv L;
  const HostTensor& w0 = sd.get(names[0] + ".weight");
  ATDN_CHECK(w0.shape.size() == 4, "conv weight must be 4-d");
  const int Cin = (int)w0.shape[1], KH = (int)w0.shape[2], KW = (int)w0.shape[3];
  L.mode = mode; L.KH = KH; L.KW = KW;
  L.C = (mode == MODE_TAP) ? round_up(Cin, 32) : Cpix;
  ATDN_CHECK(L.C >= Cin, "channel padding smaller than Cin");
  L.ldw = packed_k(mode, KH, KW, L.C);
  int N = 0;
  for (auto& nm : names) N += (int)sd.get(nm + ".weight").shape[0];
  L.N = N;
  L.w_off = A.alloc((long)N * L.ldw);
  L.b_off = A.alloc(N);
  int n0 = 0;
  for (auto& nm : names) {
    const HostTensor& w = sd.get(nm + ".weight");
    ATDN_CHECK((int)w.shape[1] == Cin && (int)w.shape[2] == KH && (int)w.shape[3] == KW, "stacked convs must agree");
    const int Co = (int)w.shape[0];
    const float* bias = (has_bias && sd.has(nm + ".bias")) ? sd.get(nm + ".bias").data.data() : nullptr;
    for (int n = 0; n < Co; ++n) {
      const double sc = fold ? fold->scale[n0 + n] : 1.0;
      float* row = A.at(L.w_off + (long)(n0 + n) * L.ldw);
      for (int c = 0; c < Cin; ++c)
        for (int ky = 0; ky < KH; ++ky)
          for (int kx = 0; kx < KW; ++kx) {
            const double v = (double)w.data[(((long)n * Cin + c) * KH + ky) * KW + kx] * sc;
            const long k = (mode == MODE_TAP) ? ((long)(ky * KW + kx) * L.C + c)
                                              : ((long)ky * round_up(KW * L.C, 32) + kx * L.C + c);
            row[k] = (float)v;
          }
      double bv = bias ? (double)bias[n] : 0.0;
      if (fold) bv = bv * sc + fold->shift[n0 + n];
      A.at(L.b_off)[n0 + n] = (float)bv;
    }
    n0 += Co;
  }
  return L;
}

inline void pack_fragment_major16(WeightArena& A, PackedConv& L) {
  const int nq = L.ldw / 32, nblk = (L.N + 15) / 16;
  L.wf16_off = A.alloc((long)nblk * nq * 512);
  const float* w = A.at(L.w_off);
  float* f = A.at(L.wf16_off);
  for (int nb = 0; nb < nblk; ++nb)
    for (int q = 0; q < nq; ++q)
      for (int hl = 0; hl < 2; ++hl)
        for (int lane = 0; lane < 64; ++lane) {
          const int r = lane & 15, gq = lane >> 4, row = nb * 16 + r, slot = 4 * hl + gq;
          float* d = f + ((((long)nb * nq + q) * 2 + hl) * 64 + lane) * 4;
          if (row < L.N) std::memcpy(d, w + (long)row * L.ldw + q * 32 + slot * 4, 16);
          else std::memset(d, 0, 16);
        }
}

inline PackedConv pack_conv_sf(WeightArena& A, const StateDict& sd, const std::vector<std::string>& names,
                               const ChannelAffine* fold = nullptr, bool has_bias = true) {
  PackedConv L = pack_conv(A, sd, names, MODE_TAP, 0, fold, has_bias);
  float* w = A.at(L.w_off);
  const long total = (long)L.N * L.ldw;
  float mx = 0.f;
  for (long i = 0; i < total; ++i) mx = std::max(mx, std::fabs(w[i]));
  int e = 0;
  if (mx > 0.f) (void)std::frexp(mx, &e);
  const int p = 1 - e;
  L.wscale = std::ldexp(1.0f, -p);
  std::vector<float> row(L.ldw);
  for (int n = 0; n < L.N; ++n) {
    float* r = w + (long)n * L.ldw;
    std::memcpy(row.data(), r, L.ldw * sizeof(float));
    _Float16* hrow = reinterpret_cast<_Float16*>(r);
    for (int q = 0; q < L.ldw / 32; ++q)
      for (int j = 0; j < 32; ++j) {
        const float v = std::ldexp(row[q * 32 + j], p);
        const _Float16 hi = (_Float16)v;
        const _Float16 lo = (_Float16)(v - (float)hi);
        hrow[q * 64 + j] = hi;
        hrow[q * 64 + 32 + j] = lo;
      }
  }
  if ((L.KH == 3 && L.KW == 3) || (L.KH == 1 && L.KW == 5) || (L.KH == 5 && L.KW == 1)) {
    pack_fragment_major16(A, L);
  }
  return L;
}

inline void pack_stem_sf(WeightArena& A, PackedConv& L) {
  ATDN_CHECK(L.mode == MODE_ROW && L.KH == 7 && L.KW == 7 && L.C == 4 && L.ldw == 224 && L.N == 64, "stem shape");
  L.wf_off = A.alloc(2L * 14 * 2 * 256);
  const float* w = A.at(L.w_off);
  float mx = 0.f;
  for (long i = 0; i < (long)L.N * L.ldw; ++i) mx = std::max(mx, std::fabs(w[i]));
  int e = 0;
  if (mx > 0.f) (void)std::frexp(mx, &e);
  const int p = 1 - e;
  L.wscale = std::ldexp(1.0f, -p);
  _Float16* f = reinterpret_cast<_Float16*>(A.at(L.wf_off));
  for (int nt = 0; nt < 2; ++nt)
    for (int q = 0; q < 14; ++q)
      for (int lane = 0; lane < 64; ++lane) {
        const int r = lane & 31, h = lane >> 5;
        for (int m = 0; m < 8; ++m) {
          const float v = std::ldexp(w[(long)(nt * 32 + r) * L.ldw + 16 * q + 8 * h + m], p);
          const _Float16 hi = (_Float16)v;
          f[(((long)(nt * 14 + q) * 2 + 0) * 64 + lane) * 8 + m] = hi;
          f[(((long)(nt * 14 + q) * 2 + 1) * 64 + lane) * 8 + m] = (_Float16)(v - (float)hi);
        }
      }
}

inline PackedConv pack_conv_sf_channels(WeightArena& A, const StateDict& sd, const std::vector<std::string>& names,
                                        const std::vector<std::pair<int, int>>& ranges, bool has_bias) {
  StateDict tmp;
  std::vector<std::string> tnames;
  for (size_t t = 0; t < names.size(); ++t) {
    const HostTensor& w = sd.get(names[t] + ".weight");
    const int Co = (int)w.shape[0], Ci = (int)w.shape[1], KH = (int)w.shape[2], KW = (int)w.shape[3];
    int Cn = 0;
    for (auto& r : ranges) Cn += r.second - r.first;
    std::vector<float> out((size_t)Co * Cn * KH * KW);
    for (int n = 0; n < Co; ++n) {
      int c2 = 0;
      for (auto& r : ranges)
        for (int c = r.first; c < r.second; ++c, ++c2)
          std::memcpy(&out[((size_t)n * Cn + c2) * KH * KW], &w.data[((size_t)n * Ci + c) * KH * KW],
                      sizeof(float) * KH * KW);
    }
    const std::string key = "s" + std::to_string(t);
    const int64_t shp[4] = {Co, Cn, KH, KW};
    tmp.put(key + ".weight", out.data(), shp, 4);
    if (has_bias && sd.has(names[t] + ".bias")) {
      const HostTensor& b = sd.get(names[t] + ".bias");
      const int64_t bs[1] = {Co};
      tmp.put(key + ".bias", b.data.data(), bs, 1);
    }
    tnames.push_back(key);
  }
  return pack_conv_sf(A, tmp, tnames, nullptr, has_bias);
}

inline PackedConv pack_gru_sf_folded(WeightArena& A, const StateDict& sd, const std::vector<std::string>& names,
                                     const HostTensor& wv, double gamma) {
  ATDN_CHECK(wv.shape.size() == 4 && wv.shape[0] == 128 && wv.shape[1] == 128 && wv.shape[2] == 1 && wv.shape[3] == 1,
             "aggregator.to_v is a 1x1 convolution, 128 -> 128");
  StateDict tmp;
  std::vector<std::string> tnames;
  for (size_t t = 0; t < names.size(); ++t) {
    const HostTensor& w = sd.get(names[t] + ".weight");
    ATDN_CHECK(w.shape.size() == 4 && w.shape[1] == 512, "ConvGRU convolutions read 512 channels");
    const int Co = (int)w.shape[0], T = (int)(w.shape[2] * w.shape[3]);
    std::vector<float> out((size_t)Co * 384 * T);
    std::vector<double> acc(128);
    for (int n = 0; n < Co; ++n) {
      const float* wn = &w.data[(size_t)n * 512 * T];
      float* on = &out[(size_t)n * 384 * T];
      std::memcpy(on, wn, sizeof(float) * 128 * T);
      for (int c = 0; c < 128; ++c)
        for (int k = 0; k < T; ++k)
          on[(128 + c) * T + k] = (float)((double)wn[(256 + c) * T + k] + (double)wn[(384 + c) * T + k]);
      for (int k = 0; k < T; ++k) {
        std::fill(acc.begin(), acc.end(), 0.0);
        for (int c = 0; c < 128; ++c) {
          const double g = (double)wn[(384 + c) * T + k];
          const float* v = &wv.data[(size_t)c * 128];
          for (int c2 = 0; c2 < 128; ++c2) acc[c2] += g * (double)v[c2];
        }
        for (int c2 = 0; c2 < 128; ++c2) on[(256 + c2) * T + k] = (float)(gamma * acc[c2]);
      }
    }
    const std::string key = "s" + std::to_string(t);
    const int64_t shp[4] = {Co, 384, w.shape[2], w.shape[3]};
    tmp.put(key + ".weight", out.data(), shp, 4);
    if (sd.has(names[t] + ".bias")) {
      const HostTensor& b = sd.get(names[t] + ".bias");
      const int64_t bs[1] = {Co};
      tmp.put(key + ".bias", b.data.data(), bs, 1);
    }
    tnames.push_back(key);
  }
  return pack_conv_sf(A, tmp, tnames, nullptr, true);
}

inline long pack_vector(WeightArena& A, const std::vector<float>& v) {
  const long off = A.alloc((long)v.size());
  std::memcpy(A.at(off), v.data(), v.size() * sizeof(float));
  return off;
}

inline void resolve(const WeightArena& A, PackedConv& L) {
  L.w = A.dev(L.w_off);
  L.b = A.dev(L.b_off);
  L.wf = L.wf_off >= 0 ? A.dev(L.wf_off) : nullptr;
  L.wf16 = L.wf16_off >= 0 ? A.dev(L.wf16_off) : nullptr;
}

}
```

Before: 436.6 frame-pairs/s.

## Fold fnet 1x1 head into correlation via Gram matrix, shrinking K to 160

```diff
diff --git a/atdn_vslam_amd/csrc/capi.hip b/atdn_vslam_amd/csrc/capi.hip
--- a/atdn_vslam_amd/csrc/capi.hip
+++ b/atdn_vslam_amd/csrc/capi.hip
@@ -558,9 +558,9 @@
       src = plain[l - 1].p;
     }
     fbrick[l].alloc((long)B * bp.NB[l] * 256);
-    launch_brick_rows(src, src_sb, B, pH[l], pW[l], 256, fbrick[l].p, (long)bp.NB[l] * 256, st);
+    launch_brick_rows(src, src_sb, B, pH[l], pW[l], 256, 256, fbrick[l].p, (long)bp.NB[l] * 256, st);
     pyr[l].alloc((long)B * bp.NPB * kBrickPixelBlock * bp.NB[l]);
-    launch_corr_bricks(f1.p, (long)N * 256, fbrick[l].p, (long)bp.NB[l] * 256, B, N, bp.NB[l], 1.0f / sqrtf(256.0f), pyr[l].p, false, st);
+    launch_corr_bricks(f1.p, (long)N * 256, fbrick[l].p, (long)bp.NB[l] * 256, B, N, bp.NB[l], 256, 1.0f / sqrtf(256.0f), pyr[l].p, false, st);
     bp.base[l] = pyr[l].p;
     if (rowmajor[l]) launch_unbrick(pyr[l].p, bp.NB[l], N, pH[l], pW[l], n8, rowmajor[l], st);
   }
diff --git a/atdn_vslam_amd/csrc/corr_bricks.hip b/atdn_vslam_amd/csrc/corr_bricks.hip
--- a/atdn_vslam_amd/csrc/corr_bricks.hip
+++ b/atdn_vslam_amd/csrc/corr_bricks.hip
@@ -18,11 +18,13 @@
   float scale;
 };
 
-template <bool FAST>
-__global__ __launch_bounds__(256, 2) void corr_bricks_kernel(const CorrArgs a) {
+constexpr int corr_resident(int nc) { return nc == 5 ? 3 : 2; }
+
+template <int NC, bool FAST>
+__device__ __forceinline__ void corr_bricks_body(const CorrArgs& a) {
   constexpr int KROW = 160;
   constexpr int KT = 32;
-  constexpr int NC = 8;
+  constexpr int ROWB = NC * 128;
   constexpr int CH = KT * KROW;
   constexpr int IMG = NC * CH;
   __shared__ __attribute__((aligned(16))) char lds[2 * IMG];
@@ -42,7 +44,7 @@
 #pragma unroll
   for (int rb = 0; rb < 2; ++rb) {
     mrow[rb] = (strip4 * 4 + wave) * 32 + 16 * rb + n16;
-    const char* qrow = f1 + (long)min(mrow[rb], a.N - 1) * 1024 + 16 * g16;
+    const char* qrow = f1 + (long)min(mrow[rb], a.N - 1) * ROWB + 16 * g16;
 #pragma unroll
     for (int c = 0; c < NC; ++c) {
       qh[rb][c] = *reinterpret_cast<const f16x8*>(qrow + c * 128);
@@ -55,7 +57,7 @@
   const int nt = min(a.tiles_per_split, a.NB / KT - t0);
   v4f kreg[NC];
   auto fetch = [&](int j) __attribute__((always_inline)) {
-    const char* src = f2 + (long)((t0 + j) * KT + lr) * 1024 + 16 * ls;
+    const char* src = f2 + (long)((t0 + j) * KT + lr) * ROWB + 16 * ls;
 #pragma unroll
     for (int c = 0; c < NC; ++c) kreg[c] = *reinterpret_cast<const v4f*>(src + c * 128);
   };
@@ -138,16 +140,23 @@
   }
 }
 
+template <bool FAST>
+__global__ __launch_bounds__(256, corr_resident(8)) void corr_bricks_kernel(const CorrArgs a) { corr_bricks_body<8, FAST>(a); }
+template <bool FAST>
+__global__ __launch_bounds__(256, corr_resident(5)) void corr_bricks_kernel_k160(const CorrArgs a) { corr_bricks_body<5, FAST>(a); }
+
 }
 
-void launch_corr_bricks(const float* f1, long sb1, const float* f2b, long sb2, int B, int N, int NB, float scale, float* out,
-                        bool fast, hipStream_t st) {
+void launch_corr_bricks(const float* f1, long sb1, const float* f2b, long sb2, int B, int N, int NB, int K, float scale,
+                        float* out, bool fast, hipStream_t st) {
   ATDN_CHECK(f1 && f2b && out && B >= 1 && N >= 1 && NB >= 32 && NB % 32 == 0, "corr_bricks: bad argument");
+  ATDN_CHECK(K == 256 || K == 160, "corr_bricks: built for K = 256 (plain features) and K = 160 (folded head)");
   CorrArgs a;
   a.NPB = brick_pixel_blocks(N);
   a.f1 = f1; a.sb1 = sb1; a.f2b = f2b; a.sb2 = sb2; a.out = out; a.B = B; a.N = N; a.NB = NB; a.scale = scale;
   a.strips = cdiv(N, 128);
   const int tiles = NB / 32;
+  const double round_blocks = 256.0 * corr_resident(K / 32);
   int best = 1;
   double best_eff = 0.0;
   for (int s = 1; s <= 8; ++s) {
@@ -155,14 +164,19 @@
     if (s > 1 && tps < 8) break;
     const int used = cdiv(tiles, tps);
     const double blocks = (double)B * a.strips * used;
-    const double eff = blocks / (512.0 * std::ceil(blocks / 512.0));
+    const double eff = blocks / (round_blocks * std::ceil(blocks / round_blocks));
     if (eff > best_eff + 0.02) { best_eff = eff; best = s; }
   }
   a.tiles_per_split = cdiv(tiles, best);
   a.splits = cdiv(tiles, a.tiles_per_split);
   const int nblk = B * a.splits * a.strips;
-  if (fast) hipLaunchKernelGGL(corr_bricks_kernel<true>, dim3(nblk), dim3(256), 0, st, a);
-  else hipLaunchKernelGGL(corr_bricks_kernel<false>, dim3(nblk), dim3(256), 0, st, a);
+  if (K == 256) {
+    if (fast) hipLaunchKernelGGL(corr_bricks_kernel<true>, dim3(nblk), dim3(256), 0, st, a);
+    else hipLaunchKernelGGL(corr_bricks_kernel<false>, dim3(nblk), dim3(256), 0, st, a);
+  } else {
+    if (fast) hipLaunchKernelGGL(corr_bricks_kernel_k160<true>, dim3(nblk), dim3(256), 0, st, a);
+    else hipLaunchKernelGGL(corr_bricks_kernel_k160<false>, dim3(nblk), dim3(256), 0, st, a);
+  }
   ATDN_HIP(hipGetLastError());
 }
 
diff --git a/atdn_vslam_amd/csrc/gma.h b/atdn_vslam_amd/csrc/gma.h
--- a/atdn_vslam_amd/csrc/gma.h
+++ b/atdn_vslam_amd/csrc/gma.h
@@ -51,6 +51,10 @@
   bool par_ok_ = true;
   void fork(hipStream_t from, hipStream_t to);
   DeviceBuf fbrick_[4], fplain_[3], coords_used_;
+  DeviceBuf fpre_, fsrc_;
+  PackedConv fhead_fold_;
+  float corr_mul_ = 1.f;
+  long fhead_w32_off_ = -1, fhead_b32_off_ = -1;
   int brickBW_[4], brickBH_[4], brickNB_[4];
   BrickPyramid brick_pyramid() const;
   DeviceBuf rowmax_, rinv_;
@@ -74,7 +78,7 @@
   void iteration(int B, hipStream_t st);
   void run_body_sf(int B, int iters, hipStream_t st);
   void run_encoder_sf(const EncoderWeights& E, bool instance, int nimg, hipStream_t st, float** out_buf, int first_img = 0,
-                      DeviceBuf* bufs = nullptr);
+                      DeviceBuf* bufs = nullptr, float* final_dst = nullptr);
   void iteration_sf(int B, hipStream_t st);
   void capture(int B, int iters);
   void launch_body(int B, int iters, hipStream_t st);
@@ -103,7 +107,7 @@
   long gamma_off_ = -1;
   long to_v_w32_off_ = -1;
 
-  DeviceBuf img4_, enc_[4], scratch_, pcnt_, fin_, fmap_, psum_, pm2_, mean_[3], rstd_[3];
+  DeviceBuf img4_, enc_[4], scratch_, pcnt_, fin_, fmap_ , psum_, pm2_, mean_[3], rstd_[3];
   DeviceBuf pyr_[4], h_[2], x_, qk_, attn_, vT_, corrfeat_, cor1_, corflo_, flo1_, z_, rh_, fh_, mask_;
   DeviceBuf coords1_, flow4_, pre_zr_[2], pre_q_[2];
   int pyrH_[4], pyrW_[4];
diff --git a/atdn_vslam_amd/csrc/gma.hip b/atdn_vslam_amd/csrc/gma.hip
--- a/atdn_vslam_amd/csrc/gma.hip
+++ b/atdn_vslam_amd/csrc/gma.hip
@@ -212,6 +212,11 @@
   };
   fnet_ = pack_encoder(arena_, sd_, "fnet.", false, sf);
   cnet_ = pack_encoder(arena_, sd_, "cnet.", true, sf);
+  if (sf) {
+    fhead_fold_ = pack_fnet_head_folded(arena_, sd_, "fnet.conv2", &corr_mul_);
+    fhead_w32_off_ = pack_vector(arena_, sd_.get("fnet.conv2.weight").data);
+    fhead_b32_off_ = pack_vector(arena_, sd_.get("fnet.conv2.bias").data);
+  }
   convc1_ = tap({u + "encoder.convc1"});
   if (sf) pack_fragment_major16(arena_, convc1_);
   convc2_ = tap({u + "encoder.convc2"});
@@ -286,7 +291,7 @@
   for (PackedConv* L : {&convc1_, &convc2_, &convf1_, &convf2_, &convm_, &to_v_, &to_qk_, &gru_zr_[0], &gru_zr_[1],
                         &gru_q_[0], &gru_q_[1], &fh1_, &fh2_, &mask0_, &mask2_})
     resolve(arena_, *L);
-  if (sf) for (PackedConv* L : {&gru_zr_ctx_[0], &gru_zr_ctx_[1], &gru_q_ctx_[0], &gru_q_ctx_[1]}) resolve(arena_, *L);
+  if (sf) for (PackedConv* L : {&gru_zr_ctx_[0], &gru_zr_ctx_[1], &gru_q_ctx_[0], &gru_q_ctx_[1], &fhead_fold_}) resolve(arena_, *L);
   gamma_ = arena_.dev(gamma_off_);
 
   const int B = maxB;
@@ -294,7 +299,8 @@
   const long n8 = (long)B * N;
   img4_.alloc(2L * B * H * W * 4);
   for (int i = 0; i < (sf ? 4 : 3); ++i) enc_[i].alloc(2L * B * H2 * W2 * 64);
-  fmap_.alloc(2L * B * N * 256);
+  if (sf) { fpre_.alloc(2L * B * N * 128); fsrc_.alloc((long)B * N * 160); }
+  else fmap_.alloc(2L * B * N * 256);
   const long groups = (long)cdiv(H2 * W2, 64) * 4 + 8;
   psum_.alloc(2L * B * groups * 128); pm2_.alloc(2L * B * groups * 128); pcnt_.alloc(2L * B * groups); fin_.alloc(2L * B * 32 * 128 * 4 * 2);
   for (int i = 0; i < 3; ++i) { mean_[i].alloc(2L * B * 128); rstd_[i].alloc(2L * B * 128); }
@@ -306,8 +312,8 @@
     pyr_[l].alloc(classic_ ? n8 * pyrH_[l] * pyrW_[l] : (long)B * brick_pixel_blocks(N) * kBrickPixelBlock * brickNB_[l]);
   }
   if (sf) {
-    for (int l = 0; l < 4; ++l) fbrick_[l].alloc((long)B * brickNB_[l] * 256);
-    for (int l = 1; l < 4; ++l) fplain_[l - 1].alloc((long)B * pyrH_[l] * pyrW_[l] * 256);
+    for (int l = 0; l < 4; ++l) fbrick_[l].alloc((long)B * brickNB_[l] * 160);
+    for (int l = 1; l < 4; ++l) fplain_[l - 1].alloc((long)B * pyrH_[l] * pyrW_[l] * 128);
     coords_used_.alloc(n8 * 2);
   }
   h_[0].alloc(n8 * 128); h_[1].alloc(n8 * 128); x_.alloc(n8 * XLD);
@@ -333,7 +339,7 @@
   ATDN_HIP(hipMemset(flow4_.p, 0, flow4_.n * sizeof(float)));
   ATDN_HIP(hipDeviceSynchronize());
   ws_bytes_ = 0;
-  DeviceBuf* all[] = {&img4_, &enc_[0], &enc_[1], &enc_[2], &enc_[3], &fmap_, &psum_, &pm2_, &pyr_[0], &pyr_[1], &pyr_[2],
+  DeviceBuf* all[] = {&img4_, &enc_[0], &enc_[1], &enc_[2], &enc_[3], &fmap_, &fpre_, &fsrc_, &psum_, &pm2_, &pyr_[0], &pyr_[1], &pyr_[2],
                       &pyr_[3], &h_[0], &h_[1], &x_, &qk_, &attn_, &vT_, &corrfeat_, &cor1_, &corflo_, &flo1_, &z_,
                       &rh_, &fh_, &mask_, &coords1_, &flow4_};
   for (auto* b : all) ws_bytes_ += (size_t)b->n * sizeof(float);
@@ -555,7 +561,7 @@
 }
 
 void GmaNet::run_encoder_sf(const EncoderWeights& E, bool instance, int nimg, hipStream_t st, float** out_buf, int first_img,
-                            DeviceBuf* bufs) {
+                            DeviceBuf* bufs, float* final_dst) {
   const float* images = img4_.p + (long)first_img * H * W * 4;
   int h = conv_out(H, 7, 2, 3), w = conv_out(W, 7, 2, 3);
   DeviceBuf* eb = bufs ? bufs : enc_;
@@ -603,6 +609,7 @@
     const int co = Bk.c1.N;
     const int oh = conv_out(h, 3, stride, 1), ow = conv_out(w, 3, stride, 1);
     const long ohw = (long)oh * ow;
+    if (bi == 5 && final_dst) O = final_dst;
     if (instance && norm_on_load_) {
       const bool raw_in = stem_raw && bi == 0;
       ATDN_CHECK(!raw_in || !Bk.has_ds, "the block behind the stem has no downsample branch");
@@ -700,26 +707,25 @@
   const int nfeat = seq_ == 0 ? 2 * B : seq_ == 1 ? B + 1 : B;
   hipStream_t sB = par_ ? par_stream_ : st;
   if (par_) fork(st, sB);
-  run_encoder_sf(fnet_, true, nfeat, st, &f, seq_ == 2 ? 1 : 0);
-  ConvShape s = conv_shape(fnet_.head, f, 128, (long)N * 128, nfeat, H8, W8, 1, 0, 0);
-  float* fdst = fmap_.p + (seq_ == 2 ? (long)N * 256 : 0);
-  conv_sf_dispatch(s, fnet_.head.wscale, SfBias<ACT_NONE>{fnet_.head.b, fdst, (long)N * 256, 256}, st);
+  run_encoder_sf(fnet_, true, nfeat, st, &f, seq_ == 2 ? 1 : 0, nullptr, fpre_.p + (seq_ == 2 ? (long)N * 128 : 0));
+  ConvShape s = conv_shape(fhead_fold_, fpre_.p, 128, (long)N * 128, B, H8, W8, 1, 0, 0);
+  conv_sf_dispatch(s, fhead_fold_.wscale, SfBias<ACT_NONE>{fhead_fold_.b, fsrc_.p, (long)N * 160, 160}, st);
   mark(ST_FNET, st);
 
-  const float* target = fmap_.p + (long)(seq_ ? 1 : B) * N * 256;
+  const float* target = fpre_.p + (long)(seq_ ? 1 : B) * N * 128;
   for (int l = 0; l < 4; ++l) {
     const float* plain = target;
-    long plain_sb = (long)N * 256;
+    long plain_sb = (long)N * 128;
     if (l > 0) {
       const float* prev = l == 1 ? target : fplain_[l - 2].p;
-      const long prev_sb = l == 1 ? (long)N * 256 : (long)pyrH_[l - 1] * pyrW_[l - 1] * 256;
-      plain_sb = (long)pyrH_[l] * pyrW_[l] * 256;
-      launch_pool_features_sf(prev, B, pyrH_[l - 1], pyrW_[l - 1], 256, prev_sb, fplain_[l - 1].p, plain_sb, st);
+      const long prev_sb = l == 1 ? (long)N * 128 : (long)pyrH_[l - 1] * pyrW_[l - 1] * 128;
+      plain_sb = (long)pyrH_[l] * pyrW_[l] * 128;
+      launch_pool_features_sf(prev, B, pyrH_[l - 1], pyrW_[l - 1], 128, prev_sb, fplain_[l - 1].p, plain_sb, st);
       plain = fplain_[l - 1].p;
     }
-    launch_brick_rows(plain, plain_sb, B, pyrH_[l], pyrW_[l], 256, fbrick_[l].p, (long)brickNB_[l] * 256, st);
-    launch_corr_bricks(fmap_.p, (long)N * 256, fbrick_[l].p, (long)brickNB_[l] * 256, B, N, brickNB_[l], 1.0f / sqrtf(256.0f), pyr_[l].p,
-                       sf_fast_mode(), st);
+    launch_brick_rows(plain, plain_sb, B, pyrH_[l], pyrW_[l], 128, 160, fbrick_[l].p, (long)brickNB_[l] * 160, st);
+    launch_corr_bricks(fsrc_.p, (long)N * 160, fbrick_[l].p, (long)brickNB_[l] * 160, B, N, brickNB_[l], 160,
+                       corr_mul_ / sqrtf(256.0f), pyr_[l].p, sf_fast_mode(), st);
     if (l == 0) mark(ST_CORR, st);
   }
   mark(ST_POOL, st);
@@ -812,7 +818,7 @@
   const long frame = 3L * H * W;
   if (continued) {
     ATDN_CHECK(last_frame_ >= 1, "continued sequence call without a previous sequence call on this handle");
-    ATDN_HIP(hipMemcpyAsync(fmap_.p, fmap_.p + (long)last_frame_ * N * 256, (size_t)N * 256 * sizeof(float),
+    ATDN_HIP(hipMemcpyAsync(fpre_.p, fpre_.p + (long)last_frame_ * N * 128, (size_t)N * 128 * sizeof(float),
                             hipMemcpyDeviceToDevice, st));
     seq_ = 2;
   } else {
@@ -925,6 +931,16 @@
   else if (k == "mask") b = &mask_; else if (k == "coords1") b = &coords1_; else if (k == "flow4") b = &flow4_;
   else if (k == "qk") b = &qk_; else if (k == "img4") b = &img4_;
   else if (k == "cor1") b = &cor1_;
+  if (k == "fmap" && !classic_) {
+    const long rows = 2L * maxB * N;
+    scratch_.reserve(rows * (128 + 256));
+    launch_from_sf(fpre_.p, scratch_.p, rows, 128, st);
+    launch_linear_rows(scratch_.p, rows, 128, arena_.dev(fhead_w32_off_), arena_.dev(fhead_b32_off_), 256, scratch_.p + rows * 128, st);
+    ATDN_HIP(hipStreamSynchronize(st));
+    const long n = std::min(capacity, rows * 256);
+    ATDN_HIP(hipMemcpy(host, scratch_.p + rows * 128, (size_t)n * sizeof(float), hipMemcpyDeviceToHost));
+    return n;
+  }
   if (k == "agg") {
     if (classic_) return -1;
     scratch_.reserve(x_.n);
diff --git a/atdn_vslam_amd/csrc/kernels.h b/atdn_vslam_amd/csrc/kernels.h
--- a/atdn_vslam_amd/csrc/kernels.h
+++ b/atdn_vslam_amd/csrc/kernels.h
@@ -78,9 +78,10 @@
   int NPB;
 };
 inline int brick_pixel_blocks(int N) { return 2 * ((N + 127) / 128); }
-void launch_brick_rows(const float* src, long sb, int nimg, int H, int W, int C, float* dst, long db, hipStream_t st);
-void launch_corr_bricks(const float* f1, long sb1, const float* f2b, long sb2, int B, int N, int NB, float scale, float* out,
-                        bool fast, hipStream_t st);
+void launch_brick_rows(const float* src, long sb, int nimg, int H, int W, int C, int Cd, float* dst, long db, hipStream_t st);
+void launch_corr_bricks(const float* f1, long sb1, const float* f2b, long sb2, int B, int N, int NB, int K, float scale,
+                        float* out, bool fast, hipStream_t st);
+void launch_linear_rows(const float* in, long rows, int Cin, const float* w, const float* b, int Cout, float* out, hipStream_t st);
 void launch_unbrick(const float* src, long NB, int N, int H, int W, long npix, float* dst, hipStream_t st);
 void launch_lookup_conv(const BrickPyramid& pyr, const float* coords1, long npix, float* coords_used, const float* wfrag,
                         float wscale, const float* bias, float* out, bool fast, hipStream_t st);
diff --git a/atdn_vslam_amd/csrc/kernels.hip b/atdn_vslam_amd/csrc/kernels.hip
--- a/atdn_vslam_amd/csrc/kernels.hip
+++ b/atdn_vslam_amd/csrc/kernels.hip
@@ -639,6 +639,26 @@
                             const float* coords_used, int N, int W8, int cflow, hipStream_t st) {
   if (rows <= 0) return;
   hipLaunchKernelGGL(mfg_reconstruct_kernel, dim3((unsigned)rows), dim3(128), 0, st, x, ld, cmf, cagg, wv, gamma, coords_used, N, W8, cflow);
+  ATDN_HIP(hipGetLastError());
+}
+
+__global__ __launch_bounds__(256) void linear_rows_kernel(const float* __restrict__ in, int Cin, const float* __restrict__ w,
+                                                          const float* __restrict__ b, int Cout, float* __restrict__ out) {
+  __shared__ float a[256];
+  const long r = blockIdx.x;
+  for (int c = threadIdx.x; c < Cin; c += blockDim.x) a[c] = in[r * Cin + c];
+  __syncthreads();
+  for (int o = threadIdx.x; o < Cout; o += blockDim.x) {
+    float s = b ? b[o] : 0.f;
+    for (int k = 0; k < Cin; ++k) s = fmaf(w[(long)o * Cin + k], a[k], s);
+    out[r * Cout + o] = s;
+  }
+}
+
+void launch_linear_rows(const float* in, long rows, int Cin, const float* w, const float* b, int Cout, float* out, hipStream_t st) {
+  ATDN_CHECK(Cin >= 1 && Cin <= 256 && Cout >= 1, "linear_rows: bad geometry");
+  if (rows <= 0) return;
+  hipLaunchKernelGGL(linear_rows_kernel, dim3((unsigned)rows), dim3(256), 0, st, in, Cin, w, b, Cout, out);
   ATDN_HIP(hipGetLastError());
 }
 
diff --git a/atdn_vslam_amd/csrc/lookup_fused.hip b/atdn_vslam_amd/csrc/lookup_fused.hip
--- a/atdn_vslam_amd/csrc/lookup_fused.hip
+++ b/atdn_vslam_amd/csrc/lookup_fused.hip
@@ -261,21 +261,24 @@
   }
 }
 
-__global__ void brick_rows_kernel(const float* __restrict__ src, long sb, int H, int W, int BW, int C,
+__global__ void brick_rows_kernel(const float* __restrict__ src, long sb, int H, int W, int BW, int C, int Cd,
                                   float* __restrict__ dst, long db, long total4) {
   const long i = (long)blockIdx.x * blockDim.x + threadIdx.x;
   if (i >= total4) return;
-  const int c4 = C / 4;
+  const int c4 = Cd / 4;
   const int part = (int)(i % c4);
   const long row = i / c4;
-  const long per_img = db / C;
+  const long per_img = db / Cd;
   const long img = row / per_img;
   const int n = (int)(row - img * per_img);
   const int brick = n >> 5, within = n & 31;
   const int y = (brick / BW) * 4 + (within >> 3), x = (brick % BW) * 8 + (within & 7);
   v4f v = {0.f, 0.f, 0.f, 0.f};
-  if (y < H && x < W) v = *reinterpret_cast<const v4f*>(src + img * sb + ((long)y * W + x) * C + part * 4);
-  *reinterpret_cast<v4f*>(dst + img * db + (long)n * C + part * 4) = v;
+  if (y < H && x < W) {
+    if (part * 4 < C) v = *reinterpret_cast<const v4f*>(src + img * sb + ((long)y * W + x) * C + part * 4);
+    else if (part * 4 == C) v[0] = __int_as_float(0x3C00);
+  }
+  *reinterpret_cast<v4f*>(dst + img * db + (long)n * Cd + part * 4) = v;
 }
 
 __global__ void unbrick_kernel(const float* __restrict__ src, long NB, int N, int NPB, int H, int W, int BW, float* __restrict__ dst,
@@ -293,11 +296,11 @@
 
 }
 
-void launch_brick_rows(const float* src, long sb, int nimg, int H, int W, int C, float* dst, long db, hipStream_t st) {
-  ATDN_CHECK(C % 4 == 0 && db % C == 0, "brick_rows: bad geometry");
+void launch_brick_rows(const float* src, long sb, int nimg, int H, int W, int C, int Cd, float* dst, long db, hipStream_t st) {
+  ATDN_CHECK(C % 4 == 0 && (Cd == C || (Cd == C + 32 && C % 32 == 0)) && db % Cd == 0, "brick_rows: bad geometry");
   const int BW = (W + 7) / 8;
-  const long total4 = (long)nimg * (db / C) * (C / 4);
-  hipLaunchKernelGGL(brick_rows_kernel, dim3((unsigned)cdivl(total4, 256)), dim3(256), 0, st, src, sb, H, W, BW, C, dst, db, total4);
+  const long total4 = (long)nimg * (db / Cd) * (Cd / 4);
+  hipLaunchKernelGGL(brick_rows_kernel, dim3((unsigned)cdivl(total4, 256)), dim3(256), 0, st, src, sb, H, W, BW, C, Cd, dst, db, total4);
   ATDN_HIP(hipGetLastError());
 }
 
diff --git a/atdn_vslam_amd/csrc/weights.h b/atdn_vslam_amd/csrc/weights.h
--- a/atdn_vslam_amd/csrc/weights.h
+++ b/atdn_vslam_amd/csrc/weights.h
@@ -277,6 +277,50 @@
   return pack_conv_sf(A, tmp, tnames, nullptr, true);
 }
 
+inline PackedConv pack_fnet_head_folded(WeightArena& A, const StateDict& sd, const std::string& name, float* corr_mul) {
+  const HostTensor& w = sd.get(name + ".weight");
+  ATDN_CHECK(w.shape.size() == 4 && w.shape[0] == 256 && w.shape[1] == 128 && w.shape[2] == 1 && w.shape[3] == 1,
+             "the feature head is a 1x1 convolution, 128 -> 256");
+  std::vector<double> b(256, 0.0);
+  if (sd.has(name + ".bias")) {
+    const HostTensor& bt = sd.get(name + ".bias");
+    ATDN_CHECK(bt.data.size() == 256, "feature head bias");
+    for (int o = 0; o < 256; ++o) b[o] = (double)bt.data[o];
+  }
+  std::vector<double> M(128 * 128, 0.0), u(128, 0.0);
+  double bb = 0.0;
+  for (int o = 0; o < 256; ++o) {
+    const float* wo = &w.data[(size_t)o * 128];
+    bb += b[o] * b[o];
+    for (int i = 0; i < 128; ++i) {
+      const double wi = (double)wo[i];
+      u[i] += wi * b[o];
+      for (int j = 0; j < 128; ++j) M[i * 128 + j] += wi * (double)wo[j];
+    }
+  }
+  double rs = 0.0;
+  for (int i = 0; i < 128; ++i) {
+    double s = 0.0;
+    for (int j = 0; j < 128; ++j) s += std::fabs(M[i * 128 + j]);
+    rs = std::max(rs, s);
+  }
+  int k = 0;
+  if (rs > 0.0) (void)std::frexp(rs, &k);
+  std::vector<float> wf(160 * 128, 0.f), bf(160, 0.f);
+  for (int i = 0; i < 128; ++i) {
+    for (int j = 0; j < 128; ++j) wf[i * 128 + j] = (float)std::ldexp(M[i * 128 + j], -k);
+    bf[i] = (float)std::ldexp(u[i], -k);
+    wf[128 * 128 + i] = (float)std::ldexp(u[i], -k);
+  }
+  bf[128] = (float)std::ldexp(bb, -k);
+  StateDict tmp;
+  const int64_t shp[4] = {160, 128, 1, 1}, bs[1] = {160};
+  tmp.put("s0.weight", wf.data(), shp, 4);
+  tmp.put("s0.bias", bf.data(), bs, 1);
+  *corr_mul = std::ldexp(1.0f, k);
+  return pack_conv_sf(A, tmp, {"s0"}, nullptr, true);
+}
+
 inline long pack_vector(WeightArena& A, const std::vector<float>& v) {
   const long off = A.alloc((long)v.size());
   std::memcpy(A.at(off), v.data(), v.size() * sizeof(float));
```

Measured after the change: 443.6 frame-pairs/s (median of 6 runs). 1.6% higher.
